# ma-compbio/MATCHA

Measured on AMD Instinct MI355X. Metric: training hyperedges/sec at k∈{2..5}, embed_dim=64; 1/2/4/8 MI355X, higher is better.
Workload: dtype f32; 1 GPU; hg38_1mb bins (N=3067), k in {2,3,4,5} mixed-k zero-padded to L=5, embed_dim=64, front end=table, neg_num=3, dropout on, AdamW lr=1e-3, 400000 known hyperedges; parallelism=dp1, hipgraph=False, table_gradient_exchange=none, embedding_backward=float atomics, exchange_overlapped=False

## Files before the change

### matcha_amd/csrc/front_fused.hip

```cpp
#include <string.h>

#include "attr_src.hpp"
#include "kernels.hpp"
#include "prep_heads.hpp"

namespace matcha {

typedef float f32x16 __attribute__((ext_vector_type(16)));

namespace {

constexpr int kLd = 68;
constexpr int kTile = 64 * kLd;
constexpr int kLdA = 36;
constexpr int kAttrCols = 32;
constexpr int kFrontSlab = 4096 + 64 * kAttrCols + 128;
constexpr float kEps = 1e-5f;

struct FrontBwdArgs {
  const float* X; const float* dxh; int nslab; int64_t tcap; const float* dxpad; const float* dXs; const float* x0;
  const int64_t* ids; AttrSrc attr; int n_attr;
  const float* Wn;
  const int32_t* count;
  float* dX0;
  float* dtable;
  float* slab;
};

template <bool NODE>
__global__ __launch_bounds__(256, 2) void front_bwd_kernel(FrontBwdArgs g) {
  extern __shared__ __attribute__((aligned(16))) float lds[];
  float* Ws = lds;
  float* Zs = lds + 1 * kTile;
  float* X0s = lds + 2 * kTile;
  float* Ds = lds + 3 * kTile;
  float* As = lds + 4 * kTile;
  int* ids_s = reinterpret_cast<int*>(As + 64 * kLdA);
  const int tid = threadIdx.x, lane = tid & 63, wave = tid >> 6;
  const int r = lane & 31, h = lane >> 5, wr = wave & 1, wc = wave >> 1;
  const int srow = tid >> 4, sc4 = (tid & 15) * 4;
  const int T = g.count[0];
  const int ntiles = (T + 63) / 64;
#pragma unroll
  for (int i = 0; i < 4; ++i)
    *reinterpret_cast<float4*>(&Ws[(srow + 16 * i) * kLd + sc4]) = *reinterpret_cast<const float4*>(g.Wn + (srow + 16 * i) * 64 + sc4);
  f32x16 aWn = {0}, aWa = {0};
  float csz = 0.f, csd = 0.f;

  float4 pxv[4], pdv[4], psv[4], px0[4], pav[2];
  int pid = 0;
  const float4 dxp = *reinterpret_cast<const float4*>(g.dxpad + sc4);
  const int a_row0 = tid >> 3, a_q = (tid & 7) * 4;
  const int a_qc = a_q < g.n_attr ? a_q : 0;
#define FBW_GLOAD(TILE)                                                                                  \
  do {                                                                                                   \
    const int64_t tb__ = (int64_t)(TILE) * 64;                                                           \
    _Pragma("unroll") for (int i__ = 0; i__ < 4; ++i__) {                                                \
// ... 84 lines not shown
          if (id != 0) atomicAdd(g.dtable + (int64_t)id * 64 + col, acc[reg]);
        }
      }
    }
#pragma unroll 8
    for (int m = 0; m < 32; ++m) {
      const int t = 2 * m + h;
      const float gz = Zs[t * kLd + 32 * wr + r];
      csz += gz;
      aWn = __builtin_amdgcn_mfma_f32_32x32x2f32(gz, X0s[t * kLd + 32 * wc + r], aWn, 0, 0, 0);
    }
    __syncthreads();
    if (g.dX0) {
#pragma unroll
      for (int i = 0; i < 4; ++i) {
        const int row = srow + 16 * i;
        const int64_t t = t_base + row;
        if (t < T) *reinterpret_cast<float4*>(g.dX0 + t * 64 + sc4) = *reinterpret_cast<const float4*>(&Ds[row * kLd + sc4]);
      }
    }
    if (wc == 0) {
#pragma unroll 8
      for (int m = 0; m < 32; ++m) {
        const int t = 2 * m + h;
        const float gd = Ds[t * kLd + 32 * wr + r];
        csd += gd;
        aWa = __builtin_amdgcn_mfma_f32_32x32x2f32(gd, As[t * kLdA + r], aWa, 0, 0, 0);
      }
    }
  }
  float* slab = g.slab + (int64_t)blockIdx.x * kFrontSlab;
#pragma unroll
  for (int reg = 0; reg < 16; ++reg) {
    const int row = 32 * wr + (reg & 3) + 8 * (reg >> 2) + 4 * h;
    slab[row * 64 + 32 * wc + r] = aWn[reg];
    if (wc == 0) slab[4096 + row * kAttrCols + r] = aWa[reg];
  }
  csz += __shfl_xor(csz, 32, 64);
  csd += __shfl_xor(csd, 32, 64);
  if (wc == 0 && h == 0) {
    slab[4096 + 64 * kAttrCols + 32 * wr + r] = csz;
    slab[4096 + 64 * kAttrCols + 64 + 32 * wr + r] = csd;
  }
}

struct FrontFwdArgs {
  const int64_t* ids; const float* table; const float* dense;
  AttrSrc attr; int n_attr;
  const float* Wa; const float* ba; const float* Wn; const float* bn;
  const int32_t* count;
  float* x0; float* X;
  int nprep; PrepArgs prep;
  int prep_walks;
};

__global__ __launch_bounds__(256, 3) void front_fwd_kernel(FrontFwdArgs g) {
  extern __shared__ __attribute__((aligned(16))) float lds[];
  const int nprep = g.nprep;
  if ((int)blockIdx.x < nprep) {
    const int b = blockIdx.x;
    prep_heads_role(g.prep, b % kPrepGridX, (b / kPrepGridX) % kPrepGridY, b / (kPrepGridX * kPrepGridY), lds);
    if (!g.prep_walks) return;
    __syncthreads();
  }
  const int nlate = g.prep_walks ? nprep : 0;
  const int vb = (int)blockIdx.x - (nprep - nlate), Gf = (int)gridDim.x - (nprep - nlate);
  float* Es = lds;
  float* As = lds + kTile;
  float* Xs = As + 64 * kLdA;
  const int tid = threadIdx.x, lane = tid & 63, wave = tid >> 6;
  const int r = lane & 31, h = lane >> 5, wr = wave & 1, wc = wave >> 1;
  const int srow = tid >> 4, sc4 = (tid & 15) * 4;
  const int T = g.count[0];
  const int ntiles = (T + 63) / 64;
  const int q = ntiles / Gf, r_last = ntiles - q * Gf;
  const int last_slot = vb >= nlate ? vb - nlate : vb - nlate + Gf;
  const int tile_last = last_slot < r_last ? q * Gf + last_slot : 0x3FFFFFF;
#define FF_TILE(IT) ((IT) < q ? vb + (IT) * Gf : ((IT) == q ? tile_last : 0x3FFFFFF))
  float4 wn[8], wa[kAttrCols / 8];
#pragma unroll
  for (int c = 0; c < 8; ++c) wn[c] = *reinterpret_cast<const float4*>(g.Wn + (32 * wc + r) * 64 + 8 * c + 4 * h);
#pragma unroll
  for (int c = 0; c < kAttrCols / 8; ++c) {
    const int q = 8 * c + 4 * h;
    wa[c] = make_float4(0.f, 0.f, 0.f, 0.f);
    if (q < g.n_attr) wa[c] = *reinterpret_cast<const float4*>(g.Wa + (32 * wc + r) * g.n_attr + q);
  }
  const int col = 32 * wc + r;
  const float bav = g.ba[col], bnv = g.bn[col];

  const int arow0 = tid >> 3, aq = (tid & 7) * 4;
  int64_t id_e[4], id_a[2];
  float4 pe[4], pa[2], qe[4], qa[2];
  const float amask = aq < g.n_attr ? 1.f : 0.f;
  const int aqc = aq < g.n_attr ? aq : g.n_attr - 4;
  const int64_t t_last = (int64_t)T - 1;
#define FF_IDS_GLOAD(TILE)                                                                               \
  do {                                                                                                   \
    const int64_t tb__ = (int64_t)(TILE) * 64;                                                           \
    _Pragma("unroll") for (int i__ = 0; i__ < 4; ++i__) {                                                \
      const int64_t t__ = tb__ + srow + 16 * i__;                                                        \
      id_e[i__] = g.ids[t__ < t_last ? t__ : t_last];                                                    \
    }                                                                                                    \
    _Pragma("unroll") for (int j__ = 0; j__ < 2; ++j__) {                                                \
      const int64_t t__ = tb__ + arow0 + 32 * j__;                                                       \
      id_a[j__] = g.ids[t__ < t_last ? t__ : t_last];                                                    \
    }                                                                                                    \
  } while (0)
#define FF_ROWS_GLOAD(TILE)                                                                              \
  do {                                                                                                   \
    const int64_t tb__ = (int64_t)(TILE) * 64;                                                           \
    _Pragma("unroll") for (int i__ = 0; i__ < 4; ++i__) {                                                \
      const int64_t t__ = tb__ + srow + 16 * i__;                                                        \
      const float* src__ = g.table ? g.table + id_e[i__] * 64 : g.dense + (t__ < t_last ? t__ : t_last) * 64; \
      pe[i__] = *reinterpret_cast<const float4*>(src__ + sc4);                                           \
    }                                                                                                    \
    _Pragma("unroll") for (int j__ = 0; j__ < 2; ++j__) {                                                \
      const float4 v__ = *reinterpret_cast<const float4*>(g.attr.table + id_a[j__] * g.attr.ld + aqc);   \
      pa[j__] = make_float4(v__.x * amask, v__.y * amask, v__.z * amask, v__.w * amask);                 \
// ... 46 lines not shown
        acc = __builtin_amdgcn_mfma_f32_32x32x2f32(a.y, b.y, acc, 0, 0, 0);
        acc = __builtin_amdgcn_mfma_f32_32x32x2f32(a.z, b.z, acc, 0, 0, 0);
        acc = __builtin_amdgcn_mfma_f32_32x32x2f32(a.w, b.w, acc, 0, 0, 0);
      }
#pragma unroll
      for (int reg = 0; reg < 16; ++reg) {
        const int row = 32 * wr + (reg & 3) + 8 * (reg >> 2) + 4 * h;
        const float v = acc[reg] + bav + Es[row * kLd + col];
        Es[row * kLd + col] = v;
      }
    }
    __syncthreads();
#pragma unroll
    for (int i = 0; i < 4; ++i) {
      const int row = srow + 16 * i;
      if (g.x0 && t_base + row < T) *reinterpret_cast<float4*>(g.x0 + (t_base + row) * 64 + sc4) = *reinterpret_cast<const float4*>(&Es[row * kLd + sc4]);
    }
    {
      f32x16 acc = {0};
#pragma unroll
      for (int c = 0; c < 8; ++c) {
        const float4 a = *reinterpret_cast<const float4*>(&Es[(32 * wr + r) * kLd + 8 * c + 4 * h]);
        const float4 b = wn[c];
        acc = __builtin_amdgcn_mfma_f32_32x32x2f32(a.x, b.x, acc, 0, 0, 0);
        acc = __builtin_amdgcn_mfma_f32_32x32x2f32(a.y, b.y, acc, 0, 0, 0);
        acc = __builtin_amdgcn_mfma_f32_32x32x2f32(a.z, b.z, acc, 0, 0, 0);
        acc = __builtin_amdgcn_mfma_f32_32x32x2f32(a.w, b.w, acc, 0, 0, 0);
      }
#pragma unroll
      for (int reg = 0; reg < 16; ++reg) {
        const int row = 32 * wr + (reg & 3) + 8 * (reg >> 2) + 4 * h;
        Xs[row * kLd + col] = fast_tanh(acc[reg] + bnv);
      }
    }
    __syncthreads();
#pragma unroll
    for (int i = 0; i < 4; ++i) {
      const int row = srow + 16 * i;
      if (t_base + row < T) *reinterpret_cast<float4*>(g.X + (t_base + row) * 64 + sc4) = *reinterpret_cast<const float4*>(&Xs[row * kLd + sc4]);
    }
  }
}

constexpr int kFPS = 80;
#define FF2_STORE4(P, A, B, C, D) (*reinterpret_cast<f32x4*>(P) = (f32x4){(A), (B), (C), (D)})
constexpr int kF3Lds = (3 * 64 * kFPS) / 2 + (kAttrCols + 2) * 64 + 64;

template <bool TRAIN>
__global__ __launch_bounds__(256, 4) void front_fwd3_kernel(FrontFwdArgs g) {
  extern __shared__ __attribute__((aligned(16))) float lds[];
  const int nprep = g.nprep;
  const int tid = threadIdx.x, lane = tid & 63, wave = tid >> 6;
  bool late = false;
  if ((int)blockIdx.x < nprep) {
    const int b = blockIdx.x;
    prep_heads_role(g.prep, b % kPrepGridX, (b / kPrepGridX) % kPrepGridY, b / (kPrepGridX * kPrepGridY), lds);
    if (!g.prep_walks) return;
    __syncthreads();
    late = true;
  }
  short* Wp = reinterpret_cast<short*>(lds);
  float* WaT = lds + (3 * 64 * kFPS) / 2;
  int* bnd = reinterpret_cast<int*>(WaT + (kAttrCols + 2) * 64);
  const int c16 = lane & 15, kq = lane >> 4;
  const int na = g.n_attr;
  {
    const int srow = tid >> 4, sc4 = (tid & 15) * 4;
#pragma unroll
    for (int i = 0; i < 4; ++i) {
      const int n = srow + 16 * i;
      const float4 w = *reinterpret_cast<const float4*>(g.Wn + n * 64 + sc4);
      const P3 p0 = split2(w.x, w.y), p1 = split2(w.z, w.w);
      short* d = Wp + n * kFPS + sc4;
      *reinterpret_cast<u32x2*>(d) = (u32x2){p0.h, p1.h}; *reinterpret_cast<u32x2*>(d + 64 * kFPS) = (u32x2){p0.m, p1.m};
      *reinterpret_cast<u32x2*>(d + 2 * 64 * kFPS) = (u32x2){p0.l, p1.l};
    }
    for (int i = tid; i < (na + 2) * 64; i += 256) {
      const int a = i >> 6, c = i & 63;
      WaT[i] = a < na - 1 ? g.Wa[c * na + a] : (a == na - 1 ? 0.f : (a == na ? g.Wa[c * na + na - 1] : g.ba[c]));
    }
    if (tid < na) bnd[tid] = g.attr.bounds[tid];
  }
  __syncthreads();
  const int T = g.count[0];
  const int64_t t_last = (int64_t)T - 1;
  const int ngroups = (T + 15) / 16;
  const int W = (int)gridDim.x * 4, Wn_ = W - nprep * 4;
  const int r0 = g.prep_walks > 0 ? g.prep_walks - 1 : 0x3FFFFF;
  const int wv = late ? (int)blockIdx.x * 4 + wave : ((int)blockIdx.x - nprep) * 4 + wave;
  const float scale = g.attr.scale;
  const int* ids32 = reinterpret_cast<const int*>(g.ids);
  const float4 bn4 = *reinterpret_cast<const float4*>(g.bn + 4 * kq);
#define F3_GROUP(R) ((R) < r0 ? (late ? 0x3FFFFFF : (R) * Wn_ + wv) : r0 * Wn_ + ((R) - r0) * W + (late ? wv : nprep * 4 + wv))
#define F3_LOAD(GRP, ID, E)                                                                              \
  do {                                                                                                   \
    const int64_t t__ = (int64_t)(GRP) * 16 + c16;                                                       \
    const int64_t tc__ = t__ < t_last ? t__ : t_last;                                                    \
    ID = ids32[2 * tc__];                                                                                \
    const float* src__ = (g.table ? g.table + (int64_t)ID * 64 : g.dense + tc__ * 64) + 8 * kq;          \
    E[0] = *reinterpret_cast<const float4*>(src__); E[1] = *reinterpret_cast<const float4*>(src__ + 4);   \
    E[2] = *reinterpret_cast<const float4*>(src__ + 32); E[3] = *reinterpret_cast<const float4*>(src__ + 36); \
  } while (0)
  int idn = 0;
  float4 en[4];
  const int r_first = late ? r0 : 0;
  int grp = F3_GROUP(r_first);
  if (grp < ngroups) F3_LOAD(grp, idn, en);
  for (int r = r_first; grp < ngroups; ++r) {
    const int id = idn;
    float4 e[4];
#pragma unroll
    for (int i = 0; i < 4; ++i) e[i] = en[i];
    const int gnext = F3_GROUP(r + 1);
    if (gnext < ngroups) F3_LOAD(gnext, idn, en);
    const int64_t t = (int64_t)grp * 16 + c16;
    const int nb_ = na - 1, top = bnd[nb_];
    const int idc = id < 1 ? 1 : (id > top ? top : id);
    const int ch = attr_chrom(bnd, nb_, idc);
    const bool real = id >= 1 && id <= top;
    const int wrow = real ? ch : nb_;
    const float co = real ? __fdiv_rn((float)(idc - bnd[ch] - 1), scale) : 0.f;
    Frag3 xf[2];
#pragma unroll
    for (int s2 = 0; s2 < 2; ++s2) {
      const int k0 = 32 * s2 + 8 * kq;
      float v[8];
#pragma unroll
      for (int hf = 0; hf < 2; ++hf) {
        const float4 wc_ = *reinterpret_cast<const float4*>(&WaT[wrow * 64 + k0 + 4 * hf]);
        const float4 wl_ = *reinterpret_cast<const float4*>(&WaT[na * 64 + k0 + 4 * hf]);
        const float4 ba_ = *reinterpret_cast<const float4*>(&WaT[(na + 1) * 64 + k0 + 4 * hf]);
        const float4 ee = e[2 * s2 + hf];
        v[4 * hf + 0] = (__builtin_fmaf(co, wl_.x, wc_.x) + ba_.x) + ee.x; v[4 * hf + 1] = (__builtin_fmaf(co, wl_.y, wc_.y) + ba_.y) + ee.y;
        v[4 * hf + 2] = (__builtin_fmaf(co, wl_.z, wc_.z) + ba_.z) + ee.z; v[4 * hf + 3] = (__builtin_fmaf(co, wl_.w, wc_.w) + ba_.w) + ee.w;
        if (TRAIN && t < T) FF2_STORE4(g.x0 + t * 64 + k0 + 4 * hf, v[4 * hf], v[4 * hf + 1], v[4 * hf + 2], v[4 * hf + 3]);
      }
      xf[s2] = split8(v);
    }
#pragma unroll 1
    for (int nb = 0; nb < 4; ++nb) {
      f32x4 acc = {0.f, 0.f, 0.f, 0.f};
      const short* ap = Wp + (16 * nb + c16) * kFPS + 8 * kq;
#pragma unroll
      for (int s2 = 0; s2 < 2; ++s2) {
        Frag3 a;
        a.h = *reinterpret_cast<const u32x4*>(ap + 32 * s2); a.m = *reinterpret_cast<const u32x4*>(ap + 32 * s2 + 64 * kFPS);
        a.l = *reinterpret_cast<const u32x4*>(ap + 32 * s2 + 2 * 64 * kFPS);
        acc = mma6(acc, a, xf[s2]);
      }
      const float4 bb = *reinterpret_cast<const float4*>(g.bn + 16 * nb + 4 * kq);
      if (t < T) FF2_STORE4(g.X + t * 64 + 16 * nb + 4 * kq, fast_tanh(acc[0] + bb.x), fast_tanh(acc[1] + bb.y), fast_tanh(acc[2] + bb.z), fast_tanh(acc[3] + bb.w));
    }
    grp = gnext;
  }
#undef F3_GROUP
#undef F3_LOAD
}

__global__ __launch_bounds__(256) void node_xhat_kernel(const float* __restrict__ XN, const int32_t* __restrict__ count, float* __restrict__ xh) {
  const int64_t row = (int64_t)blockIdx.x * 16 + (threadIdx.x >> 4);
  const int c4 = (threadIdx.x & 15) * 4;
  const int T = count[0];
  const float4 xv = *reinterpret_cast<const float4*>(XN + (row < T ? row : (int64_t)T - 1) * 64 + c4);
  const float mean = group_sum16_dpp((xv.x + xv.y) + (xv.z + xv.w)) * (1.f / 64.f);
  const float a = xv.x - mean, b = xv.y - mean, c = xv.z - mean, e = xv.w - mean;
  const float rs = __builtin_amdgcn_rsqf(group_sum16_dpp((a * a + b * b) + (c * c + e * e)) * (1.f / 64.f) + kEps);
  if (row < T) *reinterpret_cast<float4*>(xh + row * 64 + c4) = make_float4(a * rs, b * rs, c * rs, e * rs);
}

struct NodeScatterArgs {
  const float* XN; const float* dxh; const float* dxpad; const float* dXs; const int32_t* key; const int32_t* count;
  float* G;
  const int32_t* ncount; int64_t rows;
};
__device__ __forceinline__ void node_finish(const NodeScatterArgs& g) {
  const int64_t row = (int64_t)blockIdx.x * 16 + (threadIdx.x >> 4);
  const int c4 = (threadIdx.x & 15) * 4;
  const int T = g.ncount[0];
  const int64_t rc = row < T ? row : (int64_t)T - 1;
  const float4 xv = *reinterpret_cast<const float4*>(g.XN + rc * 64 + c4);
  float4 a[MATCHA_N_HEAD];
#pragma unroll
  for (int h = 0; h < MATCHA_N_HEAD; ++h) a[h] = *reinterpret_cast<const float4*>(g.dxh + ((int64_t)h * g.rows + rc) * 64 + c4);
  const float4 s = *reinterpret_cast<const float4*>(g.G + rc * 64 + c4);
  float4 d;
  d.x = ((a[0].x + a[1].x) + (a[2].x + a[3].x)) + ((a[4].x + a[5].x) + (a[6].x + a[7].x));
  d.y = ((a[0].y + a[1].y) + (a[2].y + a[3].y)) + ((a[4].y + a[5].y) + (a[6].y + a[7].y));
  d.z = ((a[0].z + a[1].z) + (a[2].z + a[3].z)) + ((a[4].z + a[5].z) + (a[6].z + a[7].z));
  d.w = ((a[0].w + a[1].w) + (a[2].w + a[3].w)) + ((a[4].w + a[5].w) + (a[6].w + a[7].w));
  if (rc == 0) {
    const float4 dxp = *reinterpret_cast<const float4*>(g.dxpad + c4);
    d.x += dxp.x; d.y += dxp.y; d.z += dxp.z; d.w += dxp.w;
  }
  const float mean = group_sum16_dpp((xv.x + xv.y) + (xv.z + xv.w)) * (1.f / 64.f);
  const float a0 = xv.x - mean, a1 = xv.y - mean, a2 = xv.z - mean, a3 = xv.w - mean;
  const float rs = __builtin_amdgcn_rsqf(group_sum16_dpp((a0 * a0 + a1 * a1) + (a2 * a2 + a3 * a3)) * (1.f / 64.f) + kEps);
  const float4 xh = make_float4(a0 * rs, a1 * rs, a2 * rs, a3 * rs);
  const float ma = group_sum16_dpp((d.x + d.y) + (d.z + d.w)) * (1.f / 64.f);
  const float mb = group_sum16_dpp((d.x * xh.x + d.y * xh.y) + (d.z * xh.z + d.w * xh.w)) * (1.f / 64.f);
  if (row < T)
    *reinterpret_cast<float4*>(g.G + row * 64 + c4) =
        make_float4(rs * (d.x - ma - xh.x * mb) + s.x, rs * (d.y - ma - xh.y * mb) + s.y, rs * (d.z - ma - xh.z * mb) + s.z, rs * (d.w - ma - xh.w * mb) + s.w);
}
__global__ __launch_bounds__(256) void node_scatter_kernel(NodeScatterArgs g) {
  if (g.ncount) { node_finish(g); return; }
  __shared__ __attribute__((aligned(16))) float rows_s[2][16 * 64];
  __shared__ int keys_s[2][16];
  const int tid = threadIdx.x, lane = tid & 63, wave = tid >> 6;
  const int srow = tid >> 4, sc4 = (tid & 15) * 4;
  const int T = g.count[0];
  const int ntrips = (T + 15) / 16;
  const float4 dxp = *reinterpret_cast<const float4*>(g.dxpad + sc4);
  const int stride = (int)gridDim.x;
  auto tok_of = [&](int trip) { const int64_t t = (int64_t)trip * 16 + srow; return t < T ? t : (int64_t)T - 1; };
  int kn = g.key[tok_of(blockIdx.x)], knn = g.key[tok_of(blockIdx.x + stride < ntrips ? blockIdx.x + stride : blockIdx.x)];
  float4 xn, dn, sn;
  {
    const int64_t tc = tok_of(blockIdx.x);
    xn = *reinterpret_cast<const float4*>(g.XN + (int64_t)kn * 64 + sc4);
    dn = *reinterpret_cast<const float4*>(g.dxh + tc * 64 + sc4);
    sn = *reinterpret_cast<const float4*>(g.dXs + tc * 64 + sc4);
  }
  int buf = 0;
  for (int trip = blockIdx.x; trip < ntrips; trip += stride, buf ^= 1) {
    const int64_t t = (int64_t)trip * 16 + srow;
    const bool valid = t < T;
    const int key = kn;
    const float4 xv = xn, s = sn;
    const float4 d = t >= (int64_t)T - 1 ? dxp : dn;
    {
      const int nxt = trip + stride < ntrips ? trip + stride : trip, nxt2 = nxt + stride < ntrips ? nxt + stride : nxt;
      const int64_t tc = tok_of(nxt);
      kn = knn;
      xn = *reinterpret_cast<const float4*>(g.XN + (int64_t)kn * 64 + sc4);
      dn = *reinterpret_cast<const float4*>(g.dxh + tc * 64 + sc4);
      sn = *reinterpret_cast<const float4*>(g.dXs + tc * 64 + sc4);
      knn = g.key[tok_of(nxt2)];
    }
    const float mean = group_sum16_dpp((xv.x + xv.y) + (xv.z + xv.w)) * (1.f / 64.f);
    const float a0 = xv.x - mean, a1 = xv.y - mean, a2 = xv.z - mean, a3 = xv.w - mean;
    const float rs = __builtin_amdgcn_rsqf(group_sum16_dpp((a0 * a0 + a1 * a1) + (a2 * a2 + a3 * a3)) * (1.f / 64.f) + kEps);
    const float4 xh = make_float4(a0 * rs, a1 * rs, a2 * rs, a3 * rs);
    const float ma = group_sum16_dpp((d.x + d.y) + (d.z + d.w)) * (1.f / 64.f);
    const float mb = group_sum16_dpp((d.x * xh.x + d.y * xh.y) + (d.z * xh.z + d.w * xh.w)) * (1.f / 64.f);
    *reinterpret_cast<float4*>(&rows_s[buf][srow * 64 + sc4]) =
        make_float4(rs * (d.x - ma - xh.x * mb) + s.x, rs * (d.y - ma - xh.y * mb) + s.y, rs * (d.z - ma - xh.z * mb) + s.z, rs * (d.w - ma - xh.w * mb) + s.w);
    if ((tid & 15) == 0) keys_s[buf][srow] = valid ? key : -1;
    __syncthreads();
#pragma unroll
    for (int i = 0; i < 4; ++i) {
      const int row = 4 * wave + i, k = keys_s[buf][row];
      if (k >= 0) atomicAdd(g.G + (int64_t)k * 64 + lane, rows_s[buf][row * 64 + lane]);
    }
  }
}

struct FrontReduceArgs {
  const float* slab; int nwg; int n_attr;
  float* dWn; float* dWa; float* dbn; float* dba;
  int32_t* touched;
};
__global__ __launch_bounds__(1024) void front_slab_reduce_kernel(FrontReduceArgs a) {
  __shared__ float part[16][64];
  if (a.touched && blockIdx.x == 0 && threadIdx.x < 2) a.touched[threadIdx.x] = 1;
  const int o = threadIdx.x & 63, q = threadIdx.x >> 6;
  const int i = blockIdx.x * 64 + o;
  float s = 0.f;
  if (i < kFrontSlab) {
    float s0 = 0.f, s1 = 0.f, s2 = 0.f, s3 = 0.f;
    int b = q;
    for (; b + 48 < a.nwg; b += 64) {
      s0 += a.slab[(int64_t)b * kFrontSlab + i]; s1 += a.slab[(int64_t)(b + 16) * kFrontSlab + i];
      s2 += a.slab[(int64_t)(b + 32) * kFrontSlab + i]; s3 += a.slab[(int64_t)(b + 48) * kFrontSlab + i];
    }
    for (; b < a.nwg; b += 16) s0 += a.slab[(int64_t)b * kFrontSlab + i];
    s = (s0 + s1) + (s2 + s3);
  }
  part[q][o] = s;
  __syncthreads();
  if (q == 0 && i < kFrontSlab) {
    float t = 0.f;
#pragma unroll
    for (int u = 0; u < 16; ++u) t += part[u][o];
    if (i < 4096) a.dWn[i] += t;
    else if (i < 4096 + 64 * kAttrCols) {
      const int n = (i - 4096) / kAttrCols, c = (i - 4096) % kAttrCols;
      if (c < a.n_attr) a.dWa[n * a.n_attr + c] += t;
    } else if (i < 4096 + 64 * kAttrCols + 64) a.dbn[i - 4096 - 64 * kAttrCols] += t;
    else a.dba[i - 4096 - 64 * kAttrCols - 64] += t;
  }
}

int front_grid() {
  const int n = 2 * device_cu_count();
  return n > 1024 ? 1024 : n;
}

}

int launch_front_fwd(const matcha_tensors& p, const int64_t* ids, const float* table, const float* dense, const matcha_frozen& f, int n_attr,
                     const Ragged& rg, int64_t tcap, float* x0, float* X, hipStream_t st, const PrepSpec* prep, const int32_t* count) {
  MATCHA_CHECK_ARG(f.attr_table, "front end: attr_table is required (also under attr_mode 1)");
  FrontFwdArgs g;
  const bool computed = f.attr_mode == 1 && f.attr_bounds && n_attr <= kAttrCols;
  g.ids = ids; g.table = table; g.dense = dense; g.attr = computed ? attr_src(f, n_attr) : attr_src_table_first(f, n_attr); g.n_attr = n_attr;
  g.Wa = p.attr_w; g.ba = p.attr_b; g.Wn = p.next_w; g.bn = p.next_b; g.count = count ? count : rg.count; g.x0 = x0; g.X = X;
  const int slots = front_grid() / 2 * 3;
  const int64_t max_tiles = cdiv(tcap, 64);
  const size_t lds = ((size_t)2 * kTile + 64 * kLdA) * sizeof(float);
  static_assert(((size_t)2 * kTile + 64 * kLdA) >= (size_t)kPrepLdsFloats && kF3Lds >= kPrepLdsFloats, "the weight-form role needs its LDS inside the front end's");
  g.nprep = 0;
  if (prep) {
    prep_heads_args(*prep->p, prep->folded, prep->merged, prep->frag, g.prep);
    g.nprep = kPrepBlocks;
  } else {
    memset(&g.prep, 0, sizeof(g.prep));
  }
  g.prep_walks = (g.nprep > 0 && max_tiles + g.nprep > slots) ? 1 : 0;
  int64_t grid = g.prep_walks ? slots : g.nprep + (max_tiles < slots ? max_tiles : slots);
  if (grid < g.nprep + 1) grid = g.nprep + 1;
  ProfScope ps(MATCHA_PROF_FRONT_FWD, (double)tcap * (8.0 + 256.0 + (computed ? 0.0 : 4.0 * n_attr) + (x0 ? 512.0 : 256.0)), st);
  if (computed) {
    const int slots4 = front_grid() * 2;
    const int64_t ngroups = cdiv(tcap, 16);
    const int64_t rounds = cdiv(ngroups, (int64_t)slots4 * 4);
    g.prep_walks = (g.nprep > 0 && rounds >= 4) ? 3 : 0;
    int64_t grid3 = g.prep_walks ? slots4 : g.nprep + (cdiv(ngroups, 4) < slots4 ? cdiv(ngroups, 4) : slots4);
    if (grid3 < g.nprep + 1) grid3 = g.nprep + 1;
    const size_t lds3 = (size_t)kF3Lds * sizeof(float);
    static_assert(kF3Lds >= kPrepLdsFloats, "the weight-form role needs its LDS inside the front end's");
    if (x0) hipLaunchKernelGGL(front_fwd3_kernel<true>, dim3((unsigned)grid3), dim3(256), lds3, st, g);
    else hipLaunchKernelGGL(front_fwd3_kernel<false>, dim3((unsigned)grid3), dim3(256), lds3, st, g);
    MATCHA_CHECK_LAUNCH("front_fwd3_kernel");
  } else {
    hipLaunchKernelGGL(front_fwd_kernel, dim3((unsigned)grid), dim3(256), lds, st, g);
    MATCHA_CHECK_LAUNCH("front_fwd_kernel");
  }
  return MATCHA_OK;
}

int launch_node_xhat(const float* XN, const int32_t* node_count, int64_t rows_cap, float* xhatN, hipStream_t st) {
  ProfScope ps(MATCHA_PROF_FRONT_FWD, (double)rows_cap * 512.0, st);
  hipLaunchKernelGGL(node_xhat_kernel, dim3((unsigned)cdiv(rows_cap, 16)), dim3(256), 0, st, XN, node_count, xhatN);
  MATCHA_CHECK_LAUNCH("node_xhat_kernel");
  return MATCHA_OK;
}

int launch_node_scatter(const float* XN, const float* dxh, const float* dxpad, const float* dXs, const Ragged& rg, int64_t tcap, float* G, hipStream_t st,
                        const int32_t* node_count, int64_t rows) {
  NodeScatterArgs g;
  g.XN = XN; g.dxh = dxh; g.dxpad = dxpad; g.dXs = dXs; g.key = rg.tok_key; g.count = rg.count; g.G = G; g.ncount = node_count; g.rows = rows;
  if (node_count) {
    MATCHA_CHECK_ARG(rows > 0, "node_scatter: the per-node finisher needs the table's row count");
    ProfScope ps(MATCHA_PROF_FRONT_BWD, (double)rows * (MATCHA_N_HEAD + 3.0) * 256.0, st);
    hipLaunchKernelGGL(node_scatter_kernel, dim3((unsigned)cdiv(rows, 16)), dim3(256), 0, st, g);
    MATCHA_CHECK_LAUNCH("node_scatter_kernel");
    return MATCHA_OK;
  }
  int64_t grid = (int64_t)front_grid() * 4;
  const int64_t trips = cdiv(tcap, 16);
  if (grid > trips) grid = trips;
  ProfScope ps(MATCHA_PROF_FRONT_BWD, (double)tcap * (4.0 * 256.0 + 4.0), st);
  hipLaunchKernelGGL(node_scatter_kernel, dim3((unsigned)grid), dim3(256), 0, st, g);
  MATCHA_CHECK_LAUNCH("node_scatter_kernel");
  return MATCHA_OK;
}

bool front_bwd_supported(int d, int n_attr) { return d == 64 && n_attr >= 4 && n_attr <= kAttrCols && n_attr % 4 == 0; }
size_t front_bwd_ws_floats() { return (size_t)1024 * kFrontSlab; }

int launch_front_bwd(const matcha_tensors& p, const float* X, const float* dxh, int nslab, int64_t tcap, const float* dxpad, const float* dXs, const float* x0,
                     const int64_t* ids, const matcha_frozen& f, int n_attr, const Ragged& rg, float* dX0, float* dtable, float* ws,
                     matcha_tensors& grads, hipStream_t st, int32_t* touched, const int32_t* node_count) {
  MATCHA_CHECK_ARG(f.attr_table, "front end: attr_table is required (also under attr_mode 1)");
  FrontBwdArgs g;
  g.X = X; g.dxh = dxh; g.nslab = nslab; g.tcap = tcap; g.dxpad = dxpad; g.dXs = dXs; g.x0 = x0; g.ids = ids; g.attr = attr_src_table_first(f, n_attr); g.n_attr = n_attr;
  g.Wn = p.next_w; g.count = node_count ? node_count : rg.count; g.dX0 = dX0; g.dtable = dtable; g.slab = ws;
  const bool node = node_count != nullptr;
  int grid = front_grid();
  const int64_t max_tiles = cdiv(tcap, 64);
  if (grid > max_tiles) grid = (int)max_tiles;
  const size_t lds = ((size_t)4 * kTile + 64 * kLdA + 64) * sizeof(float);
  (void)hipFuncSetAttribute(reinterpret_cast<const void*>(node ? front_bwd_kernel<true> : front_bwd_kernel<false>), hipFuncAttributeMaxDynamicSharedMemorySize, (int)lds);
  {
    ProfScope ps(MATCHA_PROF_FRONT_BWD, (double)tcap * ((3.0 + (node ? 0 : nslab)) * 256.0 + 8.0 + (g.attr.mode == 1 ? 0.0 : 4.0 * n_attr) + 256.0), st);
    if (node) hipLaunchKernelGGL(front_bwd_kernel<true>, dim3(grid), dim3(256), lds, st, g);
    else hipLaunchKernelGGL(front_bwd_kernel<false>, dim3(grid), dim3(256), lds, st, g);
    MATCHA_CHECK_LAUNCH("front_bwd_kernel");
  }
  FrontReduceArgs a;
  a.slab = ws; a.nwg = grid; a.n_attr = n_attr; a.dWn = grads.next_w; a.dWa = grads.attr_w; a.dbn = grads.next_b; a.dba = grads.attr_b;
  a.touched = touched;
  hipLaunchKernelGGL(front_slab_reduce_kernel, dim3((unsigned)cdiv(kFrontSlab, 64)), dim3(1024), 0, st, a);
  MATCHA_CHECK_LAUNCH("front_slab_reduce_kernel");
  return MATCHA_OK;
}

}
```

### matcha_amd/csrc/fused_bwd.hip

```cpp
#include <stdlib.h>
#include <string.h>

#include "bf16x3.hpp"
#include "kernels.hpp"
#include "tail_reduce.hpp"

namespace matcha {

typedef float f32x16 __attribute__((ext_vector_type(16)));

namespace {

constexpr int kLd = 68;
constexpr float kEpsLn = 1e-5f;
constexpr int kWgSlab = 4 * 4096 + 6 * 64;
constexpr int kVecOff = 4 * 4096;
constexpr int kMaxChunks = 64;

#define ZR8(p)                                                                                           \
  do {                                                                                                   \
    *reinterpret_cast<float4*>(p) = make_float4(0.f, 0.f, 0.f, 0.f);                                     \
    *reinterpret_cast<float4*>((p) + 4) = make_float4(0.f, 0.f, 0.f, 0.f);                               \
  } while (0)

__device__ __forceinline__ void ln_row16(const float4& v, float& mean, float& rstd) {
  const float s = group_sum<16>((v.x + v.y) + (v.z + v.w));
  mean = s * (1.f / 64.f);
  const float a = v.x - mean, b = v.y - mean, c = v.z - mean, e = v.w - mean;
  const float q = group_sum<16>((a * a + b * b) + (c * c + e * e));
  rstd = __builtin_amdgcn_rsqf(q * (1.f / 64.f) + kEpsLn);
}


#define FB_PIN(addr, x) asm volatile("" : "+v"(addr), "+v"((x).a), "+v"((x).b), "+v"((x).c), "+v"((x).d))
template <int ML>
__device__ __forceinline__ void attn_row8_kv(const float* __restrict__ Qs, const float* __restrict__ Xs, const float* __restrict__ Fs,
                                             const float* __restrict__ xpad, const float* __restrict__ Ps, float* __restrict__ dSs, int li, int li0,
                                             int k, int n_pad, int sub, float inv_temp, V8& o, V8& gq, V8& accK, V8& accV) {
  const float padf = (float)n_pad;
  const bool hp = n_pad > 0;
  float p[ML], ds[ML], pp;
  {
    const float4 pa = *reinterpret_cast<const float4*>(&Ps[li * 8]), pb = *reinterpret_cast<const float4*>(&Ps[li * 8 + 4]);
    const float w[8] = {pa.x, pa.y, pa.z, pa.w, pb.x, pb.y, pb.z, pb.w};
#pragma unroll
    for (int j = 0; j < ML; ++j) p[j] = (j < k) ? w[j] : 0.f;
    pp = hp ? w[7] : 0.f;
  }
  const float ppf = padf * pp;
  const int ro0 = li0 * kLd + 8 * sub;
  const V8 go = ld8(&Fs[li * kLd + 8 * sub]);
  const V8 vp = ld8(xpad + 8 * sub);
  const float dsp_raw = group_sum8_dpp(dot8(go, vp));
  float sig = ppf * dsp_raw;
  o = scale8(ppf, vp);
  V8 a = scale8(ppf * dsp_raw, vp);
  V8 vn = ld8(&Xs[ro0]), vn2 = ld8(&Xs[ro0 + (1 < k ? 1 : 0) * kLd]);
#pragma unroll
  for (int j = 0; j < ML; ++j) {
    const V8 v = vn;
    vn = vn2;
    if (j + 2 < ML) {
      int ad = ro0 + (j + 2 < k ? j + 2 : 0) * kLd;
      FB_PIN(ad, o);
      vn2 = ld8(&Xs[ad]);
    }
    axpy8(o, p[j], v);
    const float d = group_sum8_dpp(dot8(go, v));
    ds[j] = d;
    const float wd = p[j] * d;
    sig += wd;
    axpy8(a, wd, v);
  }
#pragma unroll
  for (int j = 0; j < ML; ++j) ds[j] = p[j] * (ds[j] - sig) * inv_temp;
  const float dspf = padf * (pp * (dsp_raw - sig) * inv_temp);
  axpy8(accV, ppf, go);
  {
    const float ns = -sig;
    axpy8(a, ns, o);
    gq = scale8(inv_temp, a);
  }
  {
    int ad = li * kLd + 8 * sub;
// ... 551 lines not shown
    if (tid < 64) upad[tid] = (redu[tid] + redu[64 + tid]) + (redu[128 + tid] + redu[192 + tid]);
    __syncthreads();
    {
      const float xc = xpad[fb + c16];
#pragma unroll
      for (int reg = 0; reg < 4; ++reg) {
        const int row = 4 * kq + reg, col = fb + c16;
        slab[1 * 4096 + row * 64 + col] = am0[reg] + upad[row] * xc; slab[1 * 4096 + (row + 16) * 64 + col] = am1[reg] + upad[row + 16] * xc;
        slab[1 * 4096 + (row + 32) * 64 + col] = am2[reg] + upad[row + 32] * xc; slab[1 * 4096 + (row + 48) * 64 + col] = am3[reg] + upad[row + 48] * xc;
      }
    }
    if (tid < 64) {
      const float* mp = g.mM + (int64_t)head * 4096 + tid;
      float s0 = 0.f, s1 = 0.f, s2 = 0.f, s3 = 0.f;
#pragma unroll 4
      for (int n = 0; n < 64; n += 4) {
        s0 += upad[n] * mp[n * 64]; s1 += upad[n + 1] * mp[(n + 1) * 64]; s2 += upad[n + 2] * mp[(n + 2) * 64]; s3 += upad[n + 3] * mp[(n + 3) * 64];
      }
      slab[kVecOffM + 128 + tid] = ((redp[tid] + redp[64 + tid]) + (redp[128 + tid] + redp[192 + tid])) + ((s0 + s1) + (s2 + s3));
    }
  }
}

struct ChainArgs {
  const float* wslab; int nchunks;
  float* red;
  const float* wq; const float* wk; const float* wv; const float* cq; const float* cv;
  const float* fc1_w;
  float* out;
  float* dxpad;
};
constexpr int kFbmReduceX = (kWgSlabM + 255) / 256;
constexpr int kFbmReduceBlocks = kFbmReduceX * MATCHA_N_HEAD;
__global__ __launch_bounds__(256) void fbm_reduce_kernel(ChainArgs a, TailReduceArgs tl, int tail_blocks) {
  __shared__ float4 part[8 * 32];
  if ((int)blockIdx.x >= kFbmReduceBlocks) {
    tail_reduce_role(tl, (int)blockIdx.x - kFbmReduceBlocks, part);
    return;
  }
  const int head = blockIdx.x / kFbmReduceX, i = (blockIdx.x % kFbmReduceX) * 256 + threadIdx.x;
  if (i >= kWgSlabM) return;
  const float* base = a.wslab + (int64_t)head * a.nchunks * kWgSlabM + i;
  float s0 = 0.f, s1 = 0.f, s2 = 0.f, s3 = 0.f, s4 = 0.f, s5 = 0.f, s6 = 0.f, s7 = 0.f;
  int c = 0;
  for (; c + 7 < a.nchunks; c += 8) {
    s0 += base[(int64_t)c * kWgSlabM]; s1 += base[(int64_t)(c + 1) * kWgSlabM]; s2 += base[(int64_t)(c + 2) * kWgSlabM]; s3 += base[(int64_t)(c + 3) * kWgSlabM];
    s4 += base[(int64_t)(c + 4) * kWgSlabM]; s5 += base[(int64_t)(c + 5) * kWgSlabM]; s6 += base[(int64_t)(c + 6) * kWgSlabM]; s7 += base[(int64_t)(c + 7) * kWgSlabM];
  }
  for (; c < a.nchunks; ++c) s0 += base[(int64_t)c * kWgSlabM];
  a.red[(int64_t)head * kWgSlabM + i] = ((s0 + s1) + (s2 + s3)) + ((s4 + s5) + (s6 + s7));
}
__device__ __forceinline__ void mm64_slice(const float* __restrict__ A, int a_rs, int a_cs, const float* __restrict__ B, int b_rs, int b_cs,
                                           const float* __restrict__ u, const float* __restrict__ v, float* __restrict__ out, int slice,
                                           float* __restrict__ As, float* __restrict__ Bs) {
  const int tid = threadIdx.x;
  {
    float av[4], bv[16];
#pragma unroll
    for (int t = 0; t < 4; ++t) { const int i = tid + 256 * t; av[t] = A[(int64_t)(16 * slice + (i >> 6)) * a_rs + (int64_t)(i & 63) * a_cs]; }
#pragma unroll
    for (int t = 0; t < 16; ++t) { const int i = tid + 256 * t; bv[t] = B[(int64_t)(i >> 6) * b_rs + (int64_t)(i & 63) * b_cs]; }
#pragma unroll
    for (int t = 0; t < 4; ++t) { const int i = tid + 256 * t; As[(i >> 6) * 65 + (i & 63)] = av[t]; }
#pragma unroll
    for (int t = 0; t < 16; ++t) { const int i = tid + 256 * t; Bs[(i >> 6) * 65 + (i & 63)] = bv[t]; }
  }
  __syncthreads();
  const int lane = tid & 63, wave = tid >> 6, c16 = lane & 15, kq = lane >> 4;
  f32x4 acc = {0.f, 0.f, 0.f, 0.f};
#pragma unroll
  for (int kk = 0; kk < 16; ++kk) acc = MFMA16(As[c16 * 65 + 4 * kk + kq], Bs[(4 * kk + kq) * 65 + 16 * wave + c16], acc);
  const int j = 16 * wave + c16;
  const float vj = u ? v[j] : 0.f;
#pragma unroll
  for (int reg = 0; reg < 4; ++reg) {
    const int i = 4 * kq + reg;
    out[(16 * slice + i) * 64 + j] = acc[reg] + (u ? u[16 * slice + i] * vj : 0.f);
  }
}
__global__ __launch_bounds__(256) void fbm_chain_kernel(ChainArgs a) {
  __shared__ float As[16 * 65];
  __shared__ float Bs[64 * 65];
  const int slice = blockIdx.x, job = blockIdx.y, head = blockIdx.z, tid = threadIdx.x;
  const float* red = a.red + (int64_t)head * kWgSlabM;
  const float* dB = red; const float* dM = red + 4096; const float* db = red + kVecOffM;
  const float* dbdyn = a.red + kVecOffM + 64;
  const float* Wq = a.wq + (int64_t)head * 4096; const float* Wk = a.wk + (int64_t)head * 4096; const float* Wv = a.wv + (int64_t)head * 4096;
  const float* Wf = a.fc1_w + head * 64;
  float* out = a.out + (int64_t)head * kWgSlab;
  if (job == 0) {
    mm64_slice(Wk, 64, 1, dB, 64, 1, nullptr, nullptr, out + 0 * 4096, slice, As, Bs);
  } else if (job == 1) {
    mm64_slice(Wq, 64, 1, dB, 1, 64, a.cq + head * 64, db, out + 1 * 4096, slice, As, Bs);
  } else if (job == 2) {
    mm64_slice(Wf, 1, 512, dM, 64, 1, nullptr, nullptr, out + 2 * 4096, slice, As, Bs);
  } else {
    mm64_slice(dM, 64, 1, Wv, 1, 64, dbdyn, a.cv + head * 64, out + 3 * 4096, slice, As, Bs);
  }
  if (slice == 0 && job == 0 && tid < 64) {
    float s0 = 0.f, s1 = 0.f, t0 = 0.f, t1 = 0.f;
#pragma unroll 8
    for (int x = 0; x < 64; x += 2) {
      s0 += Wk[tid * 64 + x] * db[x]; s1 += Wk[tid * 64 + x + 1] * db[x + 1];
      t0 += Wf[x * 512 + tid] * dbdyn[x]; t1 += Wf[(x + 1) * 512 + tid] * dbdyn[x + 1];
    }
    const float s = s0 + s1, t = t0 + t1;
    out[kVecOff + tid] = s;
    out[kVecOff + 64 + tid] = 0.f;
    out[kVecOff + 128 + tid] = t;
    out[kVecOff + 192 + tid] = 0.f; out[kVecOff + 256 + tid] = 0.f;
    out[kVecOff + 320 + tid] = head == 0 ? dbdyn[tid] : 0.f;
    if (head == 0) {
      float p = 0.f;
      for (int hh = 0; hh < MATCHA_N_HEAD; ++hh) p += a.red[(int64_t)hh * kWgSlabM + kVecOffM + 128 + tid];
      a.dxpad[tid] = p;
    }
  }
}

struct UnfoldArgs {
  const float* wslab; int nchunks;
  const float* X; const int32_t* count; int x_pad_row0;
  const float* W[3]; const float* g[3]; const float* b[3];
  float* gW[3]; float* gfc1;
  float* part;
};
__global__ __launch_bounds__(256) void fb_unfold_kernel(UnfoldArgs a) {
  __shared__ float red[16][3][64];
  const int slice = blockIdx.x, mat = blockIdx.y, head = blockIdx.z;
  const int tid = threadIdx.x, rl = tid >> 4, c4 = (tid & 15) * 4;
  const int row = slice * 16 + rl;
  const float* base = a.wslab + (int64_t)head * a.nchunks * kWgSlab;
  float4 s = make_float4(0.f, 0.f, 0.f, 0.f);
  {
    float4 t0 = s, t1 = s, t2 = s, t3 = s;
    const float* pb = base + mat * 4096 + row * 64 + c4;
    int c = 0;
    for (; c + 3 < a.nchunks; c += 4) {
      const float4 v0 = *reinterpret_cast<const float4*>(pb + (int64_t)c * kWgSlab), v1 = *reinterpret_cast<const float4*>(pb + (int64_t)(c + 1) * kWgSlab);
      const float4 v2 = *reinterpret_cast<const float4*>(pb + (int64_t)(c + 2) * kWgSlab), v3 = *reinterpret_cast<const float4*>(pb + (int64_t)(c + 3) * kWgSlab);
      t0.x += v0.x; t0.y += v0.y; t0.z += v0.z; t0.w += v0.w;
      t1.x += v1.x; t1.y += v1.y; t1.z += v1.z; t1.w += v1.w;
      t2.x += v2.x; t2.y += v2.y; t2.z += v2.z; t2.w += v2.w;
      t3.x += v3.x; t3.y += v3.y; t3.z += v3.z; t3.w += v3.w;
    }
    for (; c < a.nchunks; ++c) {
      const float4 v = *reinterpret_cast<const float4*>(pb + (int64_t)c * kWgSlab);
      t0.x += v.x; t0.y += v.y; t0.z += v.z; t0.w += v.w;
    }
    s.x = (t0.x + t1.x) + (t2.x + t3.x); s.y = (t0.y + t1.y) + (t2.y + t3.y);
    s.z = (t0.z + t1.z) + (t2.z + t3.z); s.w = (t0.w + t1.w) + (t2.w + t3.w);
  }
  if (mat == 3) {
    float4* o = reinterpret_cast<float4*>(a.gfc1 + (int64_t)row * 512 + head * 64 + c4);
    float4 v = *o;
    v.x += s.x; v.y += s.y; v.z += s.z; v.w += s.w;
    *o = v;
    return;
  }
  float dc = 0.f, dpad = 0.f;
  for (int c = 0; c < a.nchunks; ++c) {
    const float* vb = base + (int64_t)c * kWgSlab + kVecOff;
    dc += vb[mat * 64 + row];
    if (mat > 0) dpad += vb[192 + (mat - 1) * 64 + row];
  }
  const float4 xv = *reinterpret_cast<const float4*>(a.X + (a.x_pad_row0 ? (int64_t)0 : (int64_t)a.count[1] * 64) + c4);
  float m, rs;
  ln_row16(xv, m, rs);
  s.x += dpad * (xv.x - m) * rs; s.y += dpad * (xv.y - m) * rs; s.z += dpad * (xv.z - m) * rs; s.w += dpad * (xv.w - m) * rs;
  dc += dpad;
  const int64_t wi = ((int64_t)head * 64 + row) * 64 + c4;
  const float4 W = *reinterpret_cast<const float4*>(a.W[mat] + wi);
  const float4 G = *reinterpret_cast<const float4*>(a.g[mat] + c4), Bv = *reinterpret_cast<const float4*>(a.b[mat] + c4);
  {
    float4* o = reinterpret_cast<float4*>(a.gW[mat] + wi);
    float4 v = *o;
    v.x += s.x * G.x + dc * Bv.x; v.y += s.y * G.y + dc * Bv.y; v.z += s.z * G.z + dc * Bv.z; v.w += s.w * G.w + dc * Bv.w;
    *o = v;
  }
  *reinterpret_cast<float4*>(&red[rl][0][c4]) = make_float4(s.x * W.x, s.y * W.y, s.z * W.z, s.w * W.w);
  *reinterpret_cast<float4*>(&red[rl][1][c4]) = make_float4(dc * W.x, dc * W.y, dc * W.z, dc * W.w);
  *reinterpret_cast<float4*>(&red[rl][2][c4]) = make_float4(dpad * W.x * G.x, dpad * W.y * G.y, dpad * W.z * G.z, dpad * W.w * G.w);
  __syncthreads();
  if (tid < 192) {
    const int which = tid >> 6, k = tid & 63;
    float t = 0.f;
#pragma unroll
    for (int q = 0; q < 16; ++q) t += red[q][which][k];
    a.part[(((int64_t)(head * 4 + slice) * 3 + mat) * 3 + which) * 64 + k] = t;
  }
}

struct Unfold2Args {
  const float* part; const float* wslab; int nchunks;
  float* dg[3]; float* db[3]; float* dfc1_b; float* dxpad;
  int dxpad_add;
};
__global__ __launch_bounds__(512) void fb_unfold2_kernel(Unfold2Args a) {
  const int vec = threadIdx.x >> 6, k = threadIdx.x & 63;
  float s = 0.f;
  if (vec < 6) {
    const int mat = vec >> 1, which = vec & 1;
    for (int p = 0; p < 32; ++p) s += a.part[(((int64_t)p * 3 + mat) * 3 + which) * 64 + k];
    float* o = (which == 0 ? a.dg[mat] : a.db[mat]) + k;
    *o += s;
  } else if (vec == 6) {
    for (int p = 0; p < 32; ++p) s += a.part[(((int64_t)p * 3 + 1) * 3 + 2) * 64 + k] + a.part[(((int64_t)p * 3 + 2) * 3 + 2) * 64 + k];
    a.dxpad[k] = a.dxpad_add ? a.dxpad[k] + s : s;
  } else {
    for (int c = 0; c < a.nchunks; ++c) s += a.wslab[(int64_t)c * kWgSlab + kVecOff + 320 + k];
    a.dfc1_b[k] += s;
  }
}

__global__ __launch_bounds__(256) void lnhat_bwd_kernel(const float* __restrict__ X, const float* __restrict__ dxh, int64_t tcap,
                                                        const float* __restrict__ dxpad, const float* __restrict__ dXs,
                                                        float* __restrict__ dZ0, const int32_t* __restrict__ count, int nslab) {
  const int T = count[0];
  const int64_t t = (int64_t)blockIdx.x * 16 + (threadIdx.x >> 4);
  const int c4 = (threadIdx.x & 15) * 4;
  if (t >= T) return;
  const float4 xv = *reinterpret_cast<const float4*>(X + t * 64 + c4);
  float m, rs;
  ln_row16(xv, m, rs);
  const float4 xh = make_float4((xv.x - m) * rs, (xv.y - m) * rs, (xv.z - m) * rs, (xv.w - m) * rs);
  float4 d;
  if (t < T - 1) {
    d = *reinterpret_cast<const float4*>(dxh + t * 64 + c4);
    for (int hd = 1; hd < nslab; ++hd) {
      const float4 v = *reinterpret_cast<const float4*>(dxh + ((int64_t)hd * tcap + t) * 64 + c4);
      d.x += v.x; d.y += v.y; d.z += v.z; d.w += v.w;
    }
  } else {
    d = *reinterpret_cast<const float4*>(dxpad + c4);
  }
  const float a = group_sum<16>((d.x + d.y) + (d.z + d.w)) * (1.f / 64.f);
  const float b = group_sum<16>((d.x * xh.x + d.y * xh.y) + (d.z * xh.z + d.w * xh.w)) * (1.f / 64.f);
  const float4 s = *reinterpret_cast<const float4*>(dXs + t * 64 + c4);
  float4 o;
  o.x = (rs * (d.x - a - xh.x * b) + s.x) * (1.f - xv.x * xv.x);
  o.y = (rs * (d.y - a - xh.y * b) + s.y) * (1.f - xv.y * xv.y);
  o.z = (rs * (d.z - a - xh.z * b) + s.z) * (1.f - xv.z * xv.z);
  o.w = (rs * (d.w - a - xh.w * b) + s.w) * (1.f - xv.w * xv.w);
  *reinterpret_cast<float4*>(dZ0 + t * 64 + c4) = o;
}

int chunks_for(int ntiles) {
  const int cus = device_cu_count();
  int c = cus / MATCHA_N_HEAD;
  if (c > kMaxChunks) c = kMaxChunks;
  if (c > ntiles) c = ntiles;
  return c < 1 ? 1 : c;
}

}

const float* fused_bwd_dxpad(const float* ws) { return ws + (size_t)MATCHA_N_HEAD * kMaxChunks * kWgSlab + 32 * 3 * 3 * 64; }

size_t fused_bwd_ws_floats(int64_t B, int L) {
  (void)B; (void)L;
  return (size_t)MATCHA_N_HEAD * kMaxChunks * kWgSlab + (size_t)32 * 3 * 3 * 64 + 64;
}

int launch_fused_bwd_merged(const matcha_tensors& p, const Ragged& rg, int64_t B, int L, const FusedBwdLaunch& a, matcha_tensors& grads, hipStream_t st) {
  const int64_t tcap = B * L + 1;
  const float *folded = a.folded, *X = a.x.X, *xhatN = a.x.xhat, *rn = a.x.rn, *vn = a.x.vn, *dXs = a.dXs;
  const int32_t* xrow = a.x.xrow;
  const bool dx_atomic = a.dx_atomic;
  float *dxh = a.dxh, *ws = a.ws;
  MATCHA_CHECK_ARG(!xrow || xhatN, "fused backward: the node route needs the table of normalised rows");
  MATCHA_CHECK_ARG(!rn || xrow, "fused backward: the r table belongs to the node route");
  MATCHA_CHECK_ARG(!vn || rn, "fused backward: the value table needs the r table");
  MATCHA_CHECK_ARG(!a.dx_node || (vn && dx_atomic && a.dx_zeroed), "fused backward: per-node d x_hat sums need the value table, the atomics and a caller that zeroed them");
  if (dx_atomic && !a.dx_zeroed) MATCHA_TRY(zero_async(dxh, (size_t)tcap * 64 * sizeof(float), st));
  int nchunks = 2 * chunks_for(rg.nhalves);
  if (nchunks > kMaxChunks) nchunks = kMaxChunks;
  if (nchunks > rg.nhalves) nchunks = rg.nhalves > 0 ? rg.nhalves : 1;
  float* wslab = ws;
  float* chain = ws + (size_t)MATCHA_N_HEAD * kMaxChunks * kWgSlabM;
  float* part = ws + (size_t)MATCHA_N_HEAD * kMaxChunks * kWgSlab;
  float* dxpad = part + 32 * 3 * 3 * 64;
  const size_t wsz = (size_t)MATCHA_N_HEAD * 64 * 64, csz = (size_t)MATCHA_N_HEAD * 64;
  const MergedView mv = merged_view(a.merged);
  {
    FusedBwdHArgs g;
    g.X = xrow ? xhatN : X; g.dDyn = a.dDyn; g.count = rg.count; g.half_meta = rg.half_meta; g.tok_pos = rg.tok_pos; g.L = L; g.nhalves = rg.nhalves; g.nchunks = nchunks;
    g.mB = mv.B; g.mM = mv.M; g.dxh = dxh; g.tcap = tcap; g.dx_atomic = dx_atomic ? 1 : 0; g.wslab = wslab; g.rimg = a.rimg; g.xrow = xrow;
    g.rn = rn; g.rn_head = a.x.rows * 64; g.vn = vn; g.dx_node = a.dx_node ? dxh : nullptr;
    const size_t lds = kBwdLdsBytes;
    auto launch = [&](auto kfn) {
      (void)hipFuncSetAttribute(reinterpret_cast<const void*>(kfn), hipFuncAttributeMaxDynamicSharedMemorySize, 160 * 1024);
      hipLaunchKernelGGL(kfn, dim3(MATCHA_N_HEAD * nchunks), dim3(256), lds, st, g);
    };
    ProfScope ps(MATCHA_PROF_FUSED_BWD, (double)tcap * MATCHA_N_HEAD * 8.0 * 2.0 * 64.0 * 64.0, st);
    dispatch_ml(L, [&](auto ml) {
      constexpr int ML = decltype(ml)::value;
      if (vn) launch(fused_bwdh_kernel<ML, true, true>); else if (xrow) launch(fused_bwdh_kernel<ML, true>); else launch(fused_bwdh_kernel<ML, false>);
    });
    MATCHA_CHECK_LAUNCH("fused_bwdh_kernel");
  }
  {
    ChainArgs c;
    c.wslab = wslab; c.nchunks = nchunks; c.red = chain + (size_t)MATCHA_N_HEAD * kWgSlab;
    c.wq = folded; c.wk = folded + wsz; c.wv = folded + 2 * wsz; c.cq = folded + 3 * wsz; c.cv = c.cq + 2 * csz;
    c.fc1_w = p.fc1_w; c.out = chain; c.dxpad = dxpad;
    TailReduceArgs tl;
    if (a.tail) tl = *a.tail; else memset(&tl, 0, sizeof(tl));
    const int tail_blocks = a.tail ? kTailRoleBlocks : 0;
    hipLaunchKernelGGL(fbm_reduce_kernel, dim3((unsigned)(kFbmReduceBlocks + tail_blocks)), dim3(256), 0, st, c, tl, tail_blocks);
    MATCHA_CHECK_LAUNCH("fbm_reduce_kernel");
    hipLaunchKernelGGL(fbm_chain_kernel, dim3(4, 4, MATCHA_N_HEAD), dim3(256), 0, st, c);
    MATCHA_CHECK_LAUNCH("fbm_chain_kernel");
  }
  {
    UnfoldArgs a;
    a.wslab = chain; a.nchunks = 1; a.X = X; a.count = rg.count; a.x_pad_row0 = xrow ? 1 : 0;
    a.W[0] = p.w_q; a.W[1] = p.w_k; a.W[2] = p.w_v;
    a.g[0] = p.ln_q_g; a.g[1] = p.ln_k_g; a.g[2] = p.ln_v_g;
    a.b[0] = p.ln_q_b; a.b[1] = p.ln_k_b; a.b[2] = p.ln_v_b;
    a.gW[0] = grads.w_q; a.gW[1] = grads.w_k; a.gW[2] = grads.w_v; a.gfc1 = grads.fc1_w;
    a.part = part;
    hipLaunchKernelGGL(fb_unfold_kernel, dim3(4, 4, MATCHA_N_HEAD), dim3(256), 0, st, a);
    MATCHA_CHECK_LAUNCH("fb_unfold_kernel");
    Unfold2Args b;
    b.part = part; b.wslab = chain; b.nchunks = 1;
    b.dg[0] = grads.ln_q_g; b.dg[1] = grads.ln_k_g; b.dg[2] = grads.ln_v_g;
    b.db[0] = grads.ln_q_b; b.db[1] = grads.ln_k_b; b.db[2] = grads.ln_v_b;
    b.dfc1_b = grads.fc1_b; b.dxpad = dxpad; b.dxpad_add = 1;
    hipLaunchKernelGGL(fb_unfold2_kernel, dim3(1), dim3(512), 0, st, b);
    MATCHA_CHECK_LAUNCH("fb_unfold2_kernel");
  }
  if (float* dZ0 = a.dZ0) {
    MATCHA_CHECK_ARG(!xrow, "fused backward: the node route has no dZ0 output");
    hipLaunchKernelGGL(lnhat_bwd_kernel, dim3((unsigned)cdiv(tcap, 16)), dim3(256), 0, st, X, dxh, tcap, dxpad, dXs, dZ0, rg.count, dx_atomic ? 1 : MATCHA_N_HEAD);
    MATCHA_CHECK_LAUNCH("lnhat_bwd_kernel");
  }
  return MATCHA_OK;
}

}
```

### matcha_amd/csrc/fused_fwd32.hip

```cpp
#include "kernels.hpp"
#include "prep_heads.hpp"

#ifndef F32_ABL
#define F32_ABL 0
#endif

namespace matcha {

typedef float f32x16 __attribute__((ext_vector_type(16)));

namespace {

constexpr int kLdH = 68;
constexpr int kHT = 32 * kLdH;
constexpr float kEps32 = 1e-5f;
constexpr int kTailVec32 = 2 * 4096;
constexpr int kTailSlab32 = 2 * 4096 + 10 * 64;

struct FL { f32x16 lo, hi; };

__device__ __forceinline__ float xhalf_sum(float v) {
  float a = v, b = v;
  asm volatile("s_nop 1\n\tv_permlane32_swap_b32 %0, %1" : "+v"(a), "+v"(b));
  return a + b;
}
__device__ __forceinline__ float fl_sum(const FL& a) {
  float s0 = 0.f, s1 = 0.f;
#pragma unroll
  for (int e = 0; e < 16; ++e) { s0 += a.lo[e]; s1 += a.hi[e]; }
  return s0 + s1;
}
__device__ __forceinline__ float fl_dot(const FL& a, const FL& b) {
  float s0 = 0.f, s1 = 0.f;
#pragma unroll
  for (int e = 0; e < 16; ++e) { s0 += a.lo[e] * b.lo[e]; s1 += a.hi[e] * b.hi[e]; }
  return s0 + s1;
}
__device__ __forceinline__ void fl_stats(const FL& v, float& mean, float& rstd) {
  mean = xhalf_sum(fl_sum(v)) * (1.f / 64.f);
  float q0 = 0.f, q1 = 0.f;
#pragma unroll
  for (int e = 0; e < 16; ++e) { const float a = v.lo[e] - mean, b = v.hi[e] - mean; q0 += a * a; q1 += b * b; }
  rstd = __builtin_amdgcn_rsqf(xhalf_sum(q0 + q1) * (1.f / 64.f) + kEps32);
}
__device__ __forceinline__ void fl_store(float* __restrict__ rowp, const FL& v) {
#pragma unroll
  for (int g = 0; g < 4; ++g) {
    *reinterpret_cast<f32x4*>(rowp + 8 * g) = (f32x4){v.lo[4 * g], v.lo[4 * g + 1], v.lo[4 * g + 2], v.lo[4 * g + 3]};
    *reinterpret_cast<f32x4*>(rowp + 32 + 8 * g) = (f32x4){v.hi[4 * g], v.hi[4 * g + 1], v.hi[4 * g + 2], v.hi[4 * g + 3]};
  }
}
__device__ __forceinline__ FL fl_load(const float* __restrict__ rowp) {
  FL v;
#pragma unroll
// ... 476 lines not shown
  __syncthreads();
  F32_STAGE8(F32_MG_ONLY);
  {
    FL dynp = fl_zero();
    if (hd == 0) dynp = F32_BIAS(kBiasDyn);
    W32_CHAIN(dynp, o, false);
    fl_store(Pd + hd * kHT + r * kLdH + 4 * h, dynp);
  }
  __syncthreads();
  if (hd != 0) return;
  FL dyn = fl_load(Pd + r * kLdH + 4 * h);
#pragma unroll 1
  for (int j = 1; j < MATCHA_N_HEAD; ++j) {
    const FL t = fl_load(Pd + j * kHT + r * kLdH + 4 * h);
#pragma unroll
    for (int e = 0; e < 16; ++e) { dyn.lo[e] += t.lo[e]; dyn.hi[e] += t.hi[e]; }
  }
  W32_PRIME_AT(16);
#define F32_TAIL_SYNC() F32_WAVE_SYNC()
#define F32_PARK_Y(V) do { fl_store(Pd + r * kLdH + 4 * h, V); if (g.Y && !g.ddyn0 && r <= n) fl_store_global(g.Y + F32_ROW(), V); } while (0)
#define F32_PARK_H1(V) do { fl_store(Pd + kHT + r * kLdH + 4 * h, V); if (g.H1 && !g.ddyn0 && r <= n) fl_store_global(g.H1 + F32_ROW(), V); } while (0)
#define F32_UNPARK_Y() fl_unpark_lds(Pd, r * kLdH + 4 * h)
#define F32_UNPARK_H1() fl_unpark_lds(Pd + kHT, r * kLdH + 4 * h)
#define F32_PARK_HH(V) fl_store(Pd + 2 * kHT + r * kLdH + 4 * h, V)
#define F32_UNPARK_HH() fl_unpark_lds(Pd + 2 * kHT, r * kLdH + 4 * h)
#define F32_DXS_OUT(V) do { if (r <= n) fl_store_global(g.dXs + F32_ROW(), V); } while (0)
#include "fused_fwd32_tail.hpp"
#undef F32_DXS_OUT
#undef F32_TAIL_SYNC
#undef F32_PARK_Y
#undef F32_PARK_H1
#undef F32_UNPARK_Y
#undef F32_UNPARK_H1
#undef F32_PARK_HH
#undef F32_UNPARK_HH
#ifdef F32H_REPRO
  if (g.L == 0x40000000) {
    __threadfence();
    unsigned int* ctr = reinterpret_cast<unsigned int*>(g.tslab);
    unsigned int t = 0;
    if (lane == 0) t = atomicAdd(ctr, 1u);
    t = __shfl(t, 0, 64);
    if (t == gridDim.x - 1) {
      float s = 0.f;
      for (int i = lane; i < g.L * 977; i += 64) s += g.row_loss[i];
#pragma unroll
      for (int o = 32; o > 0; o >>= 1) s += __shfl_xor(s, o, 64);
      if (lane == 0) g.logits[0] = s;
    }
  }
#endif
}

struct NodeRArgs { const float* X; const u32x4* wfrag; float* rn; int rows; float* vn; };
__global__ __launch_bounds__(64) void node_r_kernel(NodeRArgs g) {
  const int lane = threadIdx.x, r = lane & 31, h = lane >> 5;
  const int hd = blockIdx.y & 7;
  const bool vrole = blockIdx.y >= MATCHA_N_HEAD;
  const int row = (int)blockIdx.x * 32 + r;
  const bool live = row < g.rows;
  const u32x4* wp;
  u32x4 W_[F32_WIN];
  W32_PRIME_AT(vrole ? (hd < 7 ? 2 * hd + 2 : 15) : (hd == 0 ? 0 : 2 * hd - 1));
  FL xh = fl_load(g.X + (int64_t)(live ? row : g.rows - 1) * 64 + 4 * h);
  {
    float mean, rx;
    fl_stats(xh, mean, rx);
#pragma unroll
    for (int e = 0; e < 16; ++e) { xh.lo[e] = (xh.lo[e] - mean) * rx; xh.hi[e] = (xh.hi[e] - mean) * rx; }
  }
  B3 xs[4];
  FL_SPLIT(xs[0], xh, 0); FL_SPLIT(xs[1], xh, 1); FL_SPLIT(xs[2], xh, 2); FL_SPLIT(xs[3], xh, 3);
  FL q = F32_BIAS(kBiasR + hd);
  if (vrole) q = fl_zero();
  W32_CHAIN_XS(q, xs, false);
  if (live) fl_store_global((vrole ? g.vn : g.rn) + ((int64_t)hd * g.rows + row) * 64 + 4 * h, q);
}

size_t node_r_floats(int64_t rows) { return (size_t)MATCHA_N_HEAD * rows * 64; }
int launch_node_r(const float* XN, const float* frag, int64_t rows, float* rn, hipStream_t st, float* vn) {
  NodeRArgs g;
  g.X = XN; g.wfrag = reinterpret_cast<const u32x4*>(frag); g.rn = rn; g.rows = (int)rows; g.vn = vn;
  ProfScope ps(MATCHA_PROF_FUSED_FWD, 0.0, st);
  hipLaunchKernelGGL(node_r_kernel, dim3((unsigned)cdiv(rows, 32), vn ? 2 * MATCHA_N_HEAD : MATCHA_N_HEAD), dim3(64), 0, st, g);
  MATCHA_CHECK_LAUNCH("node_r_kernel");
  return MATCHA_OK;
}

static int fwd32h_max_halves() { return 2 * device_cu_count(); }

bool fused_small_batch(const Ragged& rg) { return rg.nhalves <= fwd32h_max_halves() && !options().disable_small_batch; }

size_t fused_frag_floats() { return (size_t)(kNMat + 1) * kFragU4 * 4 + (size_t)kNBias * 64; }
size_t fused_tail_slab32_floats(int64_t B, int L) { return (size_t)(ragged_halves_cap(B, L) + 2) * kTailSlab32; }

size_t fused_merged_floats() { return (size_t)2 * MATCHA_N_HEAD * 4096 + MATCHA_N_HEAD * 64 + 64; }
MergedView merged_view(const float* m) {
  return MergedView{m, m + (size_t)MATCHA_N_HEAD * 4096, m + (size_t)2 * MATCHA_N_HEAD * 4096, m + (size_t)2 * MATCHA_N_HEAD * 4096 + MATCHA_N_HEAD * 64};
}
void prep_heads_args(const matcha_tensors& p, float* folded, float* merged, float* frag, PrepArgs& a) {
  const size_t wsz = (size_t)MATCHA_N_HEAD * 64 * 64, csz = (size_t)MATCHA_N_HEAD * 64;
  a.Wq = p.w_q; a.Wk = p.w_k; a.Wv = p.w_v;
  a.gq = p.ln_q_g; a.gk = p.ln_k_g; a.gv = p.ln_v_g; a.bq = p.ln_q_b; a.bv = p.ln_v_b;
  a.fc1_w = p.fc1_w; a.fc1_b = p.fc1_b; a.p0w = p.pff0_w; a.p0b = p.pff0_b; a.p1w = p.pff1_w; a.p1b = p.pff1_b;
  a.fwq = folded; a.fwk = folded + wsz; a.fwv = folded + 2 * wsz; a.fcq = folded + 3 * wsz; a.fcv = a.fcq + 2 * csz;
  const MergedView v = merged_view(merged);
  a.B = const_cast<float*>(v.B); a.M = const_cast<float*>(v.M); a.bvec = const_cast<float*>(v.bvec); a.bdyn = const_cast<float*>(v.bdyn);
  a.frag = reinterpret_cast<u32x4*>(frag);
}
int launch_prep_heads(const matcha_tensors& p, float* folded, float* merged, float* frag, hipStream_t st) {
  PrepArgs a;
  prep_heads_args(p, folded, merged, frag, a);
  hipLaunchKernelGGL(prep_heads_kernel, dim3(kPrepGridX, kPrepGridY, kPrepGridZ), dim3(256), 0, st, a);
  MATCHA_CHECK_LAUNCH("prep_heads_kernel");
  return MATCHA_OK;
}

int launch_fused_fwd32(const matcha_tensors& p, const Ragged& rg, int64_t B, int L, const FusedFwdLaunch& a, hipStream_t st) {
  Fwd32Args g;
  g.xrow = a.x.xrow;
  MATCHA_CHECK_ARG(!a.x.rn || a.x.xrow, "fused forward: the r table belongs to the node route");
  g.rn = a.x.rn; g.rn_rows = (int)a.x.rows;
  g.tail_dh2 = nullptr; g.dxs_node = nullptr;
  g.X = a.x.X; g.row_off = rg.row_off; g.tok_slot = rg.tok_slot; g.count = rg.count; g.half_meta = rg.half_meta; g.tok_pos = rg.tok_pos;
  g.L = L;
  g.wfrag = reinterpret_cast<const u32x4*>(a.frag);
  g.hp = HeadParams{p.pff_ln_g, p.pff_ln_b, p.ln1_g, p.ln1_b, p.ln2_g, p.ln2_b, p.cls_w, p.cls_b};
  const bool target = a.objective == MATCHA_OBJECTIVE_SOFTPLUS_MSE ? a.y != nullptr : (a.y && a.w);
  g.objective = a.objective;
  g.y = a.y; g.w = a.w; g.Y = a.Y; g.H1 = a.H1; g.H2 = a.H2; g.logits = a.logits; g.row_loss = target ? a.row_loss : nullptr;
  g.seed = a.seed; g.p_fc1 = a.p_fc1; g.p_pff = a.p_pff;
  g.ddyn0 = target ? a.ddyn0 : nullptr; g.dXs = a.dXs; g.tslab = a.tslab; g.alpha_over_B = a.alpha / (float)B; g.qkv = a.rimg;
  ProfScope ps(MATCHA_PROF_FUSED_FWD, (double)(B * L + 1) * (MATCHA_N_HEAD * 4.0 + 2.0) * 2.0 * 64.0 * 64.0, st);
  if (a.small) {
    MATCHA_CHECK_ARG(!a.x.xrow, "fused forward: the node route runs the large-batch kernel only");
    const size_t ldsh = ((size_t)10 * kHT + 64) * sizeof(float);
    dispatch_ml(L, [&](auto ml) {
// ... 18 lines not shown
```

### matcha_amd/csrc/kernels.hpp

```cpp
#pragma once
#include "common.hpp"

namespace matcha {

struct GemmArgs {
  const float* A[3];
  const float* B[3];
  float* C[3];
  int64_t M, N, K;
  int64_t lda, ldb, ldc;
  int batch;
  int flags;
  const float* bias[3];
  const float* residual;
  const float* aux;
  const int64_t* row_ids;
  const uint64_t* seed;
  uint32_t stream_id;
  float p_drop;
  float aux_scale;
  const int32_t* m_dev;
  const int32_t* a_row_map;
  const int32_t* c_row_map;
  const int32_t* seg;
  int n_groups;
  int64_t b_group_stride;
  const int32_t* rng_row_map;
};

struct Ragged {
  int32_t* row_off;
  int32_t* tok_slot;
  int64_t* tok_id;
  int32_t* count;
  int32_t* blk_sum;
  int nblk;
  int ntiles;
  int32_t* tok_pos;
  int32_t* tok_key;
  int32_t* tile_meta;
  int32_t* sb_tiles;
  int32_t* sb_cnt;
  int32_t* sb_first;
  int nsb, sb_cap;
  int32_t* half_meta;
  int32_t* tok_tile;
  int32_t* sb_htiles;
  int32_t* sb_hcnt;
  int nhalves, sb_hcap;
};
size_t ragged_bytes(int64_t B, int L);
int ragged_tiles_cap(int64_t B, int L);
int ragged_halves_cap(int64_t B, int L);
void ragged_carve(int64_t B, int L, char* base, Ragged& r);
int launch_ragged_plan(const int64_t* x, int64_t B, int L, int64_t n_nodes, int32_t* status, const Ragged& r, hipStream_t st, int level = 2,
                       int64_t* node_ids = nullptr, int32_t* node_cnt = nullptr, float* node_zero = nullptr);

struct HeadParams {
  const float *gp, *bp, *g1, *b1, *g2, *b2, *wc, *bc;
};

int launch_gemm_rm(bool b_kn, const GemmArgs& g, hipStream_t st);
size_t gemm_tn_ws_bytes(int64_t M, int64_t N, int64_t R);
int launch_gemm_tn(const float* A, const float* B, float* C, float* colsum, int64_t M, int64_t N, int64_t R, int64_t lda,
                   int64_t ldb, const int64_t* b_gather, bool accumulate, void* ws, size_t ws_bytes, hipStream_t st,
                   const int32_t* r_dev = nullptr, const float* out_scale_dev = nullptr, float out_scale = 1.f);
int launch_slab_reduce(const float* slab, float* out1, int64_t n1, float* out2, int64_t stride, int P, bool accumulate, hipStream_t st,
                       const float* scale_dev = nullptr, float scale = 1.f);

struct BmmProduct {
  const float* A; int64_t a_rs, a_cs, a_hs;
  const float* B; int64_t b_rs, b_cs, b_hs;
  float* C; int64_t c_rs, c_hs;
  int accumulate;
};
bool bmm_heads_supported(int d);
int launch_bmm_heads(const BmmProduct* prods, int n, int d, hipStream_t st);

bool gemm_wide_eligible(bool b_kn, const GemmArgs& g);
int launch_gemm_wide(bool b_kn, const GemmArgs& g, hipStream_t st);
bool gemm_tn_wide_eligible(int64_t M, int64_t N, int64_t R, int64_t lda, int64_t ldb, const float* A, const float* B, const int64_t* b_gather);
size_t gemm_tn_wide_ws_bytes(int64_t M, int64_t N, int64_t R);
int launch_gemm_tn_wide(const float* A, const float* B, int64_t M, int64_t N, int64_t R, int64_t lda, int64_t ldb, bool colsum, void* ws,
                        size_t ws_bytes, const int32_t* r_dev, int* P_out, int64_t* slab_stride_out, hipStream_t st);

int launch_embed_fwd(const int64_t* x, int64_t T, int d, const float* table, const float* dense, const matcha_frozen& f,
                     int n_attr, const float* Wa, const float* ba, float* x0, hipStream_t st, const int32_t* t_dev = nullptr);
int launch_embed_scatter(const int64_t* x, int64_t T, int d, const float* dx0, float* dtable, hipStream_t st, const int32_t* t_dev = nullptr);
int launch_gather_rows(const int64_t* ids, int64_t T, int d, const float* table, int64_t n_nodes, float* rows, int32_t* status, hipStream_t st);
int launch_check_ids(const int64_t* ids, int64_t T, int64_t n_nodes, int32_t* status, hipStream_t st);
int launch_expand_embedding(const int64_t* x, int64_t B, int L, int d, const int32_t* row_off, const float* H2, const float* X, const float* gp,
                            const float* bp, float* dynamic, float* static_, hipStream_t st);

size_t table_grad_ws_bytes(int64_t n, int n_nodes);
int launch_table_grad(const int32_t* ids, const float* rows, int64_t n, int d, int n_nodes, float* dtable, void* ws, size_t ws_bytes, hipStream_t st);

struct Options {
  int disable_fused;
  int disable_merged;
  int disable_small_batch;
  int disable_wide_gemm;
  int disable_node_front;
  int disable_node_r;
  int disable_node_v;
  int disable_node_dx;
  int debug_nan, fused_dbg;
};
Options& options();
int launch_fill_i32(int32_t* p, int n, int32_t v, hipStream_t st);
int zero_async(void* p, size_t bytes, hipStream_t st);
int launch_ln3_fwd(const float* X, int64_t T, int d, const float* gq, const float* bq, const float* gk, const float* bk,
                   const float* gv, const float* bv, float* qin, float* kin, float* vin, float* stats, hipStream_t st,
                   const int32_t* t_dev = nullptr);
int launch_ln3_bwd(const float* X, const float* dqin, const float* dkin, const float* dvin, const float* dXs, int64_t T, int d,
                   const float* gq, const float* gk, const float* gv, float* dZ0, float* slab, float* dgq, float* dbq,
                   float* dgk, float* dbk, float* dgv, float* dbv, hipStream_t st, const int32_t* t_dev = nullptr);
int launch_head_fwd(const int32_t* row_off, const float* H2, const float* X, int64_t B, int L, int d, const HeadParams& hp,
                    const float* y, const float* w, float* logits, float* row_loss, float* bce_out, hipStream_t st,
                    int objective = MATCHA_OBJECTIVE_BCE);
int launch_head_bwd(const int32_t* row_off, const float* H2, const float* X, int64_t B, int L, int d, const HeadParams& hp,
                    const float* y, const float* w, const float* logits, const float* dlogits, float alpha, float* dH2,
                    float* dXs, float* slab, const HeadParams& ghp, hipStream_t st, int objective = MATCHA_OBJECTIVE_BCE,
                    const int32_t* xrow = nullptr);
size_t colsum_slab_bytes(int64_t n, int nv, int d);
int launch_loss_reduce(const float* row_loss, int64_t B, float* bce_out, hipStream_t st, bool zero_recon = false,
                       float* zero_buf = nullptr, size_t zero_bytes = 0);

size_t fused_fold_floats();
size_t fused_tail_slab_floats(int64_t B, int L);
size_t fused_tail_partial_floats();
int launch_tail_reduce(const float* tslab, const Ragged& rg, int L, matcha_tensors& grads, hipStream_t st, bool halves, float* partial);
bool fused_small_batch(const Ragged& rg);

size_t fused_frag_floats();
size_t fused_tail_slab32_floats(int64_t B, int L);
size_t fused_merged_floats();
struct MergedView { const float* B; const float* M; const float* bvec; const float* bdyn; };
MergedView merged_view(const float* merged);
int launch_prep_heads(const matcha_tensors& p, float* folded, float* merged, float* frag, hipStream_t st);
struct NodeOperands {
  float* X;
  const int32_t* xrow;
  float* xhat;
  float* rn;
  float* vn;
  int64_t rows;
};
struct FusedFwdLaunch {
  const float* frag;
  NodeOperands x;
  bool small;
  const float *y, *w;
  int objective;
  float *Y, *H1, *H2;
  float *logits, *row_loss;
  const uint64_t* seed; float p_fc1, p_pff;
  float *ddyn0, *dXs, *tslab; float alpha;
  float* rimg;
  float* tail_dh2;
  float* dxs_node = nullptr;
};
int launch_fused_fwd32(const matcha_tensors& p, const Ragged& rg, int64_t B, int L, const FusedFwdLaunch& a, hipStream_t st);
size_t node_r_floats(int64_t rows);
int launch_node_r(const float* XN, const float* frag, int64_t rows, float* rn, hipStream_t st, float* vn = nullptr);
int tail_bwd_grid();
size_t tail_bwd_slab_floats();
int launch_tail_bwd64(const matcha_tensors& p, const float* dH2, const float* Y, const float* H1, const Ragged& rg, const uint64_t* seed, float p_fc1,
                      float p_pff, float* ddyn0, float* slab, const float* vslab, float* zero_rows, int64_t zero_floats, hipStream_t st,
                      const float* row_loss = nullptr, int64_t B = 0, float* losses = nullptr, bool zero_recon = false);

size_t fused_bwd_ws_floats(int64_t B, int L);
struct TailReduceArgs;
struct FusedBwdLaunch {
  const float *folded, *merged;
  NodeOperands x;
  const float *dDyn, *dXs;
  const float* rimg;
  float* dxh;
  float* ws;
  float* dZ0;
  bool dx_atomic, dx_zeroed;
  bool dx_node = false;
  const TailReduceArgs* tail;
};
int launch_fused_bwd_merged(const matcha_tensors& p, const Ragged& rg, int64_t B, int L, const FusedBwdLaunch& a, matcha_tensors& grads, hipStream_t st);
size_t fused_qkv_floats(int64_t B, int L);
constexpr int kImgRecH = 2048 + 256;

const float* fused_bwd_dxpad(const float* ws);

bool enc128_shape(int d);
size_t enc128_ws_floats();
size_t enc128_rec_floats(const Ragged& rg);
int launch_enc128_fwd(const matcha_tensors& p, const float* lwB, const float* lwM, const float* X, const Ragged& rg, int64_t B, int L, float* Y, float* rec,
                      float* ws, const int32_t* tok_slot, const uint64_t* seed, float p_drop, hipStream_t st);
int launch_enc128_bwd(const matcha_tensors& p, const float* lwB, const float* lwM, const float* X, const float* dDyn, const float* dXs, const Ragged& rg,
                      int64_t B, int L, float* dxh, const float* rec, float* ws, float* lwdB, float* lwdM, matcha_tensors& grads, float* dZ0,
                      hipStream_t st);

bool front_bwd_supported(int d, int n_attr);
struct PrepSpec { const matcha_tensors* p; float* folded; float* merged; float* frag; };
int launch_front_fwd(const matcha_tensors& p, const int64_t* ids, const float* table, const float* dense, const matcha_frozen& f, int n_attr,
                     const Ragged& rg, int64_t tcap, float* x0, float* X, hipStream_t st, const PrepSpec* prep = nullptr,
                     const int32_t* count = nullptr);
size_t front_bwd_ws_floats();
int launch_front_bwd(const matcha_tensors& p, const float* X, const float* dxh, int nslab, int64_t tcap, const float* dxpad, const float* dXs, const float* x0,
                     const int64_t* ids, const matcha_frozen& f, int n_attr, const Ragged& rg, float* dX0, float* dtable, float* ws,
                     matcha_tensors& grads, hipStream_t st, int32_t* touched = nullptr,
                     const int32_t* node_count = nullptr);
int launch_node_xhat(const float* XN, const int32_t* node_count, int64_t rows_cap, float* xhatN, hipStream_t st);
int launch_node_scatter(const float* XN, const float* dxh, const float* dxpad, const float* dXs, const Ragged& rg, int64_t tcap, float* G, hipStream_t st,
                        const int32_t* node_count = nullptr, int64_t rows = 0);

int launch_attn_fwd(const float* Q, const float* K, const float* V, const int32_t* row_off, int64_t B, int L, int d, float* O, float* P,
                    hipStream_t st, bool shared_kv = false);
int launch_attn_bwd(const float* Q, const float* K, const float* V, const float* P, const float* dO, const int32_t* row_off, int64_t B, int L,
                    int d, float* dQ, float* dK, float* dV, float* slab, hipStream_t st, bool shared_kv = false, float* dKsum = nullptr,
                    float* dVsum = nullptr);
size_t attn_bwd_slab_bytes(int64_t B, int d);
bool attn_wide_eligible(int d);
int launch_attn_fwd_wide(const float* Q, const float* K, const float* V, const int32_t* row_off, int64_t B, int L, int d, float inv_temp, float* O,
                         float* P, int nblk, hipStream_t st, bool shared_kv = false);
int launch_attn_bwd_wide(const float* Q, const float* K, const float* V, const float* P, const float* dO, const int32_t* row_off, int64_t B, int L,
                         int d, float inv_temp, float* dQ, float* dK, float* dV, float* slab, int nblk, hipStream_t st, bool shared_kv = false,
                         float* dKs = nullptr, float* dVs = nullptr);

size_t long_plan_bytes(int64_t B, int L);
void long_plan_carve(int64_t B, int L, char* base, Ragged& r, uint32_t** mask);
int launch_long_plan(const int64_t* x, int64_t B, int L, int64_t n_nodes, int32_t* status, const Ragged& r, uint32_t* mask, hipStream_t st);
int launch_attn_long(const float* Q, const float* K, const float* V, const int32_t* row_off, int64_t B, int L, int d, int64_t kv_ld, int kv_head,
                     float* O, hipStream_t st);

}
```

### matcha_amd/csrc/model.hip

```cpp
#include <stdlib.h>
#include <string.h>

#include <mutex>
#include <unordered_map>

#include "kernels.hpp"
#include "tail_reduce.hpp"

namespace matcha {

thread_local char g_err[512] = "";
void set_error(const char* fmt, ...) {
  va_list ap;
  va_start(ap, fmt);
  vsnprintf(g_err, sizeof(g_err), fmt, ap);
  va_end(ap);
}

int device_cu_count() {
  static int cache[64] = {};
  int dev = 0;
  if (hipGetDevice(&dev) != hipSuccess) { (void)hipGetLastError(); return 256; }
  if (dev >= 0 && dev < 64 && cache[dev] > 0) return cache[dev];
  int n = 0;
  if (hipDeviceGetAttribute(&n, hipDeviceAttributeMultiprocessorCount, dev) != hipSuccess || n <= 0) { (void)hipGetLastError(); return 256; }
  if (dev >= 0 && dev < 64) cache[dev] = n;
  return n;
}

int g_prof_class = 0;
static hipEvent_t* g_prof_ev = nullptr;
static int g_prof_cap = 0, g_prof_used = 0;
static double g_prof_work = 0.0;
void prof_record(bool start, double work, hipStream_t st) {
  if (start) {
    if (g_prof_used + 2 > g_prof_cap) {
      const int ncap = g_prof_cap ? 2 * g_prof_cap : 1024;
      hipEvent_t* ne = (hipEvent_t*)realloc(g_prof_ev, sizeof(hipEvent_t) * ncap);
      if (!ne) return;
      g_prof_ev = ne;
      for (int i = g_prof_cap; i < ncap; ++i)
        if (hipEventCreate(&g_prof_ev[i]) != hipSuccess) { g_prof_cap = i & ~1; return; }
      g_prof_cap = ncap;
    }
    g_prof_work += work;
    (void)hipEventRecord(g_prof_ev[g_prof_used], st);
  } else if (g_prof_used + 1 < g_prof_cap) {
    (void)hipEventRecord(g_prof_ev[g_prof_used + 1], st);
    g_prof_used += 2;
  }
}

int g_launch_log = 0;
namespace {
struct LaunchCount { const char* name; int64_t n; };
constexpr int kLaunchNames = 128;
LaunchCount g_launches[kLaunchNames];
int g_launch_names = 0;
}
void note_launch(const char* name) {
  for (int i = 0; i < g_launch_names; ++i)
    if (g_launches[i].name == name || strcmp(g_launches[i].name, name) == 0) { ++g_launches[i].n; return; }
  if (g_launch_names < kLaunchNames) g_launches[g_launch_names++] = LaunchCount{name, 1};
}

int adj_forward(const matcha_shape& s, const matcha_tensors& p, const matcha_frozen& f, const matcha_step_opts& o,
                const int64_t* x, int64_t T, float* node_out, float* recon_out, void* ws, size_t ws_bytes, hipStream_t st,
                const int32_t* t_dev, const int32_t* slot_map, float* fused_x0 = nullptr, float* fused_X = nullptr, bool save = false,
                bool fused_node = false);
int adj_backward(const matcha_shape& s, const matcha_tensors& p, const matcha_frozen& f, const matcha_step_opts& o,
                 const int64_t* x, int64_t T, float* dnode, const float* drecon, matcha_tensors& g, int32_t* touched,
                 void* ws, size_t ws_bytes, void* gemm_ws, size_t gemm_ws_bytes, hipStream_t st, const int32_t* slot_map, bool fused = false);
size_t adj_workspace_bytes(const matcha_shape& s, int64_t T);
bool adj_fused_eligible(const matcha_shape& s, const matcha_frozen& f);

struct Workspace {
  Ragged rg;
  float *x0, *X, *qin, *kin, *vin, *stats, *Q, *K, *V, *P, *O, *Y, *H1, *H2, *row_loss, *logits, *node;
  float *dH2, *dXs, *dZ1, *ddyn0, *dO, *dQ, *dK, *dV, *dqin, *dkin, *dvin, *dZ0, *dX0;
  float* slab;      size_t slab_bytes;
  float* gemm_ws;   size_t gemm_ws_bytes;
  void* adj_ws;     size_t adj_ws_bytes;
  float* folded;
  float* lwB; float* lwM; float* lwdB; float* lwdM;
  float* enc;
  float* enc_rec; size_t enc_rec_floats;
  float* merged;
  float* frag;
  float* fb_ws;
  float* tslab;
  float* tpart;
  float* tslab2;
  float* qkv;
  float* front_ws;
  void* tg_ws;      size_t tg_ws_bytes;
  float *XN, *x0N, *xhN, *GN; int64_t* node_ids; int32_t* node_cnt;
  float* RN;
  float* VN;
  size_t total;
};

struct OptionName { const char* name; int Options::*field; };
static const OptionName kOptionNames[] = {
    {"disable_fused", &Options::disable_fused}, {"disable_merged", &Options::disable_merged}, {"disable_small_batch", &Options::disable_small_batch},
    {"disable_wide_gemm", &Options::disable_wide_gemm}, {"disable_node_front", &Options::disable_node_front}, {"disable_node_r", &Options::disable_node_r}, {"disable_node_v", &Options::disable_node_v}, {"disable_node_dx", &Options::disable_node_dx}, {"debug_nan", &Options::debug_nan}, {"fused_dbg", &Options::fused_dbg}};
Options& options() {
  static Options o = [] {
    Options v;
    memset(&v, 0, sizeof(v));
    for (const OptionName& n : kOptionNames) {
      char env[64] = "MATCHA_";
      size_t k = strlen(env);
      for (const char* c = n.name; *c && k + 1 < sizeof(env); ++c) env[k++] = (char)((*c >= 'a' && *c <= 'z') ? *c - 32 : *c);
      env[k] = 0;
      const char* e = getenv(env);
      if (e) v.*(n.field) = (*e == 0) ? 1 : atoi(e);
      if (e && v.*(n.field) == 0 && strcmp(e, "0") != 0) v.*(n.field) = 1;
    }
    return v;
  }();
  return o;
}
static bool merged_layerwise_shape(const matcha_shape& s) { return s.d >= 128 && s.d % 64 == 0; }
static bool merged_layerwise(const matcha_shape& s) { return merged_layerwise_shape(s) && attn_wide_eligible(s.d) && !options().disable_merged; }
static bool enc128_enabled(const matcha_shape& s, const matcha_step_opts& o) { return enc128_shape(s.d) && merged_layerwise(s) && options().disable_fused != 1 && !o.deterministic && !o.sparse_table_grad; }
static bool fused_enabled(const matcha_shape& s) { return s.d == 64 && options().disable_fused != 1 && !options().disable_merged; }
static bool node_front_shape(const matcha_shape& s, int64_t B, int L) { return s.mode == 0 && s.d == 64 && front_bwd_supported(s.d, s.n_attr) && B * L + 1 >= 4 * ((int64_t)s.n_nodes + 1); }
static bool node_v_shape(const matcha_shape& s, int64_t B, int L) { return B * L + 1 >= 64 * ((int64_t)s.n_nodes + 1); }
static bool node_dx_shape(const matcha_shape& s, int64_t B, int L) { return node_v_shape(s, B, L); }
static bool has_target(int objective, const float* y, const float* w) { return objective == MATCHA_OBJECTIVE_SOFTPLUS_MSE ? y != nullptr : (y && w); }
static int check_objective(int32_t objective, const char* fn) {
  if (objective == MATCHA_OBJECTIVE_BCE || objective == MATCHA_OBJECTIVE_SOFTPLUS_MSE) return MATCHA_OK;
  set_error("%s: unknown objective %d (MATCHA_OBJECTIVE_BCE or MATCHA_OBJECTIVE_SOFTPLUS_MSE)", fn, (int)objective);
  return MATCHA_EINVAL;
}
struct StepRoute {
  bool compact;
  bool half_plan;
  bool fused;
  bool merged_layerwise, enc128;
  bool front, adj_fused;
  bool small;
  bool lif;
  bool split_tail, dx_zeroed;
  bool node;
  bool node_r, node_v;
  bool node_dx;
};
static std::mutex g_fwd_mu;
static std::unordered_map<const void*, std::pair<StepRoute, uint64_t>> g_fwd_state;
static uint64_t g_fwd_clock = 0;
static void note_forward(const void* ws, const StepRoute& route) {
  std::lock_guard<std::mutex> lk(g_fwd_mu);
  if (g_fwd_state.size() >= 4096 && g_fwd_state.find(ws) == g_fwd_state.end()) {
    auto old = g_fwd_state.begin();
    for (auto it = g_fwd_state.begin(); it != g_fwd_state.end(); ++it)
      if (it->second.second < old->second.second) old = it;
    g_fwd_state.erase(old);
  }
  g_fwd_state[ws] = std::make_pair(route, ++g_fwd_clock);
}
static bool recorded_route(const void* ws, StepRoute& route) {
  std::lock_guard<std::mutex> lk(g_fwd_mu);
  auto it = g_fwd_state.find(ws);
  if (it != g_fwd_state.end()) route = it->second.first;
  return it != g_fwd_state.end();
}
static void forget_forward(const void* ws) {
  std::lock_guard<std::mutex> lk(g_fwd_mu);
  g_fwd_state.erase(ws);
}

static int merged_weights(const matcha_shape& s, const matcha_tensors& p, Workspace& w, hipStream_t st) {
  const int64_t d = s.d, hd = (int64_t)MATCHA_N_HEAD * d;
  const BmmProduct pr[2] = {
      {p.w_k, 1, d, d * d, p.w_q, d, 1, d * d, w.lwB, d, d * d, 0},
      {p.fc1_w, hd, 1, d, p.w_v, d, 1, d * d, w.lwM, hd, d, 0}};
  return launch_bmm_heads(pr, 2, s.d, st);
}
static int merged_chain(const matcha_shape& s, const matcha_tensors& p, matcha_tensors& g_, Workspace& w, hipStream_t st) {
  const int64_t d = s.d, hd = (int64_t)MATCHA_N_HEAD * d;
  const BmmProduct pr[4] = {
      {p.w_k, d, 1, d * d, w.lwdB, d, 1, d * d, g_.w_q, d, d * d, 1},
      {p.w_q, d, 1, d * d, w.lwdB, 1, d, d * d, g_.w_k, d, d * d, 1},
      {w.lwdM, hd, 1, d, p.w_v, 1, d, d * d, g_.fc1_w, hd, d, 1},
      {p.fc1_w, 1, hd, d, w.lwdM, hd, 1, d, g_.w_v, d, d * d, 1}};
  return launch_bmm_heads(pr, 4, s.d, st);
}

static size_t carve(const matcha_shape& s, int64_t B, int L, char* base, Workspace& w, bool compact = false) {
  const int64_t Tn = B * L + 1, d = s.d, hd = (int64_t)MATCHA_N_HEAD * d;
  size_t off = 0;
  auto take_always = [&](size_t n_floats) {
    float* p = base ? (float*)(base + off) : nullptr;
    off += align_up(n_floats * sizeof(float), 256);
    return p;
  };
  auto take = [&](size_t n_floats) { return compact ? (float*)nullptr : take_always(n_floats); };
  {
    const size_t rb = ragged_bytes(B, L);
// ... 34 lines not shown
  w.adj_ws_bytes = (s.mode == 1) ? adj_workspace_bytes(s, Tn) : 0;
  w.adj_ws = take_always(w.adj_ws_bytes / sizeof(float));
  w.folded = take_always(s.d == 64 ? fused_fold_floats() : 0);
  w.frag = take_always(s.d == 64 ? fused_frag_floats() : 0);
  w.merged = take_always(s.d == 64 ? fused_merged_floats() : 0);
  {
    const size_t nm = merged_layerwise_shape(s) ? (size_t)hd * d : 0;
    w.lwB = take_always(nm); w.lwM = take_always(nm);
    w.lwdB = take(nm); w.lwdM = take(nm);
  }
  w.enc = take_always(enc128_shape((int)d) ? enc128_ws_floats() : 0);
  w.enc_rec = w.Q;
  w.enc_rec_floats = (w.Q && w.O) ? (size_t)((w.O + Tn * hd) - w.Q) : 0;
  w.fb_ws = take(s.d == 64 ? fused_bwd_ws_floats(B, L) : 0);
  w.tpart = take(s.d == 64 ? fused_tail_partial_floats() : 0);
  w.tslab = take(s.d == 64 ? fused_tail_slab32_floats(B, L) : 0);
  w.tslab2 = take(s.d == 64 ? tail_bwd_slab_floats() : 0);
  w.qkv = take(s.d == 64 ? fused_qkv_floats(B, L) : 0);
  w.front_ws = take(front_bwd_supported(s.d, s.n_attr) ? front_bwd_ws_floats() : 0);
  w.tg_ws_bytes = (s.mode == 0 && !compact) ? table_grad_ws_bytes(Tn, s.n_nodes) : 0;
  w.tg_ws = take(w.tg_ws_bytes / sizeof(float));
  {
    const size_t nn = node_front_shape(s, B, L) ? (size_t)(s.n_nodes + 1) : 0;
    w.XN = take_always(nn * 64); w.x0N = take(nn * 64); w.xhN = take(nn * 64); w.GN = take(nn * 64);
    w.node_ids = reinterpret_cast<int64_t*>(take_always(nn * 2));
    w.node_cnt = reinterpret_cast<int32_t*>(take_always(nn ? 64 : 0));
    w.RN = nn ? (compact ? take_always(node_r_floats((int64_t)nn)) : w.Q) : nullptr;
    w.VN = (nn && !compact && w.Q) ? w.Q + node_r_floats((int64_t)nn) : nullptr;
  }
  w.total = off;
  return off;
}

static bool compact_forward(const matcha_shape& s, const matcha_step_opts& o, bool force_layerwise) { return !force_layerwise && o.forward_only && fused_enabled(s); }
static StepRoute decide_route(const matcha_shape& s, const matcha_step_opts& o, int64_t B, int L, const Workspace& w, const matcha_frozen& f,
                              const float* y, const float* w_bce, int objective, bool force_layerwise, bool want_losses) {
  StepRoute r;
  r.compact = compact_forward(s, o, force_layerwise);
  r.fused = !force_layerwise && fused_enabled(s);
  r.merged_layerwise = merged_layerwise(s);
  r.enc128 = !force_layerwise && enc128_enabled(s, o) && (o.forward_only || enc128_rec_floats(w.rg) <= w.enc_rec_floats);
  r.half_plan = fused_enabled(s) || r.enc128;
  r.front = r.fused && front_bwd_supported(s.d, s.n_attr) && (options().disable_fused & 2) == 0;
  r.adj_fused = r.front && s.mode == 1 && adj_fused_eligible(s, f);
  r.small = r.fused && fused_small_batch(w.rg);
  const bool atomics = !o.deterministic && !o.sparse_table_grad;
  r.node = r.front && node_front_shape(s, B, L) && !r.small && atomics && !options().disable_node_front;
  r.node_r = r.node && !options().disable_node_r;
  r.node_v = r.node_r && !o.forward_only && w.VN && node_v_shape(s, B, L) && !options().disable_node_v;
  r.lif = r.fused && o.loss_in_forward && !o.forward_only && has_target(objective, y, w_bce);
  r.split_tail = r.lif && !r.small && (options().fused_dbg & 1) == 0;
  r.dx_zeroed = r.lif && atomics && (r.split_tail || r.small) && want_losses;
  r.node_dx = r.node_v && r.lif && r.split_tail && r.dx_zeroed && node_dx_shape(s, B, L) && !options().disable_node_dx;
  return r;
}
static NodeOperands node_operands(const StepRoute& r, const matcha_shape& s, const Workspace& w) {
  const int64_t rows = (int64_t)s.n_nodes + 1;
  return r.node ? NodeOperands{w.XN, w.rg.tok_key, w.xhN, r.node_r ? w.RN : nullptr, r.node_v ? w.VN : nullptr, rows} : NodeOperands{w.X, nullptr, nullptr, nullptr, nullptr, rows};
}

static int table_gradient(const matcha_shape& s, const matcha_step_opts& o, const Workspace& w, int64_t Tn, matcha_tensors& g, hipStream_t st) {
  if (o.sparse_table_grad) return MATCHA_OK;
  if (!o.deterministic) return MATCHA_OK;
  return launch_table_grad(w.rg.tok_key, w.dX0, Tn, s.d, s.n_nodes, g.table, w.tg_ws, w.tg_ws_bytes, st);
}

static int encoder_done(const matcha_step_opts& o, hipStream_t st) {
  if (o.encoder_done_event && hipEventRecord((hipEvent_t)o.encoder_done_event, st) != hipSuccess) {
    set_error("matcha_backward: recording encoder_done_event failed"); return MATCHA_EHIP;
  }
  return MATCHA_OK;
}

static int check_shape(const matcha_shape* s, int64_t B, int32_t L) {
  MATCHA_CHECK_ARG(s, "null shape");
  MATCHA_CHECK_ARG(s->d >= 8 && s->d <= 256 && s->d % 8 == 0 && (s->d <= 64 || s->d % 64 == 0),
                   "embed_dim d=%d unsupported (multiples of 8 up to 64, then 128, 192, 256)", s->d);
  MATCHA_CHECK_ARG(s->d % 4 == 0, "d must be a multiple of 4");
  MATCHA_CHECK_ARG(L >= 1 && L <= MATCHA_MAX_L, "L=%d outside 1..%d", L, MATCHA_MAX_L);
  MATCHA_CHECK_ARG(B >= 1 && B * (int64_t)L < (1ll << 31) - 2, "B=%lld must be >= 1 and B*L < 2^31", (long long)B);
  MATCHA_CHECK_ARG(s->d == 64 || B * (int64_t)L + 1 <= 65535ll * 128, "B*L=%lld exceeds the %lld token rows the layer-by-layer kernels (embed_dim != 64) launch",
                   (long long)(B * (int64_t)L), 65535ll * 128);
  MATCHA_CHECK_ARG(s->n_nodes >= 1, "n_nodes=%d must be >= 1", s->n_nodes);
  MATCHA_CHECK_ARG(s->mode == 0 || s->mode == 1, "mode=%d must be 0 (table) or 1 (adj)", s->mode);
  MATCHA_CHECK_ARG(s->n_attr >= 1 && (size_t)s->n_attr * s->d * 4 <= 160 * 1024, "n_attr=%d does not fit the LDS staging", s->n_attr);
  return MATCHA_OK;
}

static GemmArgs gemm1(const Workspace& w, const float* A, const float* B, float* C, int64_t M, int64_t N, int64_t K, bool b_kn) {
  GemmArgs g;
  memset(&g, 0, sizeof(g));
  g.A[0] = A; g.B[0] = B; g.C[0] = C; g.batch = 1;
  g.M = M; g.N = N; g.K = K; g.lda = K; g.ldb = b_kn ? N : K; g.ldc = N;
  g.aux_scale = 1.f;
  g.m_dev = w.rg.count;
  g.rng_row_map = w.rg.tok_slot;
  return g;
}

__global__ void nan_count_kernel(const float* __restrict__ p, const int32_t* __restrict__ rows_dev, int64_t rows, int64_t width, int* __restrict__ out) {
  if (rows_dev) rows = *rows_dev;
  int bad = 0;
  for (int64_t i = (int64_t)blockIdx.x * blockDim.x + threadIdx.x; i < rows * width; i += (int64_t)gridDim.x * blockDim.x)
    bad += isfinite(p[i]) ? 0 : 1;
  if (bad) atomicAdd(out, bad);
}
// ... 55 lines not shown
    if (hipEventElapsedTime(&t, g_prof_ev[i], g_prof_ev[i + 1]) != hipSuccess) { set_error("matcha_profile_read: elapsed failed"); return MATCHA_EHIP; }
    ms += t;
  }
  if (total_ms) *total_ms = ms;
  if (launches) *launches = g_prof_used / 2;
  if (work) *work = g_prof_work;
  g_prof_used = 0;
  g_prof_work = 0.0;
  return MATCHA_OK;
}

extern "C" size_t matcha_workspace_bytes(const matcha_shape* shp, int64_t B, int32_t L) {
  if (check_shape(shp, B, L) != MATCHA_OK) return 0;
  Workspace w;
  return carve(*shp, B, L, nullptr, w);
}

extern "C" size_t matcha_workspace_bytes_forward(const matcha_shape* shp, int64_t B, int32_t L) {
  if (check_shape(shp, B, L) != MATCHA_OK) return 0;
  Workspace w;
  return carve(*shp, B, L, nullptr, w, fused_enabled(*shp));
}

static int forward_impl(const matcha_shape* shp, const matcha_tensors* params, const matcha_frozen* frozen,
                        const matcha_step_opts* opts, const int64_t* x, int64_t B, int32_t L, const float* y,
                        const float* w_bce, float* logits, float* losses, void* ws, size_t ws_bytes,
                        matcha_stream_t stream, bool force_layerwise, bool stop_before_head, int objective) {
  MATCHA_TRY(check_shape(shp, B, L));
  MATCHA_CHECK_ARG(params && frozen && opts && x && ws, "matcha_forward: null pointer");
  MATCHA_CHECK_ARG(((uintptr_t)ws) % 256 == 0, "matcha_forward: workspace must be 256-byte aligned");
  const matcha_shape& s = *shp;
  const matcha_tensors& p = *params;
  hipStream_t st = (hipStream_t)stream;
  Workspace w;
  const size_t need = carve(s, B, L, (char*)ws, w, compact_forward(s, *opts, force_layerwise));
  if (ws_bytes < need) { set_error("matcha_forward: workspace %zu < %zu bytes", ws_bytes, need); return MATCHA_ENOMEM; }
  const int64_t Tn = B * L + 1;
  const int d = s.d;
  const int64_t hd = (int64_t)MATCHA_N_HEAD * d;
  const bool train = opts->training != 0;
  MATCHA_CHECK_ARG(!train || opts->seed || (opts->p_drop_adj <= 0 && opts->p_drop_fc1 <= 0 && opts->p_drop_pff <= 0),
                   "matcha_forward: training with dropout needs opts->seed");
  MATCHA_CHECK_ARG((frozen->attr_table || frozen->attr_mode == 1) && p.attr_w && p.attr_b && p.next_w && p.next_b && p.w_q && p.w_k && p.w_v && p.fc1_w &&
                       p.fc1_b && p.pff0_w && p.pff0_b && p.pff1_w && p.pff1_b && p.pff_ln_g && p.pff_ln_b && p.ln1_g && p.ln1_b &&
                       p.ln2_g && p.ln2_b && p.cls_w && p.cls_b && p.ln_q_g && p.ln_q_b && p.ln_k_g && p.ln_k_b && p.ln_v_g && p.ln_v_b,
                   "matcha_forward: a parameter pointer is null");
  const int32_t* cnt = w.rg.count;
  const int64_t* ids = w.rg.tok_id;

  const StepRoute route = decide_route(s, *opts, B, L, w, *frozen, y, w_bce, objective, force_layerwise, losses != nullptr);
  const bool keep = !opts->forward_only;
  const NodeOperands nx = node_operands(route, s, w);
  const bool tgt = has_target(objective, y, w_bce);
  MATCHA_TRY(launch_ragged_plan(x, B, L, s.n_nodes, opts->status, w.rg, st, route.half_plan ? 1 : 0, route.node ? w.node_ids : nullptr, route.node ? w.node_cnt : nullptr,
                                (route.node && keep) ? w.GN : nullptr));
  float* recon_out = losses ? losses + 1 : nullptr;
  const bool recon_zero_in_loss = s.mode == 0 && recon_out && route.fused && tgt;
  if (s.mode == 0) {
    MATCHA_CHECK_ARG(p.table, "matcha_forward: table mode without table");
    if (recon_out && !recon_zero_in_loss) MATCHA_TRY(zero_async(recon_out, 2 * sizeof(float), st));
  } else if (route.adj_fused) {
    MATCHA_TRY(adj_forward(s, p, *frozen, *opts, ids, Tn, nullptr, recon_out, w.adj_ws, w.adj_ws_bytes, st, cnt, w.rg.tok_slot, keep ? w.x0 : nullptr, w.X, keep));
  } else {
    MATCHA_TRY(adj_forward(s, p, *frozen, *opts, ids, Tn, w.node, recon_out, w.adj_ws, w.adj_ws_bytes, st, cnt, w.rg.tok_slot));
  }
  const bool prep_in_front = route.front && !route.adj_fused;
  if (prep_in_front) {
    const PrepSpec prep = {&p, w.folded, w.merged, w.frag};
    if (route.node) {
      MATCHA_TRY(launch_front_fwd(p, w.node_ids, p.table, nullptr, *frozen, s.n_attr, w.rg, nx.rows, keep ? w.x0N : nullptr, nx.X, st, &prep, w.node_cnt));
      if (keep) MATCHA_TRY(launch_node_xhat(nx.X, w.node_cnt, nx.rows, nx.xhat, st));
      if (nx.rn) MATCHA_TRY(launch_node_r(nx.X, w.frag, nx.rows, nx.rn, st, nx.vn));
    } else
    MATCHA_TRY(launch_front_fwd(p, ids, s.mode == 0 ? p.table : nullptr, s.mode == 0 ? nullptr : w.node, *frozen, s.n_attr, w.rg, Tn, keep ? w.x0 : nullptr, w.X, st, &prep));
  } else if (!route.adj_fused) {
    MATCHA_TRY(launch_embed_fwd(ids, Tn, d, s.mode == 0 ? p.table : nullptr, s.mode == 0 ? nullptr : w.node, *frozen, s.n_attr, p.attr_w, p.attr_b, w.x0, st, cnt));
    GemmArgs g = gemm1(w, w.x0, p.next_w, w.X, Tn, d, d, false);
    g.flags = MATCHA_EPI_BIAS | MATCHA_EPI_TANH; g.bias[0] = p.next_b;
    MATCHA_TRY(launch_gemm_rm(false, g, st));
  }
  if (keep) note_forward(ws, route); else forget_forward(ws);
  if (route.fused) {
    const bool save = keep && !route.lif;
    if (!prep_in_front) MATCHA_TRY(launch_prep_heads(p, w.folded, w.merged, w.frag, st));
    float* lg_out = (logits && !save) ? logits : w.logits;
    FusedFwdLaunch a;
    a.frag = w.frag; a.small = route.small; a.y = y; a.w = w_bce; a.objective = objective; a.logits = lg_out; a.row_loss = w.row_loss;
    a.x = nx;
    a.Y = keep ? w.Y : nullptr; a.H1 = keep ? w.H1 : nullptr; a.H2 = keep ? w.H2 : nullptr; a.rimg = keep ? w.qkv : nullptr;
    a.seed = opts->seed; a.p_fc1 = train ? opts->p_drop_fc1 : 0.f; a.p_pff = train ? opts->p_drop_pff : 0.f; a.alpha = opts->alpha;
    a.ddyn0 = route.lif ? w.ddyn0 : nullptr; a.dXs = w.dXs; a.tslab = w.tslab; a.tail_dh2 = route.split_tail ? w.dH2 : nullptr;
    a.dxs_node = route.node_dx ? w.GN : nullptr;
    MATCHA_CHECK_ARG(!route.node_dx || nx.rows <= Tn, "matcha_forward: the heads' per-node d x_hat rows do not fit dO");
    MATCHA_TRY(launch_fused_fwd32(p, w.rg, B, L, a, st));
    if (route.split_tail)
      MATCHA_TRY(launch_tail_bwd64(p, w.dH2, w.Y, w.H1, w.rg, opts->seed, a.p_fc1, a.p_pff, w.ddyn0, w.tslab2, w.tslab, route.dx_zeroed ? w.dO : nullptr,
                                   route.node_dx ? (int64_t)MATCHA_N_HEAD * nx.rows * 64 : 0, st, w.row_loss, B, tgt ? losses : nullptr, recon_zero_in_loss));
    const bool zero_in_loss = route.dx_zeroed && !route.split_tail;
    if (tgt && losses && !route.split_tail)
      MATCHA_TRY(launch_loss_reduce(w.row_loss, B, losses, st, recon_zero_in_loss, zero_in_loss ? w.dO : nullptr, zero_in_loss ? (size_t)Tn * 64 * sizeof(float) : 0));
    if (logits && lg_out != logits && hipMemcpyAsync(logits, w.logits, B * sizeof(float), hipMemcpyDeviceToDevice, st) != hipSuccess) {
      set_error("logits copy failed"); return MATCHA_EHIP;
    }
    return MATCHA_OK;
  }
  nan_check("x0", w.x0, cnt, 0, d, st);
  nan_check("X", w.X, cnt, 0, d, st);
  if (route.enc128) {
    MATCHA_TRY(merged_weights(s, p, w, st));
    MATCHA_TRY(launch_enc128_fwd(p, w.lwB, w.lwM, w.X, w.rg, B, L, w.Y, keep ? w.enc_rec : nullptr, w.enc, w.rg.tok_slot, opts->seed,
                                 (train && opts->p_drop_fc1 > 0.f) ? opts->p_drop_fc1 : 0.f, st));
  } else {
  MATCHA_TRY(launch_ln3_fwd(w.X, Tn, d, p.ln_q_g, p.ln_q_b, p.ln_k_g, p.ln_k_b, p.ln_v_g, p.ln_v_b, w.qin, w.kin, w.vin, w.stats, st, cnt));
  if (route.merged_layerwise) {
    MATCHA_TRY(merged_weights(s, p, w, st));
    GemmArgs g = gemm1(w, w.qin, w.lwB, w.Q, Tn, hd, d, false);
    MATCHA_TRY(launch_gemm_rm(false, g, st));
  } else {
    GemmArgs g = gemm1(w, w.qin, p.w_q, w.Q, Tn, hd, d, false);
    g.A[1] = w.kin; g.B[1] = p.w_k; g.C[1] = w.K;
    g.A[2] = w.vin; g.B[2] = p.w_v; g.C[2] = w.V;
    g.batch = 3;
    MATCHA_TRY(launch_gemm_rm(false, g, st));
  }
  nan_check("qin", w.qin, cnt, 0, d, st);
// ... 138 lines not shown
  hipStream_t st = (hipStream_t)stream;
  Workspace w;
  const size_t need = carve(s, B, L, (char*)ws, w);
  if (ws_bytes < need) { set_error("matcha_backward: workspace %zu < %zu bytes", ws_bytes, need); return MATCHA_ENOMEM; }
  const int64_t Tn = B * L + 1;
  const int d = s.d;
  const int64_t hd = (int64_t)MATCHA_N_HEAD * d;
  const bool train = opts->training != 0;
  const bool drop_fc1 = train && opts->p_drop_fc1 > 0.f, drop_pff = train && opts->p_drop_pff > 0.f;
  const int32_t* cnt = w.rg.count;
  const int64_t* ids = w.rg.tok_id;

  StepRoute route;
  MATCHA_CHECK_ARG(recorded_route(ws, route), "matcha_backward: no matcha_forward on record for this workspace (one backward per forward, same ws pointer)");
  MATCHA_CHECK_ARG(!route.fused || route.lif == (opts->loss_in_forward && has_target(objective, y, w_bce)),
                   "matcha_backward: loss_in_forward / targets differ from the forward's on this workspace");
  MATCHA_CHECK_ARG(!(route.lif && dlogits), "matcha_backward: opts->loss_in_forward excludes an explicit dlogits");
  forget_forward(ws);
  const bool tail_in_bwd = route.lif && (route.split_tail || route.small);
  const bool dx_zeroed = route.dx_zeroed && !opts->deterministic && !opts->sparse_table_grad;
  TailReduceArgs tail_args;
  const NodeOperands nx = node_operands(route, s, w);
  if (route.lif) {
    if (route.split_tail) tail_reduce_args(w.tslab2, w.rg, L, g_, true, tail_bwd_grid(), true, tail_args);
    else if (route.small) tail_reduce_args(w.tslab, w.rg, L, g_, true, -1, false, tail_args);
    else MATCHA_TRY(launch_tail_reduce(w.tslab, w.rg, L, g_, st, true, w.tpart));
  } else {
  HeadParams hp = {p.pff_ln_g, p.pff_ln_b, p.ln1_g, p.ln1_b, p.ln2_g, p.ln2_b, p.cls_w, p.cls_b};
  HeadParams ghp = {g_.pff_ln_g, g_.pff_ln_b, g_.ln1_g, g_.ln1_b, g_.ln2_g, g_.ln2_b, g_.cls_w, g_.cls_b};
  MATCHA_TRY(launch_head_bwd(w.rg.row_off, w.H2, nx.X, B, L, d, hp, y, w_bce, w.logits, dlogits, opts->alpha, w.dH2, w.dXs, w.slab, ghp, st, objective, nx.xrow));
  MATCHA_TRY(launch_gemm_tn(w.dH2, w.H1, g_.pff1_w, g_.pff1_b, d, d, Tn, d, d, nullptr, true, w.gemm_ws, w.gemm_ws_bytes, st, cnt));
  {
    GemmArgs g = gemm1(w, w.dH2, p.pff1_w, w.dZ1, Tn, d, d, true);
    g.flags = MATCHA_EPI_DTANH; g.aux = w.H1;
    if (drop_pff) { g.flags |= MATCHA_EPI_DROPOUT; g.seed = opts->seed; g.stream_id = kStreamDropPff; g.p_drop = opts->p_drop_pff; g.aux_scale = 1.f - opts->p_drop_pff; }
    MATCHA_TRY(launch_gemm_rm(true, g, st));
  }
  MATCHA_TRY(launch_gemm_tn(w.dZ1, w.Y, g_.pff0_w, g_.pff0_b, d, d, Tn, d, d, nullptr, true, w.gemm_ws, w.gemm_ws_bytes, st, cnt));
  {
    GemmArgs g = gemm1(w, w.dZ1, p.pff0_w, w.ddyn0, Tn, d, d, true);
    g.flags = MATCHA_EPI_RESIDUAL | MATCHA_EPI_ROWMASK; g.residual = w.dH2; g.row_ids = ids;
    if (drop_fc1) { g.flags |= MATCHA_EPI_DROPOUT; g.seed = opts->seed; g.stream_id = kStreamDropFc1; g.p_drop = opts->p_drop_fc1; }
    MATCHA_TRY(launch_gemm_rm(true, g, st));
  }
  }
  if (route.fused) {
    const bool dx_atomic = !opts->deterministic && !opts->sparse_table_grad;
    MATCHA_CHECK_ARG(!route.node || dx_atomic, "matcha_backward: deterministic / sparse_table_grad differ from the forward's on this workspace");
    FusedBwdLaunch a;
    a.folded = w.folded; a.merged = w.merged; a.x = nx; a.dDyn = w.ddyn0; a.dXs = w.dXs; a.rimg = w.qkv;
    a.dxh = w.dO; a.ws = w.fb_ws; a.dZ0 = route.front ? nullptr : w.dZ0;
    a.dx_atomic = dx_atomic; a.dx_zeroed = dx_zeroed; a.tail = tail_in_bwd ? &tail_args : nullptr;
    a.dx_node = route.node_dx;
    MATCHA_CHECK_ARG(!route.node_dx || (dx_zeroed && nx.rows <= Tn), "matcha_backward: the heads' per-node d x_hat rows do not fit dO");
    MATCHA_TRY(launch_fused_bwd_merged(p, w.rg, B, L, a, g_, st));
    MATCHA_TRY(encoder_done(*opts, st));
    if (route.front) {
      if (s.mode == 0) MATCHA_CHECK_ARG(g_.table, "matcha_backward: table mode without a table gradient buffer");
      if (route.node) {
        MATCHA_TRY(launch_node_scatter(nx.X, w.dO, fused_bwd_dxpad(w.fb_ws), w.dXs, w.rg, Tn, w.GN, st, route.node_dx ? w.node_cnt : nullptr, nx.rows));
        MATCHA_TRY(launch_front_bwd(p, nx.X, nullptr, 1, nx.rows, fused_bwd_dxpad(w.fb_ws), w.GN, w.x0N, w.node_ids, *frozen, s.n_attr, w.rg, nullptr, g_.table, w.front_ws, g_, st, touched, w.node_cnt));
        return MATCHA_OK;
      }
      const bool rows_out = s.mode == 1 || opts->deterministic || opts->sparse_table_grad;
      MATCHA_TRY(launch_front_bwd(p, w.X, w.dO, dx_atomic ? 1 : MATCHA_N_HEAD, Tn, fused_bwd_dxpad(w.fb_ws), w.dXs, w.x0, ids, *frozen, s.n_attr, w.rg,
                                  rows_out ? w.dX0 : nullptr, rows_out ? nullptr : g_.table, w.front_ws, g_, st, s.mode == 0 ? touched : nullptr));
      if (s.mode == 0) MATCHA_TRY(table_gradient(s, *opts, w, Tn, g_, st));
      else MATCHA_TRY(adj_backward(s, p, *frozen, *opts, ids, Tn, w.dX0, drecon, g_, touched, w.adj_ws, w.adj_ws_bytes, w.gemm_ws, w.gemm_ws_bytes, st, w.rg.tok_slot, route.adj_fused));
      return MATCHA_OK;
    }
  } else {
  if (route.enc128) {
    MATCHA_TRY(launch_enc128_bwd(p, w.lwB, w.lwM, w.X, w.ddyn0, w.dXs, w.rg, B, L, w.dqin, w.enc_rec, w.enc, w.lwdB, w.lwdM, g_, w.dZ0, st));
    MATCHA_TRY(merged_chain(s, p, g_, w, st));
    MATCHA_TRY(encoder_done(*opts, st));
  } else {
  if (route.merged_layerwise) {
    MATCHA_TRY(zero_async(w.lwdM, (size_t)hd * d * sizeof(float), st));
    MATCHA_TRY(zero_async(w.lwdB, (size_t)hd * d * sizeof(float), st));
    MATCHA_TRY(launch_gemm_tn(w.ddyn0, w.O, w.lwdM, g_.fc1_b, d, hd, Tn, d, hd, nullptr, true, w.gemm_ws, w.gemm_ws_bytes, st, cnt));
    {
      GemmArgs g = gemm1(w, w.ddyn0, w.lwM, w.dO, Tn, hd, d, true);
      MATCHA_TRY(launch_gemm_rm(true, g, st));
    }
    MATCHA_TRY(launch_attn_bwd(w.Q, w.kin, w.vin, w.P, w.dO, w.rg.row_off, B, L, d, w.dQ, w.dK, w.dV, w.slab, st, true, w.dkin, w.dvin));
    MATCHA_TRY(launch_gemm_tn(w.dQ, w.qin, w.lwdB, nullptr, hd, d, Tn, hd, d, nullptr, true, w.gemm_ws, w.gemm_ws_bytes, st, cnt));
    {
      GemmArgs g = gemm1(w, w.dQ, w.lwB, w.dqin, Tn, d, hd, true);
      MATCHA_TRY(launch_gemm_rm(true, g, st));
    }
    MATCHA_TRY(merged_chain(s, p, g_, w, st));
  } else {
  MATCHA_TRY(launch_gemm_tn(w.ddyn0, w.O, g_.fc1_w, g_.fc1_b, d, hd, Tn, d, hd, nullptr, true, w.gemm_ws, w.gemm_ws_bytes, st, cnt));
  {
    GemmArgs g = gemm1(w, w.ddyn0, p.fc1_w, w.dO, Tn, hd, d, true);
    MATCHA_TRY(launch_gemm_rm(true, g, st));
  }
  MATCHA_TRY(launch_attn_bwd(w.Q, w.K, w.V, w.P, w.dO, w.rg.row_off, B, L, d, w.dQ, w.dK, w.dV, w.slab, st));
  MATCHA_TRY(launch_gemm_tn(w.dQ, w.qin, g_.w_q, nullptr, hd, d, Tn, hd, d, nullptr, true, w.gemm_ws, w.gemm_ws_bytes, st, cnt));
  MATCHA_TRY(launch_gemm_tn(w.dK, w.kin, g_.w_k, nullptr, hd, d, Tn, hd, d, nullptr, true, w.gemm_ws, w.gemm_ws_bytes, st, cnt));
  MATCHA_TRY(launch_gemm_tn(w.dV, w.vin, g_.w_v, nullptr, hd, d, Tn, hd, d, nullptr, true, w.gemm_ws, w.gemm_ws_bytes, st, cnt));
  {
    GemmArgs g = gemm1(w, w.dQ, p.w_q, w.dqin, Tn, d, hd, true);
    g.A[1] = w.dK; g.B[1] = p.w_k; g.C[1] = w.dkin;
    g.A[2] = w.dV; g.B[2] = p.w_v; g.C[2] = w.dvin;
    g.batch = 3;
    MATCHA_TRY(launch_gemm_rm(true, g, st));
  }
  }
  MATCHA_TRY(launch_ln3_bwd(w.X, w.dqin, w.dkin, w.dvin, w.dXs, Tn, d, p.ln_q_g, p.ln_k_g, p.ln_v_g, w.dZ0, w.slab, g_.ln_q_g,
                            g_.ln_q_b, g_.ln_k_g, g_.ln_k_b, g_.ln_v_g, g_.ln_v_b, st, cnt));
  MATCHA_TRY(encoder_done(*opts, st));
  }
// ... 54 lines not shown
```

### matcha_amd/csrc/ragged.hip

```cpp
#include "kernels.hpp"

namespace matcha {

constexpr int kRpt = 1;
constexpr int kRowsPerBlock = 256 * kRpt;

__device__ __forceinline__ int block_exclusive_scan_256(int v, int* lds4, int* total) {
  const int lane = threadIdx.x & 63, wave = threadIdx.x >> 6;
  int incl = v;
#pragma unroll
  for (int o = 1; o < 64; o <<= 1) {
    const int u = __shfl_up(incl, o, 64);
    if (lane >= o) incl += u;
  }
  if (lane == 63) lds4[wave] = incl;
  __syncthreads();
  int base = 0;
  for (int w = 0; w < wave; ++w) base += lds4[w];
  if (total) *total = lds4[0] + lds4[1] + lds4[2] + lds4[3];
  return base + incl - v;
}

__global__ __launch_bounds__(256) void row_count_kernel(const int64_t* __restrict__ x, int64_t B, int L, int32_t* __restrict__ blk_sum) {
  __shared__ int lds4[4];
  const int64_t b0 = (int64_t)blockIdx.x * kRowsPerBlock + threadIdx.x * kRpt;
  int cnt = 0;
  for (int i = 0; i < kRpt; ++i)
    if (b0 + i < B)
      for (int l = 0; l < L; ++l) cnt += x[(b0 + i) * L + l] != 0 ? 1 : 0;
  int total;
  (void)block_exclusive_scan_256(cnt, lds4, &total);
  if (threadIdx.x == 0) blk_sum[blockIdx.x] = total;
}

__global__ __launch_bounds__(1024) void row_scan_kernel(int32_t* __restrict__ blk_sum, int nblk, int32_t* __restrict__ count,
                                                        int32_t* __restrict__ sb_first, int nsb, int32_t n_rows) {
  __shared__ int part[1024];
  for (int i = threadIdx.x; i <= nsb; i += 1024) sb_first[i] = n_rows;
  const int chunk = (nblk + 1023) / 1024;
  const int b0 = threadIdx.x * chunk, b1 = (b0 + chunk < nblk) ? b0 + chunk : nblk;
  int local = 0;
  for (int b = b0; b < b1; ++b) local += blk_sum[b];
  __shared__ int wtot[16];
  const int lane = threadIdx.x & 63, wave = threadIdx.x >> 6;
  int incl = local;
#pragma unroll
  for (int o = 1; o < 64; o <<= 1) {
    const int u = __shfl_up(incl, o, 64);
    if (lane >= o) incl += u;
  }
  if (lane == 63) wtot[wave] = incl;
  __syncthreads();
  int wbase = 0, total = 0;
// ... 33 lines not shown
  for (int i = 0; i < kRpt; ++i) {
    int k = 0;
#pragma unroll
    for (int l = 0; l < MATCHA_MAX_L; ++l) {
      v[i][l] = (b0 + i < B && l < L) ? v[i][l] : 0;
      k += v[i][l] != 0 ? 1 : 0;
    }
    kk[i] = k;
    cnt += k;
  }
  int kprev = 0;
#pragma unroll
  for (int l = 0; l < MATCHA_MAX_L; ++l) kprev += (b0 > 0 && l < L && vp[l] != 0) ? 1 : 0;
  int pos = blk_base[blockIdx.x] + block_exclusive_scan_256(cnt, lds4, nullptr);
#pragma unroll
  for (int i = 0; i < kRpt; ++i) {
    const int64_t b = b0 + i;
    if (b < B) {
      row_off[b] = pos;
      const int k = kk[i];
      if (b == 0 || pos / super_tok != (pos - kprev) / super_tok) sb_first[pos / super_tok] = (int32_t)b;
      kprev = k;
      int nth = 0;
#pragma unroll
      for (int l = 0; l < MATCHA_MAX_L; ++l) {
        int64_t id = v[i][l];
        if (id != 0) {
          if (id < 0 || id > n_nodes) {
            if (status) atomicOr(status, MATCHA_STATUS_BAD_ID);
            id = 0;
          }
          tok_slot[pos] = (int32_t)(b * L + l); tok_id[pos] = id; tok_key[pos] = (int32_t)id; tok_pos[pos] = nth | (k << 8); ++pos; ++nth;
        }
      }
    }
  }
  const int tr = count[1];
  if (blockIdx.x == 0 && threadIdx.x == 0) {
    row_off[B] = tr;
    tok_slot[tr] = (int32_t)(B * L);
    tok_id[tr] = 0;
    tok_pos[tr] = 0;
  }
  for (int64_t i = tr + (int64_t)blockIdx.x * 256 + threadIdx.x; i < B * L + 1; i += (int64_t)gridDim.x * 256) tok_key[i] = 0;
  if (node_ids) {
    for (int64_t i = (int64_t)blockIdx.x * 256 + threadIdx.x; i <= n_nodes; i += (int64_t)gridDim.x * 256) node_ids[i] = i;
    if (blockIdx.x == 0 && threadIdx.x == 0) { node_cnt[0] = (int32_t)(n_nodes + 1); node_cnt[1] = (int32_t)n_nodes; }
  }
  if (node_zero)
    for (int64_t i = (int64_t)blockIdx.x * 256 + threadIdx.x; i < (n_nodes + 1) * 16; i += (int64_t)gridDim.x * 256)
      reinterpret_cast<float4*>(node_zero)[i] = make_float4(0.f, 0.f, 0.f, 0.f);
}

constexpr int kFullTok = 63;
constexpr int kHalfTok = 31;
constexpr int kSuperTok = 63 * 32;

__device__ __forceinline__ int tile_pack_wave(const int32_t* __restrict__ row_off, int64_t B, int nsb, int s, bool half, int cap_per_sb,
                                              const int32_t* __restrict__ sb_first, int4* __restrict__ out, int lane) {
  const int kTileTok = half ? kHalfTok : kFullTok;
  const int b_lo = sb_first[s];
  int b_hi = (int)B;
  for (int q = s + 1; q < nsb; ++q)
    if (sb_first[q] < (int)B) { b_hi = sb_first[q]; break; }
  int nt = 0;
  if (b_lo < b_hi) {
    int tile_b0 = b_lo;
    int tile_tok0 = __builtin_amdgcn_readfirstlane(row_off[b_lo]);
    for (int base = b_lo; base < b_hi; base += 64) {
      const int idx = base + lane;
      const bool valid = idx < b_hi;
      const int so = valid ? row_off[idx] : 0;
      const int eo = valid ? row_off[idx + 1] : 0;
      for (;;) {
        const uint64_t over = __ballot(valid && eo - tile_tok0 > kTileTok);
        if (over == 0) break;
        const int i = __ffsll((long long)over) - 1;
        const int start = __builtin_amdgcn_readlane(so, i);
        if (lane == 0 && nt < cap_per_sb) out[nt] = make_int4(tile_tok0, start - tile_tok0, tile_b0, base + i - tile_b0);
        ++nt;
        tile_b0 = base + i;
        tile_tok0 = start;
      }
    }
    const int end = __builtin_amdgcn_readfirstlane(row_off[b_hi]);
    if (lane == 0 && nt < cap_per_sb) out[nt] = make_int4(tile_tok0, end - tile_tok0, tile_b0, b_hi - tile_b0);
    ++nt;
  }
  return nt < cap_per_sb ? nt : cap_per_sb;
}

__global__ __launch_bounds__(64) void tile_pack_kernel(const int32_t* __restrict__ row_off, int64_t B, int nsb, int cap_per_sb0, int cap_per_sb1,
                                                       const int32_t* __restrict__ sb_first, int32_t* __restrict__ sb_tiles0,
                                                       int32_t* __restrict__ sb_cnt0, int32_t* __restrict__ sb_tiles1, int32_t* __restrict__ sb_cnt1, int y0) {
  const int s = blockIdx.x, lane = threadIdx.x;
  const bool half = (int)blockIdx.y + y0 != 0;
  const int cap_per_sb = half ? cap_per_sb1 : cap_per_sb0;
  int32_t* sb_tiles = half ? sb_tiles1 : sb_tiles0;
  int32_t* sb_cnt = half ? sb_cnt1 : sb_cnt0;
  const int nt = tile_pack_wave(row_off, B, nsb, s, half, cap_per_sb, sb_first, reinterpret_cast<int4*>(sb_tiles) + (int64_t)s * cap_per_sb, lane);
  if (lane == 0) sb_cnt[s] = nt;
}

struct CompactArgs {
  const int32_t* sb_tiles[2]; int32_t* sb_cnt[2]; int cap_per_sb[2]; int ntiles_cap[2]; int32_t* meta[2];
};
__global__ __launch_bounds__(1024) void tile_compact_kernel(CompactArgs a, int nsb, int32_t* __restrict__ count, int x0) {
  const int which = (int)blockIdx.x + x0;
  if (x0 != 0 && threadIdx.x == 0) count[2] = 0;
  const int32_t* __restrict__ sb_tiles = a.sb_tiles[which];
  int32_t* __restrict__ sb_cnt = a.sb_cnt[which];
  const int cap_per_sb = a.cap_per_sb[which], ntiles_cap = a.ntiles_cap[which];
  int32_t* __restrict__ meta = a.meta[which];
  __shared__ int wtot[16];
  __shared__ int carry;
  if (threadIdx.x == 0) carry = 0;
  __syncthreads();
  const int lane = threadIdx.x & 63, wave = threadIdx.x >> 6;
  for (int base = 0; base < nsb; base += 1024) {
    const int i = base + threadIdx.x;
    const int c = i < nsb ? sb_cnt[i] : 0;
    int incl = c;
#pragma unroll
    for (int o = 1; o < 64; o <<= 1) {
      const int u = __shfl_up(incl, o, 64);
      if (lane >= o) incl += u;
    }
    if (lane == 63) wtot[wave] = incl;
    __syncthreads();
    int wbase = 0, tot = 0;
#pragma unroll
    for (int w2 = 0; w2 < 16; ++w2) { const int v = wtot[w2]; if (w2 < wave) wbase += v; tot += v; }
    if (i < nsb) sb_cnt[i] = carry + wbase + incl - c;
    __syncthreads();
    if (threadIdx.x == 0) carry += tot;
    __syncthreads();
  }
  const int total = carry < ntiles_cap ? carry : ntiles_cap;
  if (threadIdx.x == 0) count[2 + which] = total;
  __syncthreads();
  const int4* __restrict__ src = reinterpret_cast<const int4*>(sb_tiles);
  int4* __restrict__ dst = reinterpret_cast<int4*>(meta);
  __shared__ int offs[1025];
  if (nsb <= 1024) {
    for (int i = threadIdx.x; i < nsb; i += 1024) offs[i] = sb_cnt[i];
    if (threadIdx.x == 0) offs[nsb] = total;
    __syncthreads();
    for (int i0 = threadIdx.x; i0 < total; i0 += 4 * 1024) {
      int4 v[4];
#pragma unroll
      for (int u = 0; u < 4; ++u) {
        const int i = i0 + u * 1024 < total ? i0 + u * 1024 : total - 1;
        int lo = 0, hi = nsb;
        while (hi - lo > 1) { const int mid = (lo + hi) >> 1; if (offs[mid] <= i) lo = mid; else hi = mid; }
        v[u] = src[(int64_t)lo * cap_per_sb + (i - offs[lo])];
      }
#pragma unroll
      for (int u = 0; u < 4; ++u)
        if (i0 + u * 1024 < total) dst[i0 + u * 1024] = v[u];
    }
// ... 130 lines not shown
static inline int halves_cap(int64_t T, int L) { return (int)cdiv(T + 1, 32 - L) + super_blocks(T); }

int ragged_tiles_cap(int64_t B, int L) { return tiles_cap(B * L, L); }
int ragged_halves_cap(int64_t B, int L) { return halves_cap(B * L, L); }

size_t ragged_bytes(int64_t B, int L) {
  const int64_t T = B * L;
  size_t n = 0;
  n += align_up((size_t)(B + 1) * 4, 256);
  n += align_up((size_t)(T + 1) * 4, 256);
  n += align_up((size_t)(T + 1) * 8, 256);
  n += 256;
  n += align_up((size_t)cdiv(B, kRowsPerBlock) * 4, 256);
  n += align_up((size_t)(T + 1) * 4, 256);
  n += align_up((size_t)(T + 1) * 4, 256);
  n += align_up((size_t)(tiles_cap(T, L) + 2) * 16, 256);
  n += align_up((size_t)super_blocks(T) * super_cap(L) * 16, 256);
  n += align_up((size_t)super_blocks(T) * 4, 256);
  n += align_up((size_t)(super_blocks(T) + 1) * 4, 256);
  n += align_up((size_t)(halves_cap(T, L) + 2) * 16, 256);
  n += align_up((size_t)super_blocks(T) * super_hcap(L) * 16, 256);
  n += align_up((size_t)super_blocks(T) * 4, 256);
  n += align_up((size_t)(T + 1) * 4, 256);
  return n;
}

void ragged_carve(int64_t B, int L, char* base, Ragged& r) {
  const int64_t T = B * L;
  size_t off = 0;
  auto take = [&](size_t bytes) { char* p = base + off; off += align_up(bytes, 256); return p; };
  r.row_off = (int32_t*)take((size_t)(B + 1) * 4);
  r.tok_slot = (int32_t*)take((size_t)(T + 1) * 4);
  r.tok_id = (int64_t*)take((size_t)(T + 1) * 8);
  r.count = (int32_t*)take(256);
  r.blk_sum = (int32_t*)take((size_t)cdiv(B, kRowsPerBlock) * 4);
  r.nblk = (int)cdiv(B, kRowsPerBlock);
  r.ntiles = tiles_cap(T, L);
  r.tok_pos = (int32_t*)take((size_t)(T + 1) * 4);
  r.tok_key = (int32_t*)take((size_t)(T + 1) * 4);
  r.tile_meta = (int32_t*)take((size_t)(r.ntiles + 2) * 16);
  r.nsb = super_blocks(T);
  r.sb_cap = super_cap(L);
  r.sb_tiles = (int32_t*)take((size_t)r.nsb * r.sb_cap * 16);
  r.sb_cnt = (int32_t*)take((size_t)r.nsb * 4);
  r.sb_first = (int32_t*)take((size_t)(r.nsb + 1) * 4);
  r.nhalves = halves_cap(T, L);
  r.sb_hcap = super_hcap(L);
  r.half_meta = (int32_t*)take((size_t)(r.nhalves + 2) * 16);
  r.sb_htiles = (int32_t*)take((size_t)r.nsb * r.sb_hcap * 16);
  r.sb_hcnt = (int32_t*)take((size_t)r.nsb * 4);
  r.tok_tile = (int32_t*)take((size_t)(T + 1) * 4);
}

int launch_ragged_plan(const int64_t* x, int64_t B, int L, int64_t n_nodes, int32_t* status, const Ragged& r, hipStream_t st, int level,
                       int64_t* node_ids, int32_t* node_cnt, float* node_zero) {
  if (B <= kSmallRows && r.nsb <= kSmallSb && !options().disable_small_batch) {
    PlanSmallArgs a;
    a.x = x; a.B = B; a.L = L; a.n_nodes = n_nodes; a.status = status;
    a.row_off = r.row_off; a.tok_slot = r.tok_slot; a.tok_id = r.tok_id; a.tok_pos = r.tok_pos; a.tok_key = r.tok_key; a.count = r.count; a.sb_first = r.sb_first;
    a.nsb = r.nsb; a.level = level;
    a.sb_tiles[0] = r.sb_tiles; a.cap_per_sb[0] = r.sb_cap; a.ntiles_cap[0] = r.ntiles; a.meta[0] = r.tile_meta;
    a.sb_tiles[1] = r.sb_htiles; a.cap_per_sb[1] = r.sb_hcap; a.ntiles_cap[1] = r.nhalves; a.meta[1] = r.half_meta;
    a.tok_tile = r.tok_tile;
    a.node_ids = node_ids; a.node_cnt = node_cnt; a.node_zero = node_zero;
    hipLaunchKernelGGL(plan_small_kernel, dim3(1), dim3(1024), 0, st, a);
    MATCHA_CHECK_LAUNCH("plan_small_kernel");
    return MATCHA_OK;
  }
  hipLaunchKernelGGL(row_count_kernel, dim3(r.nblk), dim3(256), 0, st, x, B, L, r.blk_sum);
  MATCHA_CHECK_LAUNCH("row_count_kernel");
  hipLaunchKernelGGL(row_scan_kernel, dim3(1), dim3(1024), 0, st, r.blk_sum, r.nblk, r.count, r.sb_first, r.nsb, (int32_t)B);
  MATCHA_CHECK_LAUNCH("row_scan_kernel");
  hipLaunchKernelGGL(row_fill_kernel, dim3(r.nblk), dim3(256), 0, st, x, B, L, r.blk_sum, r.count, r.row_off, r.tok_slot, r.tok_id, r.tok_pos, r.sb_first, kSuperTok,
                     r.tok_key, n_nodes, status, node_ids, node_cnt, node_zero);
  MATCHA_CHECK_LAUNCH("row_fill_kernel");
  if (level <= 0) return MATCHA_OK;
  const int first = level >= 2 ? 0 : 1;
  hipLaunchKernelGGL(tile_pack_kernel, dim3(r.nsb, 2 - first), dim3(64), 0, st, r.row_off, B, r.nsb, r.sb_cap, r.sb_hcap, r.sb_first, r.sb_tiles, r.sb_cnt,
                     r.sb_htiles, r.sb_hcnt, first);
  MATCHA_CHECK_LAUNCH("tile_pack_kernel");
  CompactArgs ca;
  ca.sb_tiles[0] = r.sb_tiles; ca.sb_cnt[0] = r.sb_cnt; ca.cap_per_sb[0] = r.sb_cap; ca.ntiles_cap[0] = r.ntiles; ca.meta[0] = r.tile_meta;
  ca.sb_tiles[1] = r.sb_htiles; ca.sb_cnt[1] = r.sb_hcnt; ca.cap_per_sb[1] = r.sb_hcap; ca.ntiles_cap[1] = r.nhalves; ca.meta[1] = r.half_meta;
  hipLaunchKernelGGL(tile_compact_kernel, dim3(2 - first), dim3(1024), 0, st, ca, r.nsb, r.count, first);
  MATCHA_CHECK_LAUNCH("tile_compact_kernel");
  if (level >= 2) {
    hipLaunchKernelGGL(tok_tile_kernel, dim3(r.ntiles), dim3(64), 0, st, r.tile_meta, r.tok_tile);
    MATCHA_CHECK_LAUNCH("tok_tile_kernel");
  }
  return MATCHA_OK;
}

}

using namespace matcha;

extern "C" size_t matcha_ragged_plan_bytes(int64_t B, int32_t L) {
  if (B < 1 || L < 1 || L > MATCHA_MAX_L || B * (int64_t)L >= (1ll << 31) - 2) return 0;
  return ragged_bytes(B, L);
}

extern "C" int matcha_ragged_plan(const int64_t* x, int64_t B, int32_t L, int32_t n_nodes, int32_t* status, void* ws, size_t ws_bytes,
                                  matcha_ragged_view* view, matcha_stream_t stream) {
  MATCHA_CHECK_ARG(x && ws && view, "matcha_ragged_plan: null pointer");
  MATCHA_CHECK_ARG(B >= 1 && L >= 1 && L <= MATCHA_MAX_L && B * (int64_t)L < (1ll << 31) - 2, "matcha_ragged_plan: B=%lld L=%d", (long long)B, L);
  MATCHA_CHECK_ARG(n_nodes >= 1, "matcha_ragged_plan: n_nodes=%d", n_nodes);
  MATCHA_CHECK_ARG(((uintptr_t)ws) % 256 == 0, "matcha_ragged_plan: workspace must be 256-byte aligned");
  if (ws_bytes < ragged_bytes(B, L)) { set_error("matcha_ragged_plan: workspace %zu < %zu bytes", ws_bytes, ragged_bytes(B, L)); return MATCHA_ENOMEM; }
  Ragged r;
  ragged_carve(B, L, (char*)ws, r);
  view->row_off = r.row_off; view->tok_slot = r.tok_slot; view->tok_id = r.tok_id; view->tok_key = r.tok_key; view->tok_pos = r.tok_pos;
  view->count = r.count; view->tile_meta = r.tile_meta; view->tiles_cap = r.ntiles;
  view->half_meta = r.half_meta; view->halves_cap = r.nhalves; view->tok_tile = r.tok_tile;
  return launch_ragged_plan(x, B, L, n_nodes, status, r, (hipStream_t)stream, 2);
}
```

Measured before the change: 57.59 million hyperedges/s.

## Host ragged-plan tile packing and backward unfold reductions inside existing kernel launches

Moves the ragged plan's tile_pack work into extra blocks of the front-end forward kernel when spare slots exist, and defers the tile_compact step. It also folds the fb_unfold second-stage vector reductions into extra blocks of node_scatter, and lets fbm_chain write its outputs to LDS so the unfold can pair with it. The aim is fewer small kernel launches and less serialization on the stream. The cost is more complex grid accounting, and extra role blocks that can compete with the main blocks for slots.

```diff
diff --git a/matcha_amd/csrc/fb_unfold.hpp b/matcha_amd/csrc/fb_unfold.hpp
--- /dev/null
+++ b/matcha_amd/csrc/fb_unfold.hpp
@@ -0,0 +1,90 @@
+#pragma once
+#include "kernels.hpp"
+
+namespace matcha {
+
+constexpr int kWgSlab = 4 * 4096 + 6 * 64;
+constexpr int kVecOff = 4 * 4096;
+constexpr float kEpsLn = 1e-5f;
+
+__device__ __forceinline__ void ln_row16(const float4& v, float& mean, float& rstd) {
+  const float s = group_sum<16>((v.x + v.y) + (v.z + v.w));
+  mean = s * (1.f / 64.f);
+  const float a = v.x - mean, b = v.y - mean, c = v.z - mean, e = v.w - mean;
+  const float q = group_sum<16>((a * a + b * b) + (c * c + e * e));
+  rstd = __builtin_amdgcn_rsqf(q * (1.f / 64.f) + kEpsLn);
+}
+
+struct UnfoldArgs {
+  const float* wslab; int nchunks;
+  const float* X; const int32_t* count; int x_pad_row0;
+  const float* W[3]; const float* g[3]; const float* b[3];
+  float* gW[3]; float* gfc1;
+  float* part;
+};
+__device__ __forceinline__ void fb_unfold_rows(const UnfoldArgs& a, int slice, int mat, int head, float4 s, float dc, float dpad, float (*red)[3][64]) {
+  const int tid = threadIdx.x, rl = tid >> 4, c4 = (tid & 15) * 4;
+  const int row = slice * 16 + rl;
+  if (mat == 3) {
+    float4* o = reinterpret_cast<float4*>(a.gfc1 + (int64_t)row * 512 + head * 64 + c4);
+    float4 v = *o;
+    v.x += s.x; v.y += s.y; v.z += s.z; v.w += s.w;
+    *o = v;
+    return;
+  }
+  const float4 xv = *reinterpret_cast<const float4*>(a.X + (a.x_pad_row0 ? (int64_t)0 : (int64_t)a.count[1] * 64) + c4);
+  float m, rs;
+  ln_row16(xv, m, rs);
+  s.x += dpad * (xv.x - m) * rs; s.y += dpad * (xv.y - m) * rs; s.z += dpad * (xv.z - m) * rs; s.w += dpad * (xv.w - m) * rs;
+  dc += dpad;
+  const int64_t wi = ((int64_t)head * 64 + row) * 64 + c4;
+  const float4 W = *reinterpret_cast<const float4*>(a.W[mat] + wi);
+  const float4 G = *reinterpret_cast<const float4*>(a.g[mat] + c4), Bv = *reinterpret_cast<const float4*>(a.b[mat] + c4);
+  {
+    float4* o = reinterpret_cast<float4*>(a.gW[mat] + wi);
+    float4 v = *o;
+    v.x += s.x * G.x + dc * Bv.x; v.y += s.y * G.y + dc * Bv.y; v.z += s.z * G.z + dc * Bv.z; v.w += s.w * G.w + dc * Bv.w;
+    *o = v;
+  }
+  *reinterpret_cast<float4*>(&red[rl][0][c4]) = make_float4(s.x * W.x, s.y * W.y, s.z * W.z, s.w * W.w);
+  *reinterpret_cast<float4*>(&red[rl][1][c4]) = make_float4(dc * W.x, dc * W.y, dc * W.z, dc * W.w);
+  *reinterpret_cast<float4*>(&red[rl][2][c4]) = make_float4(dpad * W.x * G.x, dpad * W.y * G.y, dpad * W.z * G.z, dpad * W.w * G.w);
+  __syncthreads();
+  if (tid < 192) {
+    const int which = tid >> 6, k = tid & 63;
+    float t = 0.f;
+#pragma unroll
+    for (int q = 0; q < 16; ++q) t += red[q][which][k];
+    a.part[(((int64_t)(head * 4 + slice) * 3 + mat) * 3 + which) * 64 + k] = t;
+  }
+}
+
+struct Unfold2Args {
+  const float* part; const float* wslab; int nchunks;
+  float* dg[3]; float* db[3]; float* dfc1_b; float* dxpad;
+  int dxpad_add;
+};
+__device__ __forceinline__ void fb_unfold2_vec(const Unfold2Args& a, int vec, int k) {
+  float s = 0.f;
+  if (vec < 6) {
+    const int mat = vec >> 1, which = vec & 1;
+#pragma unroll 16
+    for (int p = 0; p < 32; ++p) s += a.part[(((int64_t)p * 3 + mat) * 3 + which) * 64 + k];
+    float* o = (which == 0 ? a.dg[mat] : a.db[mat]) + k;
+    *o += s;
+  } else if (vec == 6) {
+    if (a.dxpad_add == 2) return;
+#pragma unroll 8
+    for (int p = 0; p < 32; ++p) s += a.part[(((int64_t)p * 3 + 1) * 3 + 2) * 64 + k] + a.part[(((int64_t)p * 3 + 2) * 3 + 2) * 64 + k];
+    a.dxpad[k] = a.dxpad_add ? a.dxpad[k] + s : s;
+  } else {
+    for (int c = 0; c < a.nchunks; ++c) s += a.wslab[(int64_t)c * kWgSlab + kVecOff + 320 + k];
+    a.dfc1_b[k] += s;
+  }
+}
+constexpr int kUnfold2RoleBlocks = 2;
+__device__ __forceinline__ void fb_unfold2_role(const Unfold2Args& a, int role_block) {
+  fb_unfold2_vec(a, role_block * 4 + ((int)threadIdx.x >> 6), (int)threadIdx.x & 63);
+}
+
+}
diff --git a/matcha_amd/csrc/front_fused.hip b/matcha_amd/csrc/front_fused.hip
--- a/matcha_amd/csrc/front_fused.hip
+++ b/matcha_amd/csrc/front_fused.hip
@@ -3,6 +3,8 @@
 #include "attr_src.hpp"
 #include "kernels.hpp"
 #include "prep_heads.hpp"
+#include "fb_unfold.hpp"
+#include "ragged_roles.hpp"
 
 namespace matcha {
 
@@ -193,11 +195,17 @@
   float* x0; float* X;
   int nprep; PrepArgs prep;
   int prep_walks;
+  int npack; TilePackArgs pack;
 };
 
 __global__ __launch_bounds__(256, 3) void front_fwd_kernel(FrontFwdArgs g) {
   extern __shared__ __attribute__((aligned(16))) float lds[];
   const int nprep = g.nprep;
+  const int nblk = (int)gridDim.x - g.npack;
+  if ((int)blockIdx.x >= nblk) {
+    tile_pack_role(g.pack, ((int)blockIdx.x - nblk) * 4 + ((int)threadIdx.x >> 6), (int)threadIdx.x & 63);
+    return;
+  }
   if ((int)blockIdx.x < nprep) {
     const int b = blockIdx.x;
     prep_heads_role(g.prep, b % kPrepGridX, (b / kPrepGridX) % kPrepGridY, b / (kPrepGridX * kPrepGridY), lds);
@@ -205,7 +213,7 @@
     __syncthreads();
   }
   const int nlate = g.prep_walks ? nprep : 0;
-  const int vb = (int)blockIdx.x - (nprep - nlate), Gf = (int)gridDim.x - (nprep - nlate);
+  const int vb = (int)blockIdx.x - (nprep - nlate), Gf = nblk - (nprep - nlate);
   float* Es = lds;
   float* As = lds + kTile;
   float* Xs = As + 64 * kLdA;
@@ -358,6 +366,11 @@
   const int nprep = g.nprep;
   const int tid = threadIdx.x, lane = tid & 63, wave = tid >> 6;
   bool late = false;
+  const int nblk = (int)gridDim.x - g.npack;
+  if ((int)blockIdx.x >= nblk) {
+    tile_pack_role(g.pack, ((int)blockIdx.x - nblk) * 4 + wave, lane);
+    return;
+  }
   if ((int)blockIdx.x < nprep) {
     const int b = blockIdx.x;
     prep_heads_role(g.prep, b % kPrepGridX, (b / kPrepGridX) % kPrepGridY, b / (kPrepGridX * kPrepGridY), lds);
@@ -391,7 +404,7 @@
   const int T = g.count[0];
   const int64_t t_last = (int64_t)T - 1;
   const int ngroups = (T + 15) / 16;
-  const int W = (int)gridDim.x * 4, Wn_ = W - nprep * 4;
+  const int W = nblk * 4, Wn_ = W - nprep * 4;
   const int r0 = g.prep_walks > 0 ? g.prep_walks - 1 : 0x3FFFFF;
   const int wv = late ? (int)blockIdx.x * 4 + wave : ((int)blockIdx.x - nprep) * 4 + wave;
   const float scale = g.attr.scale;
@@ -478,6 +491,8 @@
   const float* XN; const float* dxh; const float* dxpad; const float* dXs; const int32_t* key; const int32_t* count;
   float* G;
   const int32_t* ncount; int64_t rows;
+  int node_blocks;
+  Unfold2Args unfold2;
 };
 __device__ __forceinline__ void node_finish(const NodeScatterArgs& g) {
   const int64_t row = (int64_t)blockIdx.x * 16 + (threadIdx.x >> 4);
@@ -509,6 +524,7 @@
         make_float4(rs * (d.x - ma - xh.x * mb) + s.x, rs * (d.y - ma - xh.y * mb) + s.y, rs * (d.z - ma - xh.z * mb) + s.z, rs * (d.w - ma - xh.w * mb) + s.w);
 }
 __global__ __launch_bounds__(256) void node_scatter_kernel(NodeScatterArgs g) {
+  if ((int)blockIdx.x >= g.node_blocks) { fb_unfold2_role(g.unfold2, (int)blockIdx.x - g.node_blocks); return; }
   if (g.ncount) { node_finish(g); return; }
   __shared__ __attribute__((aligned(16))) float rows_s[2][16 * 64];
   __shared__ int keys_s[2][16];
@@ -517,7 +533,7 @@
   const int T = g.count[0];
   const int ntrips = (T + 15) / 16;
   const float4 dxp = *reinterpret_cast<const float4*>(g.dxpad + sc4);
-  const int stride = (int)gridDim.x;
+  const int stride = g.node_blocks;
   auto tok_of = [&](int trip) { const int64_t t = (int64_t)trip * 16 + srow; return t < T ? t : (int64_t)T - 1; };
   int kn = g.key[tok_of(blockIdx.x)], knn = g.key[tok_of(blockIdx.x + stride < ntrips ? blockIdx.x + stride : blockIdx.x)];
   float4 xn, dn, sn;
@@ -605,7 +621,7 @@
 }
 
 int launch_front_fwd(const matcha_tensors& p, const int64_t* ids, const float* table, const float* dense, const matcha_frozen& f, int n_attr,
-                     const Ragged& rg, int64_t tcap, float* x0, float* X, hipStream_t st, const PrepSpec* prep, const int32_t* count) {
+                     const Ragged& rg, int64_t tcap, float* x0, float* X, hipStream_t st, const PrepSpec* prep, const int32_t* count, const TilePackArgs* pack) {
   MATCHA_CHECK_ARG(f.attr_table, "front end: attr_table is required (also under attr_mode 1)");
   FrontFwdArgs g;
   const bool computed = f.attr_mode == 1 && f.attr_bounds && n_attr <= kAttrCols;
@@ -625,6 +641,14 @@
   g.prep_walks = (g.nprep > 0 && max_tiles + g.nprep > slots) ? 1 : 0;
   int64_t grid = g.prep_walks ? slots : g.nprep + (max_tiles < slots ? max_tiles : slots);
   if (grid < g.nprep + 1) grid = g.nprep + 1;
+  g.npack = 0;
+  memset(&g.pack, 0, sizeof(g.pack));
+  const int pack_blocks = pack ? (int)cdiv(pack->ntasks, 4) : 0;
+  auto host_pack = [&](int64_t own_blocks, int64_t chip_slots) {
+    if (!pack) return MATCHA_OK;
+    if (own_blocks + pack_blocks <= chip_slots) { g.npack = pack_blocks; g.pack = *pack; return MATCHA_OK; }
+    return launch_tile_pack(*pack, st);
+  };
   ProfScope ps(MATCHA_PROF_FRONT_FWD, (double)tcap * (8.0 + 256.0 + (computed ? 0.0 : 4.0 * n_attr) + (x0 ? 512.0 : 256.0)), st);
   if (computed) {
     const int slots4 = front_grid() * 2;
@@ -633,12 +657,16 @@
     g.prep_walks = (g.nprep > 0 && rounds >= 4) ? 3 : 0;
     int64_t grid3 = g.prep_walks ? slots4 : g.nprep + (cdiv(ngroups, 4) < slots4 ? cdiv(ngroups, 4) : slots4);
     if (grid3 < g.nprep + 1) grid3 = g.nprep + 1;
+    MATCHA_TRY(host_pack(grid3, slots4));
+    grid3 += g.npack;
     const size_t lds3 = (size_t)kF3Lds * sizeof(float);
     static_assert(kF3Lds >= kPrepLdsFloats, "the weight-form role needs its LDS inside the front end's");
     if (x0) hipLaunchKernelGGL(front_fwd3_kernel<true>, dim3((unsigned)grid3), dim3(256), lds3, st, g);
     else hipLaunchKernelGGL(front_fwd3_kernel<false>, dim3((unsigned)grid3), dim3(256), lds3, st, g);
     MATCHA_CHECK_LAUNCH("front_fwd3_kernel");
   } else {
+    MATCHA_TRY(host_pack(grid, slots));
+    grid += g.npack;
     hipLaunchKernelGGL(front_fwd_kernel, dim3((unsigned)grid), dim3(256), lds, st, g);
     MATCHA_CHECK_LAUNCH("front_fwd_kernel");
   }
@@ -653,21 +681,26 @@
 }
 
 int launch_node_scatter(const float* XN, const float* dxh, const float* dxpad, const float* dXs, const Ragged& rg, int64_t tcap, float* G, hipStream_t st,
-                        const int32_t* node_count, int64_t rows) {
+                        const int32_t* node_count, int64_t rows, const Unfold2Args* unfold2) {
   NodeScatterArgs g;
+  MATCHA_CHECK_ARG(!unfold2 || unfold2->dxpad_add == 2, "node_scatter: the launch hosts fb_unfold2's vectors only with dxpad final");
+  g.node_blocks = node_count ? (int)cdiv(rows, 16) : 0;
+  if (unfold2) g.unfold2 = *unfold2; else memset(&g.unfold2, 0, sizeof(g.unfold2));
   g.XN = XN; g.dxh = dxh; g.dxpad = dxpad; g.dXs = dXs; g.key = rg.tok_key; g.count = rg.count; g.G = G; g.ncount = node_count; g.rows = rows;
   if (node_count) {
     MATCHA_CHECK_ARG(rows > 0, "node_scatter: the per-node finisher needs the table's row count");
     ProfScope ps(MATCHA_PROF_FRONT_BWD, (double)rows * (MATCHA_N_HEAD + 3.0) * 256.0, st);
-    hipLaunchKernelGGL(node_scatter_kernel, dim3((unsigned)cdiv(rows, 16)), dim3(256), 0, st, g);
+    hipLaunchKernelGGL(node_scatter_kernel, dim3((unsigned)(g.node_blocks + (unfold2 ? kUnfold2RoleBlocks : 0))), dim3(256), 0, st, g);
     MATCHA_CHECK_LAUNCH("node_scatter_kernel");
     return MATCHA_OK;
   }
   int64_t grid = (int64_t)front_grid() * 4;
   const int64_t trips = cdiv(tcap, 16);
   if (grid > trips) grid = trips;
+  if (unfold2 && grid > 4 * kUnfold2RoleBlocks) grid -= kUnfold2RoleBlocks;
+  g.node_blocks = (int)grid;
   ProfScope ps(MATCHA_PROF_FRONT_BWD, (double)tcap * (4.0 * 256.0 + 4.0), st);
-  hipLaunchKernelGGL(node_scatter_kernel, dim3((unsigned)grid), dim3(256), 0, st, g);
+  hipLaunchKernelGGL(node_scatter_kernel, dim3((unsigned)(grid + (unfold2 ? kUnfold2RoleBlocks : 0))), dim3(256), 0, st, g);
   MATCHA_CHECK_LAUNCH("node_scatter_kernel");
   return MATCHA_OK;
 }
diff --git a/matcha_amd/csrc/fused_bwd.hip b/matcha_amd/csrc/fused_bwd.hip
--- a/matcha_amd/csrc/fused_bwd.hip
+++ b/matcha_amd/csrc/fused_bwd.hip
@@ -4,6 +4,7 @@
 #include "bf16x3.hpp"
 #include "kernels.hpp"
 #include "tail_reduce.hpp"
+#include "fb_unfold.hpp"
 
 namespace matcha {
 
@@ -12,9 +13,6 @@
 namespace {
 
 constexpr int kLd = 68;
-constexpr float kEpsLn = 1e-5f;
-constexpr int kWgSlab = 4 * 4096 + 6 * 64;
-constexpr int kVecOff = 4 * 4096;
 constexpr int kMaxChunks = 64;
 
 #define ZR8(p)                                                                                           \
@@ -22,14 +20,6 @@
     *reinterpret_cast<float4*>(p) = make_float4(0.f, 0.f, 0.f, 0.f);                                     \
     *reinterpret_cast<float4*>((p) + 4) = make_float4(0.f, 0.f, 0.f, 0.f);                               \
   } while (0)
-
-__device__ __forceinline__ void ln_row16(const float4& v, float& mean, float& rstd) {
-  const float s = group_sum<16>((v.x + v.y) + (v.z + v.w));
-  mean = s * (1.f / 64.f);
-  const float a = v.x - mean, b = v.y - mean, c = v.z - mean, e = v.w - mean;
-  const float q = group_sum<16>((a * a + b * b) + (c * c + e * e));
-  rstd = __builtin_amdgcn_rsqf(q * (1.f / 64.f) + kEpsLn);
-}
 
 
 #define FB_PIN(addr, x) asm volatile("" : "+v"(addr), "+v"((x).a), "+v"((x).b), "+v"((x).c), "+v"((x).d))
@@ -687,7 +677,7 @@
 }
 __device__ __forceinline__ void mm64_slice(const float* __restrict__ A, int a_rs, int a_cs, const float* __restrict__ B, int b_rs, int b_cs,
                                            const float* __restrict__ u, const float* __restrict__ v, float* __restrict__ out, int slice,
-                                           float* __restrict__ As, float* __restrict__ Bs) {
+                                           float* __restrict__ As, float* __restrict__ Bs, bool lds_out = false) {
   const int tid = threadIdx.x;
   {
     float av[4], bv[16];
@@ -707,15 +697,30 @@
   for (int kk = 0; kk < 16; ++kk) acc = MFMA16(As[c16 * 65 + 4 * kk + kq], Bs[(4 * kk + kq) * 65 + 16 * wave + c16], acc);
   const int j = 16 * wave + c16;
   const float vj = u ? v[j] : 0.f;
+  if (lds_out) __syncthreads();
 #pragma unroll
   for (int reg = 0; reg < 4; ++reg) {
     const int i = 4 * kq + reg;
-    out[(16 * slice + i) * 64 + j] = acc[reg] + (u ? u[16 * slice + i] * vj : 0.f);
-  }
-}
-__global__ __launch_bounds__(256) void fbm_chain_kernel(ChainArgs a) {
+    const float o = acc[reg] + (u ? u[16 * slice + i] * vj : 0.f);
+    if (lds_out) As[i * 65 + j] = o; else out[(16 * slice + i) * 64 + j] = o;
+  }
+}
+__device__ __forceinline__ float chain_dcq(const float* __restrict__ Wk, const float* __restrict__ db, int m) {
+  float s0 = 0.f, s1 = 0.f;
+#pragma unroll 8
+  for (int x = 0; x < 64; x += 2) { s0 += Wk[m * 64 + x] * db[x]; s1 += Wk[m * 64 + x + 1] * db[x + 1]; }
+  return s0 + s1;
+}
+__device__ __forceinline__ float chain_dcv(const float* __restrict__ Wf, const float* __restrict__ dbdyn, int m) {
+  float t0 = 0.f, t1 = 0.f;
+#pragma unroll 8
+  for (int x = 0; x < 64; x += 2) { t0 += Wf[x * 512 + m] * dbdyn[x]; t1 += Wf[(x + 1) * 512 + m] * dbdyn[x + 1]; }
+  return t0 + t1;
+}
+__global__ __launch_bounds__(256) void fbm_chain_kernel(ChainArgs a, UnfoldArgs uf, int paired, int dxpad_final) {
   __shared__ float As[16 * 65];
   __shared__ float Bs[64 * 65];
+  static_assert(sizeof(float) * 64 * 65 >= sizeof(float) * 16 * 3 * 64, "the un-folding's partials live in Bs");
   const int slice = blockIdx.x, job = blockIdx.y, head = blockIdx.z, tid = threadIdx.x;
   const float* red = a.red + (int64_t)head * kWgSlabM;
   const float* dB = red; const float* dM = red + 4096; const float* db = red + kVecOffM;
@@ -723,23 +728,18 @@
   const float* Wq = a.wq + (int64_t)head * 4096; const float* Wk = a.wk + (int64_t)head * 4096; const float* Wv = a.wv + (int64_t)head * 4096;
   const float* Wf = a.fc1_w + head * 64;
   float* out = a.out + (int64_t)head * kWgSlab;
+  const bool lds_out = paired != 0;
   if (job == 0) {
-    mm64_slice(Wk, 64, 1, dB, 64, 1, nullptr, nullptr, out + 0 * 4096, slice, As, Bs);
+    mm64_slice(Wk, 64, 1, dB, 64, 1, nullptr, nullptr, out + 0 * 4096, slice, As, Bs, lds_out);
   } else if (job == 1) {
-    mm64_slice(Wq, 64, 1, dB, 1, 64, a.cq + head * 64, db, out + 1 * 4096, slice, As, Bs);
+    mm64_slice(Wq, 64, 1, dB, 1, 64, a.cq + head * 64, db, out + 1 * 4096, slice, As, Bs, lds_out);
   } else if (job == 2) {
-    mm64_slice(Wf, 1, 512, dM, 64, 1, nullptr, nullptr, out + 2 * 4096, slice, As, Bs);
+    mm64_slice(Wf, 1, 512, dM, 64, 1, nullptr, nullptr, out + 2 * 4096, slice, As, Bs, lds_out);
   } else {
-    mm64_slice(dM, 64, 1, Wv, 1, 64, dbdyn, a.cv + head * 64, out + 3 * 4096, slice, As, Bs);
+    mm64_slice(dM, 64, 1, Wv, 1, 64, dbdyn, a.cv + head * 64, out + 3 * 4096, slice, As, Bs, lds_out);
   }
   if (slice == 0 && job == 0 && tid < 64) {
-    float s0 = 0.f, s1 = 0.f, t0 = 0.f, t1 = 0.f;
-#pragma unroll 8
-    for (int x = 0; x < 64; x += 2) {
-      s0 += Wk[tid * 64 + x] * db[x]; s1 += Wk[tid * 64 + x + 1] * db[x + 1];
-      t0 += Wf[x * 512 + tid] * dbdyn[x]; t1 += Wf[(x + 1) * 512 + tid] * dbdyn[x + 1];
-    }
-    const float s = s0 + s1, t = t0 + t1;
+    const float s = chain_dcq(Wk, db, tid), t = chain_dcv(Wf, dbdyn, tid);
     out[kVecOff + tid] = s;
     out[kVecOff + 64 + tid] = 0.f;
     out[kVecOff + 128 + tid] = t;
@@ -748,18 +748,22 @@
     if (head == 0) {
       float p = 0.f;
       for (int hh = 0; hh < MATCHA_N_HEAD; ++hh) p += a.red[(int64_t)hh * kWgSlabM + kVecOffM + 128 + tid];
-      a.dxpad[tid] = p;
-    }
-  }
-}
-
-struct UnfoldArgs {
-  const float* wslab; int nchunks;
-  const float* X; const int32_t* count; int x_pad_row0;
-  const float* W[3]; const float* g[3]; const float* b[3];
-  float* gW[3]; float* gfc1;
-  float* part;
-};
+      a.dxpad[tid] = dxpad_final ? p + 0.f : p;
+    }
+  }
+  if (!paired) return;
+  const int rl = tid >> 4, c4 = (tid & 15) * 4, row = slice * 16 + rl;
+  float dc = 0.f, dpad = 0.f;
+  if (job == 0) dc += chain_dcq(Wk, db, row);
+  else if (job == 1) dc += 0.f;
+  else if (job == 2) dc += chain_dcv(Wf, dbdyn, row);
+  if (job == 1 || job == 2) dpad += 0.f;
+  __syncthreads();
+  float4 s;
+  s.x = 0.f + As[rl * 65 + c4]; s.y = 0.f + As[rl * 65 + c4 + 1]; s.z = 0.f + As[rl * 65 + c4 + 2]; s.w = 0.f + As[rl * 65 + c4 + 3];
+  fb_unfold_rows(uf, slice, job, head, s, dc, dpad, reinterpret_cast<float (*)[3][64]>(Bs));
+}
+
 __global__ __launch_bounds__(256) void fb_unfold_kernel(UnfoldArgs a) {
   __shared__ float red[16][3][64];
   const int slice = blockIdx.x, mat = blockIdx.y, head = blockIdx.z;
@@ -786,66 +790,18 @@
     s.x = (t0.x + t1.x) + (t2.x + t3.x); s.y = (t0.y + t1.y) + (t2.y + t3.y);
     s.z = (t0.z + t1.z) + (t2.z + t3.z); s.w = (t0.w + t1.w) + (t2.w + t3.w);
   }
-  if (mat == 3) {
-    float4* o = reinterpret_cast<float4*>(a.gfc1 + (int64_t)row * 512 + head * 64 + c4);
-    float4 v = *o;
-    v.x += s.x; v.y += s.y; v.z += s.z; v.w += s.w;
-    *o = v;
-    return;
-  }
   float dc = 0.f, dpad = 0.f;
-  for (int c = 0; c < a.nchunks; ++c) {
-    const float* vb = base + (int64_t)c * kWgSlab + kVecOff;
-    dc += vb[mat * 64 + row];
-    if (mat > 0) dpad += vb[192 + (mat - 1) * 64 + row];
-  }
-  const float4 xv = *reinterpret_cast<const float4*>(a.X + (a.x_pad_row0 ? (int64_t)0 : (int64_t)a.count[1] * 64) + c4);
-  float m, rs;
-  ln_row16(xv, m, rs);
-  s.x += dpad * (xv.x - m) * rs; s.y += dpad * (xv.y - m) * rs; s.z += dpad * (xv.z - m) * rs; s.w += dpad * (xv.w - m) * rs;
-  dc += dpad;
-  const int64_t wi = ((int64_t)head * 64 + row) * 64 + c4;
-  const float4 W = *reinterpret_cast<const float4*>(a.W[mat] + wi);
-  const float4 G = *reinterpret_cast<const float4*>(a.g[mat] + c4), Bv = *reinterpret_cast<const float4*>(a.b[mat] + c4);
-  {
-    float4* o = reinterpret_cast<float4*>(a.gW[mat] + wi);
-    float4 v = *o;
-    v.x += s.x * G.x + dc * Bv.x; v.y += s.y * G.y + dc * Bv.y; v.z += s.z * G.z + dc * Bv.z; v.w += s.w * G.w + dc * Bv.w;
-    *o = v;
-  }
-  *reinterpret_cast<float4*>(&red[rl][0][c4]) = make_float4(s.x * W.x, s.y * W.y, s.z * W.z, s.w * W.w);
-  *reinterpret_cast<float4*>(&red[rl][1][c4]) = make_float4(dc * W.x, dc * W.y, dc * W.z, dc * W.w);
-  *reinterpret_cast<float4*>(&red[rl][2][c4]) = make_float4(dpad * W.x * G.x, dpad * W.y * G.y, dpad * W.z * G.z, dpad * W.w * G.w);
-  __syncthreads();
-  if (tid < 192) {
-    const int which = tid >> 6, k = tid & 63;
-    float t = 0.f;
-#pragma unroll
-    for (int q = 0; q < 16; ++q) t += red[q][which][k];
-    a.part[(((int64_t)(head * 4 + slice) * 3 + mat) * 3 + which) * 64 + k] = t;
-  }
-}
-
-struct Unfold2Args {
-  const float* part; const float* wslab; int nchunks;
-  float* dg[3]; float* db[3]; float* dfc1_b; float* dxpad;
-  int dxpad_add;
-};
+  if (mat < 3)
+    for (int c = 0; c < a.nchunks; ++c) {
+      const float* vb = base + (int64_t)c * kWgSlab + kVecOff;
+      dc += vb[mat * 64 + row];
+      if (mat > 0) dpad += vb[192 + (mat - 1) * 64 + row];
+    }
+  fb_unfold_rows(a, slice, mat, head, s, dc, dpad, red);
+}
+
 __global__ __launch_bounds__(512) void fb_unfold2_kernel(Unfold2Args a) {
-  const int vec = threadIdx.x >> 6, k = threadIdx.x & 63;
-  float s = 0.f;
-  if (vec < 6) {
-    const int mat = vec >> 1, which = vec & 1;
-    for (int p = 0; p < 32; ++p) s += a.part[(((int64_t)p * 3 + mat) * 3 + which) * 64 + k];
-    float* o = (which == 0 ? a.dg[mat] : a.db[mat]) + k;
-    *o += s;
-  } else if (vec == 6) {
-    for (int p = 0; p < 32; ++p) s += a.part[(((int64_t)p * 3 + 1) * 3 + 2) * 64 + k] + a.part[(((int64_t)p * 3 + 2) * 3 + 2) * 64 + k];
-    a.dxpad[k] = a.dxpad_add ? a.dxpad[k] + s : s;
-  } else {
-    for (int c = 0; c < a.nchunks; ++c) s += a.wslab[(int64_t)c * kWgSlab + kVecOff + 320 + k];
-    a.dfc1_b[k] += s;
-  }
+  fb_unfold2_vec(a, threadIdx.x >> 6, threadIdx.x & 63);
 }
 
 __global__ __launch_bounds__(256) void lnhat_bwd_kernel(const float* __restrict__ X, const float* __restrict__ dxh, int64_t tcap,
@@ -944,26 +900,31 @@
     const int tail_blocks = a.tail ? kTailRoleBlocks : 0;
     hipLaunchKernelGGL(fbm_reduce_kernel, dim3((unsigned)(kFbmReduceBlocks + tail_blocks)), dim3(256), 0, st, c, tl, tail_blocks);
     MATCHA_CHECK_LAUNCH("fbm_reduce_kernel");
-    hipLaunchKernelGGL(fbm_chain_kernel, dim3(4, 4, MATCHA_N_HEAD), dim3(256), 0, st, c);
+    UnfoldArgs u;
+    u.wslab = chain; u.nchunks = 1; u.X = X; u.count = rg.count; u.x_pad_row0 = xrow ? 1 : 0;
+    u.W[0] = p.w_q; u.W[1] = p.w_k; u.W[2] = p.w_v;
+    u.g[0] = p.ln_q_g; u.g[1] = p.ln_k_g; u.g[2] = p.ln_v_g;
+    u.b[0] = p.ln_q_b; u.b[1] = p.ln_k_b; u.b[2] = p.ln_v_b;
+    u.gW[0] = grads.w_q; u.gW[1] = grads.w_k; u.gW[2] = grads.w_v; u.gfc1 = grads.fc1_w;
+    u.part = part;
+    MATCHA_CHECK_ARG(!a.unfold2 || a.paired, "fused backward: handing the final vectors on belongs to the paired launches");
+    hipLaunchKernelGGL(fbm_chain_kernel, dim3(4, 4, MATCHA_N_HEAD), dim3(256), 0, st, c, u, a.paired ? 1 : 0, a.unfold2 ? 1 : 0);
     MATCHA_CHECK_LAUNCH("fbm_chain_kernel");
-  }
-  {
-    UnfoldArgs a;
-    a.wslab = chain; a.nchunks = 1; a.X = X; a.count = rg.count; a.x_pad_row0 = xrow ? 1 : 0;
-    a.W[0] = p.w_q; a.W[1] = p.w_k; a.W[2] = p.w_v;
-    a.g[0] = p.ln_q_g; a.g[1] = p.ln_k_g; a.g[2] = p.ln_v_g;
-    a.b[0] = p.ln_q_b; a.b[1] = p.ln_k_b; a.b[2] = p.ln_v_b;
-    a.gW[0] = grads.w_q; a.gW[1] = grads.w_k; a.gW[2] = grads.w_v; a.gfc1 = grads.fc1_w;
-    a.part = part;
-    hipLaunchKernelGGL(fb_unfold_kernel, dim3(4, 4, MATCHA_N_HEAD), dim3(256), 0, st, a);
-    MATCHA_CHECK_LAUNCH("fb_unfold_kernel");
+    if (!a.paired) {
+      hipLaunchKernelGGL(fb_unfold_kernel, dim3(4, 4, MATCHA_N_HEAD), dim3(256), 0, st, u);
+      MATCHA_CHECK_LAUNCH("fb_unfold_kernel");
+    }
     Unfold2Args b;
     b.part = part; b.wslab = chain; b.nchunks = 1;
     b.dg[0] = grads.ln_q_g; b.dg[1] = grads.ln_k_g; b.dg[2] = grads.ln_v_g;
     b.db[0] = grads.ln_q_b; b.db[1] = grads.ln_k_b; b.db[2] = grads.ln_v_b;
-    b.dfc1_b = grads.fc1_b; b.dxpad = dxpad; b.dxpad_add = 1;
-    hipLaunchKernelGGL(fb_unfold2_kernel, dim3(1), dim3(512), 0, st, b);
-    MATCHA_CHECK_LAUNCH("fb_unfold2_kernel");
+    b.dfc1_b = grads.fc1_b; b.dxpad = dxpad; b.dxpad_add = a.unfold2 ? 2 : 1;
+    if (a.unfold2) {
+      *a.unfold2 = b;
+    } else {
+      hipLaunchKernelGGL(fb_unfold2_kernel, dim3(1), dim3(512), 0, st, b);
+      MATCHA_CHECK_LAUNCH("fb_unfold2_kernel");
+    }
   }
   if (float* dZ0 = a.dZ0) {
     MATCHA_CHECK_ARG(!xrow, "fused backward: the node route has no dZ0 output");
diff --git a/matcha_amd/csrc/fused_fwd32.hip b/matcha_amd/csrc/fused_fwd32.hip
--- a/matcha_amd/csrc/fused_fwd32.hip
+++ b/matcha_amd/csrc/fused_fwd32.hip
@@ -1,5 +1,6 @@
 #include "kernels.hpp"
 #include "prep_heads.hpp"
+#include "ragged_roles.hpp"
 
 #ifndef F32_ABL
 #define F32_ABL 0
@@ -582,11 +583,17 @@
 #endif
 }
 
-struct NodeRArgs { const float* X; const u32x4* wfrag; float* rn; int rows; float* vn; };
+struct NodeRArgs { const float* X; const u32x4* wfrag; float* rn; int rows; float* vn; int ncompact; CompactArgs compact; };
 __global__ __launch_bounds__(64) void node_r_kernel(NodeRArgs g) {
   const int lane = threadIdx.x, r = lane & 31, h = lane >> 5;
-  const int hd = blockIdx.y & 7;
-  const bool vrole = blockIdx.y >= MATCHA_N_HEAD;
+  if ((int)blockIdx.y < g.ncompact) {
+    __shared__ int offs[kCompactRoleSb + 1];
+    tile_compact_role(g.compact, (int)blockIdx.x, (int)gridDim.x, lane, offs);
+    return;
+  }
+  const int by = (int)blockIdx.y - g.ncompact;
+  const int hd = by & 7;
+  const bool vrole = by >= MATCHA_N_HEAD;
   const int row = (int)blockIdx.x * 32 + r;
   const bool live = row < g.rows;
   const u32x4* wp;
@@ -608,11 +615,17 @@
 }
 
 size_t node_r_floats(int64_t rows) { return (size_t)MATCHA_N_HEAD * rows * 64; }
-int launch_node_r(const float* XN, const float* frag, int64_t rows, float* rn, hipStream_t st, float* vn) {
+int launch_node_r(const float* XN, const float* frag, int64_t rows, float* rn, hipStream_t st, float* vn, const CompactArgs* compact) {
   NodeRArgs g;
   g.X = XN; g.wfrag = reinterpret_cast<const u32x4*>(frag); g.rn = rn; g.rows = (int)rows; g.vn = vn;
+  g.ncompact = 0;
+  g.compact = CompactArgs{};
+  if (compact) {
+    if (compact->first == 1 && compact->nsb <= kCompactRoleSb) { g.ncompact = 1; g.compact = *compact; }
+    else MATCHA_TRY(launch_tile_compact(*compact, st));
+  }
   ProfScope ps(MATCHA_PROF_FUSED_FWD, 0.0, st);
-  hipLaunchKernelGGL(node_r_kernel, dim3((unsigned)cdiv(rows, 32), vn ? 2 * MATCHA_N_HEAD : MATCHA_N_HEAD), dim3(64), 0, st, g);
+  hipLaunchKernelGGL(node_r_kernel, dim3((unsigned)cdiv(rows, 32), (vn ? 2 * MATCHA_N_HEAD : MATCHA_N_HEAD) + g.ncompact), dim3(64), 0, st, g);
   MATCHA_CHECK_LAUNCH("node_r_kernel");
   return MATCHA_OK;
 }
diff --git a/matcha_amd/csrc/kernels.hpp b/matcha_amd/csrc/kernels.hpp
--- a/matcha_amd/csrc/kernels.hpp
+++ b/matcha_amd/csrc/kernels.hpp
@@ -53,8 +53,10 @@
 int ragged_tiles_cap(int64_t B, int L);
 int ragged_halves_cap(int64_t B, int L);
 void ragged_carve(int64_t B, int L, char* base, Ragged& r);
+struct PlanDeferred; struct TilePackArgs; struct CompactArgs;
 int launch_ragged_plan(const int64_t* x, int64_t B, int L, int64_t n_nodes, int32_t* status, const Ragged& r, hipStream_t st, int level = 2,
-                       int64_t* node_ids = nullptr, int32_t* node_cnt = nullptr, float* node_zero = nullptr);
+                       int64_t* node_ids = nullptr, int32_t* node_cnt = nullptr, float* node_zero = nullptr,
+                       PlanDeferred* defer = nullptr);
 
 struct HeadParams {
   const float *gp, *bp, *g1, *b1, *g2, *b2, *wc, *bc;
@@ -104,6 +106,7 @@
   int disable_node_r;
   int disable_node_v;
   int disable_node_dx;
+  int disable_launch_pairs;
   int debug_nan, fused_dbg;
 };
 Options& options();
@@ -162,7 +165,7 @@
 };
 int launch_fused_fwd32(const matcha_tensors& p, const Ragged& rg, int64_t B, int L, const FusedFwdLaunch& a, hipStream_t st);
 size_t node_r_floats(int64_t rows);
-int launch_node_r(const float* XN, const float* frag, int64_t rows, float* rn, hipStream_t st, float* vn = nullptr);
+int launch_node_r(const float* XN, const float* frag, int64_t rows, float* rn, hipStream_t st, float* vn = nullptr, const CompactArgs* compact = nullptr);
 int tail_bwd_grid();
 size_t tail_bwd_slab_floats();
 int launch_tail_bwd64(const matcha_tensors& p, const float* dH2, const float* Y, const float* H1, const Ragged& rg, const uint64_t* seed, float p_fc1,
@@ -171,6 +174,7 @@
 
 size_t fused_bwd_ws_floats(int64_t B, int L);
 struct TailReduceArgs;
+struct Unfold2Args;
 struct FusedBwdLaunch {
   const float *folded, *merged;
   NodeOperands x;
@@ -182,6 +186,8 @@
   bool dx_atomic, dx_zeroed;
   bool dx_node = false;
   const TailReduceArgs* tail;
+  bool paired = false;
+  Unfold2Args* unfold2 = nullptr;
 };
 int launch_fused_bwd_merged(const matcha_tensors& p, const Ragged& rg, int64_t B, int L, const FusedBwdLaunch& a, matcha_tensors& grads, hipStream_t st);
 size_t fused_qkv_floats(int64_t B, int L);
@@ -202,7 +208,8 @@
 struct PrepSpec { const matcha_tensors* p; float* folded; float* merged; float* frag; };
 int launch_front_fwd(const matcha_tensors& p, const int64_t* ids, const float* table, const float* dense, const matcha_frozen& f, int n_attr,
                      const Ragged& rg, int64_t tcap, float* x0, float* X, hipStream_t st, const PrepSpec* prep = nullptr,
-                     const int32_t* count = nullptr);
+                     const int32_t* count = nullptr,
+                     const TilePackArgs* pack = nullptr);
 size_t front_bwd_ws_floats();
 int launch_front_bwd(const matcha_tensors& p, const float* X, const float* dxh, int nslab, int64_t tcap, const float* dxpad, const float* dXs, const float* x0,
                      const int64_t* ids, const matcha_frozen& f, int n_attr, const Ragged& rg, float* dX0, float* dtable, float* ws,
@@ -210,7 +217,8 @@
                      const int32_t* node_count = nullptr);
 int launch_node_xhat(const float* XN, const int32_t* node_count, int64_t rows_cap, float* xhatN, hipStream_t st);
 int launch_node_scatter(const float* XN, const float* dxh, const float* dxpad, const float* dXs, const Ragged& rg, int64_t tcap, float* G, hipStream_t st,
-                        const int32_t* node_count = nullptr, int64_t rows = 0);
+                        const int32_t* node_count = nullptr, int64_t rows = 0,
+                        const Unfold2Args* unfold2 = nullptr);
 
 int launch_attn_fwd(const float* Q, const float* K, const float* V, const int32_t* row_off, int64_t B, int L, int d, float* O, float* P,
                     hipStream_t st, bool shared_kv = false);
diff --git a/matcha_amd/csrc/model.hip b/matcha_amd/csrc/model.hip
--- a/matcha_amd/csrc/model.hip
+++ b/matcha_amd/csrc/model.hip
@@ -6,6 +6,8 @@
 
 #include "kernels.hpp"
 #include "tail_reduce.hpp"
+#include "fb_unfold.hpp"
+#include "ragged_roles.hpp"
 
 namespace matcha {
 
@@ -103,7 +105,7 @@
 struct OptionName { const char* name; int Options::*field; };
 static const OptionName kOptionNames[] = {
     {"disable_fused", &Options::disable_fused}, {"disable_merged", &Options::disable_merged}, {"disable_small_batch", &Options::disable_small_batch},
-    {"disable_wide_gemm", &Options::disable_wide_gemm}, {"disable_node_front", &Options::disable_node_front}, {"disable_node_r", &Options::disable_node_r}, {"disable_node_v", &Options::disable_node_v}, {"disable_node_dx", &Options::disable_node_dx}, {"debug_nan", &Options::debug_nan}, {"fused_dbg", &Options::fused_dbg}};
+    {"disable_wide_gemm", &Options::disable_wide_gemm}, {"disable_node_front", &Options::disable_node_front}, {"disable_node_r", &Options::disable_node_r}, {"disable_node_v", &Options::disable_node_v}, {"disable_node_dx", &Options::disable_node_dx}, {"disable_launch_pairs", &Options::disable_launch_pairs}, {"debug_nan", &Options::debug_nan}, {"fused_dbg", &Options::fused_dbg}};
 Options& options() {
   static Options o = [] {
     Options v;
@@ -146,6 +148,7 @@
   bool node;
   bool node_r, node_v;
   bool node_dx;
+  bool paired;
 };
 static std::mutex g_fwd_mu;
 static std::unordered_map<const void*, std::pair<StepRoute, uint64_t>> g_fwd_state;
@@ -286,6 +289,7 @@
   r.split_tail = r.lif && !r.small && (options().fused_dbg & 1) == 0;
   r.dx_zeroed = r.lif && atomics && (r.split_tail || r.small) && want_losses;
   r.node_dx = r.node_v && r.lif && r.split_tail && r.dx_zeroed && node_dx_shape(s, B, L) && !options().disable_node_dx;
+  r.paired = r.fused && !options().disable_launch_pairs;
   return r;
 }
 static NodeOperands node_operands(const StepRoute& r, const matcha_shape& s, const Workspace& w) {
@@ -447,8 +451,11 @@
   const bool keep = !opts->forward_only;
   const NodeOperands nx = node_operands(route, s, w);
   const bool tgt = has_target(objective, y, w_bce);
+  PlanDeferred deferred;
+  deferred.pending = false;
   MATCHA_TRY(launch_ragged_plan(x, B, L, s.n_nodes, opts->status, w.rg, st, route.half_plan ? 1 : 0, route.node ? w.node_ids : nullptr, route.node ? w.node_cnt : nullptr,
-                                (route.node && keep) ? w.GN : nullptr));
+                                (route.node && keep) ? w.GN : nullptr,
+                                (route.paired && route.node) ? &deferred : nullptr));
   float* recon_out = losses ? losses + 1 : nullptr;
   const bool recon_zero_in_loss = s.mode == 0 && recon_out && route.fused && tgt;
   if (s.mode == 0) {
@@ -463,9 +470,11 @@
   if (prep_in_front) {
     const PrepSpec prep = {&p, w.folded, w.merged, w.frag};
     if (route.node) {
-      MATCHA_TRY(launch_front_fwd(p, w.node_ids, p.table, nullptr, *frozen, s.n_attr, w.rg, nx.rows, keep ? w.x0N : nullptr, nx.X, st, &prep, w.node_cnt));
+      MATCHA_TRY(launch_front_fwd(p, w.node_ids, p.table, nullptr, *frozen, s.n_attr, w.rg, nx.rows, keep ? w.x0N : nullptr, nx.X, st, &prep, w.node_cnt,
+                                  deferred.pending ? &deferred.pack : nullptr));
       if (keep) MATCHA_TRY(launch_node_xhat(nx.X, w.node_cnt, nx.rows, nx.xhat, st));
-      if (nx.rn) MATCHA_TRY(launch_node_r(nx.X, w.frag, nx.rows, nx.rn, st, nx.vn));
+      if (nx.rn) MATCHA_TRY(launch_node_r(nx.X, w.frag, nx.rows, nx.rn, st, nx.vn, deferred.pending ? &deferred.compact : nullptr));
+      else if (deferred.pending) MATCHA_TRY(launch_tile_compact(deferred.compact, st));
     } else
     MATCHA_TRY(launch_front_fwd(p, ids, s.mode == 0 ? p.table : nullptr, s.mode == 0 ? nullptr : w.node, *frozen, s.n_attr, w.rg, Tn, keep ? w.x0 : nullptr, w.X, st, &prep));
   } else if (!route.adj_fused) {
@@ -710,13 +719,18 @@
     a.dxh = w.dO; a.ws = w.fb_ws; a.dZ0 = route.front ? nullptr : w.dZ0;
     a.dx_atomic = dx_atomic; a.dx_zeroed = dx_zeroed; a.tail = tail_in_bwd ? &tail_args : nullptr;
     a.dx_node = route.node_dx;
+    Unfold2Args unfold2;
+    const bool unfold2_in_scatter = route.paired && route.front && route.node;
+    a.paired = route.paired; a.unfold2 = unfold2_in_scatter ? &unfold2 : nullptr;
     MATCHA_CHECK_ARG(!route.node_dx || (dx_zeroed && nx.rows <= Tn), "matcha_backward: the heads' per-node d x_hat rows do not fit dO");
     MATCHA_TRY(launch_fused_bwd_merged(p, w.rg, B, L, a, g_, st));
-    MATCHA_TRY(encoder_done(*opts, st));
+    if (!unfold2_in_scatter) MATCHA_TRY(encoder_done(*opts, st));
     if (route.front) {
       if (s.mode == 0) MATCHA_CHECK_ARG(g_.table, "matcha_backward: table mode without a table gradient buffer");
       if (route.node) {
-        MATCHA_TRY(launch_node_scatter(nx.X, w.dO, fused_bwd_dxpad(w.fb_ws), w.dXs, w.rg, Tn, w.GN, st, route.node_dx ? w.node_cnt : nullptr, nx.rows));
+        MATCHA_TRY(launch_node_scatter(nx.X, w.dO, fused_bwd_dxpad(w.fb_ws), w.dXs, w.rg, Tn, w.GN, st, route.node_dx ? w.node_cnt : nullptr, nx.rows,
+                                       unfold2_in_scatter ? &unfold2 : nullptr));
+        if (unfold2_in_scatter) MATCHA_TRY(encoder_done(*opts, st));
         MATCHA_TRY(launch_front_bwd(p, nx.X, nullptr, 1, nx.rows, fused_bwd_dxpad(w.fb_ws), w.GN, w.x0N, w.node_ids, *frozen, s.n_attr, w.rg, nullptr, g_.table, w.front_ws, g_, st, touched, w.node_cnt));
         return MATCHA_OK;
       }
diff --git a/matcha_amd/csrc/ragged.hip b/matcha_amd/csrc/ragged.hip
--- a/matcha_amd/csrc/ragged.hip
+++ b/matcha_amd/csrc/ragged.hip
@@ -1,4 +1,5 @@
 #include "kernels.hpp"
+#include "ragged_roles.hpp"
 
 namespace matcha {
 
@@ -138,60 +139,13 @@
       reinterpret_cast<float4*>(node_zero)[i] = make_float4(0.f, 0.f, 0.f, 0.f);
 }
 
-constexpr int kFullTok = 63;
-constexpr int kHalfTok = 31;
-constexpr int kSuperTok = 63 * 32;
-
-__device__ __forceinline__ int tile_pack_wave(const int32_t* __restrict__ row_off, int64_t B, int nsb, int s, bool half, int cap_per_sb,
-                                              const int32_t* __restrict__ sb_first, int4* __restrict__ out, int lane) {
-  const int kTileTok = half ? kHalfTok : kFullTok;
-  const int b_lo = sb_first[s];
-  int b_hi = (int)B;
-  for (int q = s + 1; q < nsb; ++q)
-    if (sb_first[q] < (int)B) { b_hi = sb_first[q]; break; }
-  int nt = 0;
-  if (b_lo < b_hi) {
-    int tile_b0 = b_lo;
-    int tile_tok0 = __builtin_amdgcn_readfirstlane(row_off[b_lo]);
-    for (int base = b_lo; base < b_hi; base += 64) {
-      const int idx = base + lane;
-      const bool valid = idx < b_hi;
-      const int so = valid ? row_off[idx] : 0;
-      const int eo = valid ? row_off[idx + 1] : 0;
-      for (;;) {
-        const uint64_t over = __ballot(valid && eo - tile_tok0 > kTileTok);
-        if (over == 0) break;
-        const int i = __ffsll((long long)over) - 1;
-        const int start = __builtin_amdgcn_readlane(so, i);
-        if (lane == 0 && nt < cap_per_sb) out[nt] = make_int4(tile_tok0, start - tile_tok0, tile_b0, base + i - tile_b0);
-        ++nt;
-        tile_b0 = base + i;
-        tile_tok0 = start;
-      }
-    }
-    const int end = __builtin_amdgcn_readfirstlane(row_off[b_hi]);
-    if (lane == 0 && nt < cap_per_sb) out[nt] = make_int4(tile_tok0, end - tile_tok0, tile_b0, b_hi - tile_b0);
-    ++nt;
-  }
-  return nt < cap_per_sb ? nt : cap_per_sb;
-}
-
-__global__ __launch_bounds__(64) void tile_pack_kernel(const int32_t* __restrict__ row_off, int64_t B, int nsb, int cap_per_sb0, int cap_per_sb1,
-                                                       const int32_t* __restrict__ sb_first, int32_t* __restrict__ sb_tiles0,
-                                                       int32_t* __restrict__ sb_cnt0, int32_t* __restrict__ sb_tiles1, int32_t* __restrict__ sb_cnt1, int y0) {
-  const int s = blockIdx.x, lane = threadIdx.x;
-  const bool half = (int)blockIdx.y + y0 != 0;
-  const int cap_per_sb = half ? cap_per_sb1 : cap_per_sb0;
-  int32_t* sb_tiles = half ? sb_tiles1 : sb_tiles0;
-  int32_t* sb_cnt = half ? sb_cnt1 : sb_cnt0;
-  const int nt = tile_pack_wave(row_off, B, nsb, s, half, cap_per_sb, sb_first, reinterpret_cast<int4*>(sb_tiles) + (int64_t)s * cap_per_sb, lane);
-  if (lane == 0) sb_cnt[s] = nt;
-}
-
-struct CompactArgs {
-  const int32_t* sb_tiles[2]; int32_t* sb_cnt[2]; int cap_per_sb[2]; int ntiles_cap[2]; int32_t* meta[2];
-};
-__global__ __launch_bounds__(1024) void tile_compact_kernel(CompactArgs a, int nsb, int32_t* __restrict__ count, int x0) {
+__global__ __launch_bounds__(64) void tile_pack_kernel(TilePackArgs a) {
+  tile_pack_role(a, (int)blockIdx.y * a.nsb + (int)blockIdx.x, threadIdx.x);
+}
+
+__global__ __launch_bounds__(1024) void tile_compact_kernel(CompactArgs a) {
+  const int nsb = a.nsb, x0 = a.first;
+  int32_t* __restrict__ count = a.count;
   const int which = (int)blockIdx.x + x0;
   if (x0 != 0 && threadIdx.x == 0) count[2] = 0;
   const int32_t* __restrict__ sb_tiles = a.sb_tiles[which];
@@ -428,8 +382,20 @@
   r.tok_tile = (int32_t*)take((size_t)(T + 1) * 4);
 }
 
+int launch_tile_pack(const TilePackArgs& a, hipStream_t st) {
+  hipLaunchKernelGGL(tile_pack_kernel, dim3(a.nsb, 2 - a.first), dim3(64), 0, st, a);
+  MATCHA_CHECK_LAUNCH("tile_pack_kernel");
+  return MATCHA_OK;
+}
+int launch_tile_compact(const CompactArgs& a, hipStream_t st) {
+  hipLaunchKernelGGL(tile_compact_kernel, dim3(2 - a.first), dim3(1024), 0, st, a);
+  MATCHA_CHECK_LAUNCH("tile_compact_kernel");
+  return MATCHA_OK;
+}
+
 int launch_ragged_plan(const int64_t* x, int64_t B, int L, int64_t n_nodes, int32_t* status, const Ragged& r, hipStream_t st, int level,
-                       int64_t* node_ids, int32_t* node_cnt, float* node_zero) {
+                       int64_t* node_ids, int32_t* node_cnt, float* node_zero, PlanDeferred* defer) {
+  if (defer) defer->pending = false;
   if (B <= kSmallRows && r.nsb <= kSmallSb && !options().disable_small_batch) {
     PlanSmallArgs a;
     a.x = x; a.B = B; a.L = L; a.n_nodes = n_nodes; a.status = status;
@@ -452,14 +418,20 @@
   MATCHA_CHECK_LAUNCH("row_fill_kernel");
   if (level <= 0) return MATCHA_OK;
   const int first = level >= 2 ? 0 : 1;
-  hipLaunchKernelGGL(tile_pack_kernel, dim3(r.nsb, 2 - first), dim3(64), 0, st, r.row_off, B, r.nsb, r.sb_cap, r.sb_hcap, r.sb_first, r.sb_tiles, r.sb_cnt,
-                     r.sb_htiles, r.sb_hcnt, first);
-  MATCHA_CHECK_LAUNCH("tile_pack_kernel");
+  TilePackArgs pa;
+  pa.row_off = r.row_off; pa.B = B; pa.nsb = r.nsb; pa.sb_first = r.sb_first; pa.first = first; pa.ntasks = r.nsb * (2 - first);
+  pa.cap_per_sb[0] = r.sb_cap; pa.sb_tiles[0] = r.sb_tiles; pa.sb_cnt[0] = r.sb_cnt;
+  pa.cap_per_sb[1] = r.sb_hcap; pa.sb_tiles[1] = r.sb_htiles; pa.sb_cnt[1] = r.sb_hcnt;
   CompactArgs ca;
   ca.sb_tiles[0] = r.sb_tiles; ca.sb_cnt[0] = r.sb_cnt; ca.cap_per_sb[0] = r.sb_cap; ca.ntiles_cap[0] = r.ntiles; ca.meta[0] = r.tile_meta;
   ca.sb_tiles[1] = r.sb_htiles; ca.sb_cnt[1] = r.sb_hcnt; ca.cap_per_sb[1] = r.sb_hcap; ca.ntiles_cap[1] = r.nhalves; ca.meta[1] = r.half_meta;
-  hipLaunchKernelGGL(tile_compact_kernel, dim3(2 - first), dim3(1024), 0, st, ca, r.nsb, r.count, first);
-  MATCHA_CHECK_LAUNCH("tile_compact_kernel");
+  ca.nsb = r.nsb; ca.count = r.count; ca.first = first;
+  if (defer && level == 1) {
+    defer->pending = true; defer->pack = pa; defer->compact = ca;
+    return MATCHA_OK;
+  }
+  MATCHA_TRY(launch_tile_pack(pa, st));
+  MATCHA_TRY(launch_tile_compact(ca, st));
   if (level >= 2) {
     hipLaunchKernelGGL(tok_tile_kernel, dim3(r.ntiles), dim3(64), 0, st, r.tile_meta, r.tok_tile);
     MATCHA_CHECK_LAUNCH("tok_tile_kernel");
diff --git a/matcha_amd/csrc/ragged_roles.hpp b/matcha_amd/csrc/ragged_roles.hpp
--- /dev/null
+++ b/matcha_amd/csrc/ragged_roles.hpp
@@ -0,0 +1,113 @@
+#pragma once
+#include "kernels.hpp"
+
+namespace matcha {
+
+constexpr int kFullTok = 63;
+constexpr int kHalfTok = 31;
+constexpr int kSuperTok = 63 * 32;
+
+__device__ __forceinline__ int tile_pack_wave(const int32_t* __restrict__ row_off, int64_t B, int nsb, int s, bool half, int cap_per_sb,
+                                              const int32_t* __restrict__ sb_first, int4* __restrict__ out, int lane) {
+  const int kTileTok = half ? kHalfTok : kFullTok;
+  const int b_lo = sb_first[s];
+  int b_hi = (int)B;
+  for (int q = s + 1; q < nsb; ++q)
+    if (sb_first[q] < (int)B) { b_hi = sb_first[q]; break; }
+  int nt = 0;
+  if (b_lo < b_hi) {
+    int tile_b0 = b_lo;
+    int tile_tok0 = __builtin_amdgcn_readfirstlane(row_off[b_lo]);
+    for (int base = b_lo; base < b_hi; base += 64) {
+      const int idx = base + lane;
+      const bool valid = idx < b_hi;
+      const int so = valid ? row_off[idx] : 0;
+      const int eo = valid ? row_off[idx + 1] : 0;
+      for (;;) {
+        const uint64_t over = __ballot(valid && eo - tile_tok0 > kTileTok);
+        if (over == 0) break;
+        const int i = __ffsll((long long)over) - 1;
+        const int start = __builtin_amdgcn_readlane(so, i);
+        if (lane == 0 && nt < cap_per_sb) out[nt] = make_int4(tile_tok0, start - tile_tok0, tile_b0, base + i - tile_b0);
+        ++nt;
+        tile_b0 = base + i;
+        tile_tok0 = start;
+      }
+    }
+    const int end = __builtin_amdgcn_readfirstlane(row_off[b_hi]);
+    if (lane == 0 && nt < cap_per_sb) out[nt] = make_int4(tile_tok0, end - tile_tok0, tile_b0, b_hi - tile_b0);
+    ++nt;
+  }
+  return nt < cap_per_sb ? nt : cap_per_sb;
+}
+
+struct TilePackArgs {
+  const int32_t* row_off; int64_t B; int nsb; const int32_t* sb_first;
+  int cap_per_sb[2]; int32_t* sb_tiles[2]; int32_t* sb_cnt[2];
+  int first, ntasks;
+};
+__device__ __forceinline__ void tile_pack_role(const TilePackArgs& a, int task, int lane) {
+  if (task >= a.ntasks) return;
+  const bool half = a.first + task / a.nsb != 0;
+  const int s = task % a.nsb;
+  const int cap_per_sb = half ? a.cap_per_sb[1] : a.cap_per_sb[0];
+  int32_t* sb_tiles = half ? a.sb_tiles[1] : a.sb_tiles[0];
+  int32_t* sb_cnt = half ? a.sb_cnt[1] : a.sb_cnt[0];
+  const int nt = tile_pack_wave(a.row_off, a.B, a.nsb, s, half, cap_per_sb, a.sb_first, reinterpret_cast<int4*>(sb_tiles) + (int64_t)s * cap_per_sb, lane);
+  if (lane == 0) sb_cnt[s] = nt;
+}
+
+struct CompactArgs {
+  const int32_t* sb_tiles[2]; int32_t* sb_cnt[2]; int cap_per_sb[2]; int ntiles_cap[2]; int32_t* meta[2];
+  int nsb; int32_t* count; int first;
+};
+constexpr int kCompactRoleSb = 1024;
+__device__ __forceinline__ void tile_compact_role(const CompactArgs& a, int part, int nparts, int lane, int* __restrict__ offs) {
+  const bool half = a.first != 0;
+  const int which = half ? 1 : 0, nsb = a.nsb;
+  const int32_t* __restrict__ sb_cnt = half ? a.sb_cnt[1] : a.sb_cnt[0];
+  const int cap_per_sb = half ? a.cap_per_sb[1] : a.cap_per_sb[0], ntiles_cap = half ? a.ntiles_cap[1] : a.ntiles_cap[0];
+  int carry = 0;
+  for (int base = 0; base < nsb; base += 64) {
+    const int i = base + lane;
+    const int c = i < nsb ? sb_cnt[i] : 0;
+    int incl = c;
+#pragma unroll
+    for (int o = 1; o < 64; o <<= 1) {
+      const int u = __shfl_up(incl, o, 64);
+      if (lane >= o) incl += u;
+    }
+    if (i < nsb) offs[i] = carry + incl - c;
+    carry += __shfl(incl, 63, 64);
+  }
+  const int total = carry < ntiles_cap ? carry : ntiles_cap;
+  if (lane == 0) offs[nsb] = total;
+  if (part == 0 && lane == 0) {
+    a.count[2 + which] = total;
+    if (which != 0) a.count[2] = 0;
+  }
+  __syncthreads();
+  const int4* __restrict__ src = reinterpret_cast<const int4*>(half ? a.sb_tiles[1] : a.sb_tiles[0]);
+  int4* __restrict__ dst = reinterpret_cast<int4*>(half ? a.meta[1] : a.meta[0]);
+  const int step = nparts * 64;
+  auto fetch = [&](int j) {
+    const int i = j < total ? j : total - 1;
+    int lo = 0, hi = nsb;
+    while (hi - lo > 1) { const int mid = (lo + hi) >> 1; if (offs[mid] <= i) lo = mid; else hi = mid; }
+    return src[(int64_t)lo * cap_per_sb + (i - offs[lo])];
+  };
+  for (int i0 = part * 64 + lane; i0 < total; i0 += 4 * step) {
+    const int4 v0 = fetch(i0), v1 = fetch(i0 + step), v2 = fetch(i0 + 2 * step), v3 = fetch(i0 + 3 * step);
+    dst[i0] = v0;
+    if (i0 + step < total) dst[i0 + step] = v1;
+    if (i0 + 2 * step < total) dst[i0 + 2 * step] = v2;
+    if (i0 + 3 * step < total) dst[i0 + 3 * step] = v3;
+  }
+  for (int i = total + part * 64 + lane; i < ntiles_cap + 2; i += step) dst[i] = make_int4(0, 0, 0, 0);
+}
+
+struct PlanDeferred { bool pending; TilePackArgs pack; CompactArgs compact; };
+int launch_tile_pack(const TilePackArgs& a, hipStream_t st);
+int launch_tile_compact(const CompactArgs& a, hipStream_t st);
+
+}
```

Result: faster. 58.98 million hyperedges/s, median of 6 (+2.4%).
